# GiviMAD/rustpotter

Measured on AMD Instinct MI355X. Metric: 10ms-frame MFCC+DTW scorings/sec, higher is better.
Workload: dtype f32; 1 GPU; C3: 65536 synthetic 16 kHz f32 streams x 8 templates per GPU (4 s streams, L=100, K=5, band 5, ScoreMode::Max, avg gate off); streams_per_gpu=65536, templates=8, template_chunks=1, device=AMD Radeon Graphics, compute_units=256, build=gfx950, world_size=1, backend=none (one rank)

## Files before the change

### bindings/rustpotter_hip.rs

```rust
#![allow(non_camel_case_types)]
use std::collections::HashMap;
use std::ffi::{c_void, CStr, CString};
use std::os::raw::{c_char, c_int};

use crate::{
    AudioFmt, BandPassConfig, DetectorConfig, Endianness, FiltersConfig, GainNormalizationConfig, RustpotterConfig, SampleFormat,
    ScoreMode, VADMode, WakewordModel, WakewordRef, WakewordSave,
};

pub const RP_SAMPLE_I8: c_int = 0;
pub const RP_SAMPLE_I16: c_int = 1;
pub const RP_SAMPLE_I32: c_int = 2;
pub const RP_SAMPLE_F32: c_int = 3;
pub const RP_ENDIAN_BIG: c_int = 0;
pub const RP_ENDIAN_LITTLE: c_int = 1;
pub const RP_ENDIAN_NATIVE: c_int = 2;
pub const RP_SCORE_AVERAGE: c_int = 0;
pub const RP_SCORE_MAX: c_int = 1;
pub const RP_SCORE_MEDIAN: c_int = 2;
pub const RP_SCORE_P25: c_int = 3;
pub const RP_SCORE_P50: c_int = 4;
pub const RP_SCORE_P75: c_int = 5;
pub const RP_SCORE_P80: c_int = 6;
pub const RP_SCORE_P90: c_int = 7;
pub const RP_SCORE_P95: c_int = 8;
pub const RP_VAD_NONE: c_int = 0;
pub const RP_VAD_EASY: c_int = 1;
pub const RP_VAD_MEDIUM: c_int = 2;
pub const RP_VAD_HARD: c_int = 3;
pub const RP_MODEL_TINY: c_int = 0;
pub const RP_MODEL_SMALL: c_int = 1;
pub const RP_MODEL_MEDIUM: c_int = 2;
pub const RP_MODEL_LARGE: c_int = 3;
pub const RP_CTX_DEVICE_POINTERS: c_int = 0;
pub const RP_CTX_HOST_POINTERS: c_int = 1;
pub const RP_CTX_FULL_SCORES: c_int = 2;
pub const RP_CTX_ARITH_STRICT_F32: c_int = 4;
pub const RP_CTX_ARITH_FAST_SPLIT: c_int = 8;
pub const RP_CTX_RAGGED_MATRIX: c_int = 16;
pub const RP_ARITH_F32_MATRIX: c_int = 0;
pub const RP_ARITH_STRICT_F32: c_int = 1;
pub const RP_ARITH_FAST_SPLIT: c_int = 2;
pub const RP_DTW_KERNEL_MFMA: c_int = 1;
pub const RP_DTW_KERNEL_MFMA_WIDE: c_int = 2;
pub const RP_DTW_KERNEL_RAGGED: c_int = 4;
pub const RP_DTW_KERNEL_REGISTER: c_int = 8;
pub const RP_DTW_KERNEL_GENERIC: c_int = 16;
pub const RP_DTW_KERNEL_SINGLE: c_int = 32;
pub const RP_DTW_KERNEL_REF_ALL: c_int = 64;
pub const RP_DTW_KERNEL_MFMA_GROUP: c_int = 128;
pub const RP_DTW_PRODUCTS_BF16X3: c_int = 256;
pub const RP_DTW_PRODUCTS_F16X2: c_int = 512;
pub const RP_MLP_F32: c_int = 0;
pub const RP_MLP_BF16: c_int = 1;
pub const RP_MLP_F32_STRICT: c_int = 2;
pub const RP_MLP_F32_FAST: c_int = 3;

#[repr(C)] #[derive(Clone, Copy)] pub struct rp_audio_fmt { pub sample_rate: usize, pub sample_format: c_int, pub channels: u16, pub endianness: c_int }
#[repr(C)] #[derive(Clone, Copy)] pub struct rp_detector_config { pub avg_threshold: f32, pub threshold: f32, pub min_scores: usize, pub eager: bool, pub score_ref: f32, pub band_size: u16, pub score_mode: c_int, pub vad_mode: c_int }
#[repr(C)] #[derive(Clone, Copy)] pub struct rp_gain_normalization_config { pub enabled: bool, pub has_gain_ref: bool, pub gain_ref: f32, pub min_gain: f32, pub max_gain: f32 }
#[repr(C)] #[derive(Clone, Copy)] pub struct rp_band_pass_config { pub enabled: bool, pub low_cutoff: f32, pub high_cutoff: f32 }
#[repr(C)] #[derive(Clone, Copy)] pub struct rp_filters_config { pub gain_normalizer: rp_gain_normalization_config, pub band_pass: rp_band_pass_config }
#[repr(C)] #[derive(Clone, Copy)] pub struct rp_config { pub fmt: rp_audio_fmt, pub detector: rp_detector_config, pub filters: rp_filters_config }
#[repr(C)] pub struct rp_detection { pub name: *const c_char, pub avg_score: f32, pub score: f32, pub n_scores: usize, pub score_names: *const *const c_char, pub scores: *const f32, pub counter: usize, pub gain: f32 }
#[repr(C)] #[derive(Clone, Copy)] pub struct rp_train_options { pub m_type: c_int, pub learning_rate: f32, pub epochs: usize, pub test_epochs: usize, pub mfcc_size: u16, pub seed: u64 }
#[repr(C)] #[derive(Clone, Copy)] pub struct rp_wakeword_spec { pub templates: *const rp_templates, pub model: *const rp_model, pub none_index: c_int, pub precision: c_int, pub threshold: f32, pub avg_threshold: f32 }
#[repr(C)] #[derive(Clone, Copy, Default, Debug, PartialEq)] pub struct rp_batch_detection { pub stream: i32, pub frame: i32, pub window: i32, pub counter: i32, pub avg_score: f32, pub score: f32 }
pub enum rp_detector {}
pub enum rp_ctx {}
pub enum rp_templates {}
pub enum rp_stream_batch {}
pub enum rp_model {}

extern "C" {
    pub fn rp_config_default(out: *mut rp_config);
    pub fn rp_new(config: *const rp_config, out: *mut *mut rp_detector) -> c_int;
    pub fn rp_free(d: *mut rp_detector);
    pub fn rp_add_wakeword_from_buffer(d: *mut rp_detector, key: *const c_char, buffer: *const u8, len: usize) -> c_int;
    pub fn rp_add_wakeword_from_file(d: *mut rp_detector, key: *const c_char, path: *const c_char) -> c_int;
    pub fn rp_remove_wakeword(d: *mut rp_detector, key: *const c_char) -> bool;
    pub fn rp_remove_wakewords(d: *mut rp_detector) -> bool;
    pub fn rp_get_samples_per_frame(d: *const rp_detector) -> usize;
    pub fn rp_get_bytes_per_frame(d: *const rp_detector) -> usize;
    pub fn rp_get_partial_detection(d: *const rp_detector, out: *mut rp_detection) -> c_int;
    pub fn rp_get_rms_level(d: *const rp_detector) -> f32;
    pub fn rp_get_gain(d: *const rp_detector) -> f32;
    pub fn rp_get_rms_level_ref(d: *const rp_detector) -> f32;
    pub fn rp_process_bytes(d: *mut rp_detector, audio_bytes: *const u8, len: usize, out: *mut rp_detection) -> c_int;
    pub fn rp_process_samples_i8(d: *mut rp_detector, samples: *const i8, n: usize, out: *mut rp_detection) -> c_int;
    pub fn rp_process_samples_i16(d: *mut rp_detector, samples: *const i16, n: usize, out: *mut rp_detection) -> c_int;
    pub fn rp_process_samples_i32(d: *mut rp_detector, samples: *const i32, n: usize, out: *mut rp_detection) -> c_int;
    pub fn rp_process_samples_f32(d: *mut rp_detector, samples: *const f32, n: usize, out: *mut rp_detection) -> c_int;
    pub fn rp_update_config(d: *mut rp_detector, config: *const rp_config) -> c_int;
    pub fn rp_update_detector_config(d: *mut rp_detector, config: *const rp_detector_config) -> c_int;
    pub fn rp_update_filters_config(d: *mut rp_detector, config: *const rp_filters_config) -> c_int;
    pub fn rp_reset(d: *mut rp_detector);
    pub fn rp_last_error() -> *const c_char;

    pub fn rp_ctx_new(device: c_int, flags: c_int, out: *mut *mut rp_ctx) -> c_int;
    pub fn rp_ctx_free(ctx: *mut rp_ctx);
    pub fn rp_ctx_set_stream(ctx: *mut rp_ctx, hip_stream: *mut c_void) -> c_int;
    pub fn rp_ctx_synchronize(ctx: *mut rp_ctx) -> c_int;
    pub fn rp_ctx_dtw_ref_pairs(ctx: *mut rp_ctx, pairs: *mut u64) -> c_int;
    pub fn rp_ctx_dtw_kernels(ctx: *mut rp_ctx) -> c_int;
    pub fn rp_ctx_set_arithmetic(ctx: *mut rp_ctx, arith: c_int, ragged_matrix: c_int) -> c_int;
    pub fn rp_ctx_arithmetic(ctx: *mut rp_ctx, ragged_matrix: *mut c_int) -> c_int;
    pub fn rp_ctx_last_mlp_kernel(ctx: *mut rp_ctx) -> *const c_char;
    pub fn rp_build_info() -> *const c_char;
    pub fn rp_sharded_gather_info() -> *const c_char;
    pub fn rp_mfcc_num_frames(n_samples: usize) -> usize;
    pub fn rp_mfcc_batch(ctx: *mut rp_ctx, pcm: *const f32, S: usize, n_samples: usize, pcm_stride: usize, K: c_int, mfcc: *mut f32) -> c_int;
    pub fn rp_mfcc_batch_fmt(ctx: *mut rp_ctx, pcm: *const c_void, fmt: c_int, S: usize, n_samples: usize, pcm_stride: usize, K: c_int,
                             mfcc: *mut f32) -> c_int;
    pub fn rp_wakeword_ref_build(ctx: *mut rp_ctx, name: *const c_char, threshold: *const f32, avg_threshold: *const f32, n: usize,
                                 sample_names: *const *const c_char, wav_buffers: *const *const u8, wav_lens: *const usize,
                                 mfcc_size: u16, rms_from_files: c_int, out_rpw: *mut *mut u8, out_len: *mut usize) -> c_int;
    pub fn rp_buffer_free(buffer: *mut u8);
    pub fn rp_wakeword_model_train(ctx: *mut rp_ctx, options: *const rp_train_options, n_train: usize, train_names: *const *const c_char,
                                   train_wavs: *const *const u8, train_lens: *const usize, n_test: usize, test_names: *const *const c_char,
                                   test_wavs: *const *const u8, test_lens: *const usize, prev_model: *const u8, prev_model_len: usize,
                                   out_rpw: *mut *mut u8, out_len: *mut usize, final_loss: *mut f32, test_accuracy: *mut f32) -> c_int;
    pub fn rp_frontend_batch(ctx: *mut rp_ctx, pcm: *const c_void, fmt: c_int, S: usize, n_samples: usize, pcm_stride: usize,
                             filters: *const rp_filters_config, rms_level_ref: f32, window_size: usize, pcm_out: *mut f32,
                             out_stride: usize, rms: *mut f32, gains: *mut f32) -> c_int;
    pub fn rp_templates_new(ctx: *mut rp_ctx, T: c_int, K: c_int, lens: *const c_int, feats: *const f32, avg_len: c_int, avg: *const f32,
                            out: *mut *mut rp_templates) -> c_int;
    pub fn rp_templates_free(t: *mut rp_templates);
    pub fn rp_templates_max_len(t: *const rp_templates) -> c_int;
    pub fn rp_dtw_score_batch(ctx: *mut rp_ctx, mfcc: *const f32, S: usize, n_frames: usize, t: *const rp_templates, score_ref: f32,
                              band_size: c_int, score_mode: c_int, with_avg: c_int, scores: *mut f32, avg: *mut f32, agg: *mut f32) -> c_int;
    pub fn rp_detect_scan(ctx: *mut rp_ctx, agg: *const f32, avg: *const f32, S: usize, n_frames: usize, max_len: c_int,
                          config: *const rp_detector_config, avg_enabled: c_int, mfcc: *const f32, K: c_int,
                          det: *mut rp_batch_detection, n_det: *mut i32, max_det: c_int) -> c_int;
    pub fn rp_batch_detect(ctx: *mut rp_ctx, pcm: *const f32, S: usize, n_samples: usize, pcm_stride: usize, t: *const rp_templates,
                           config: *const rp_detector_config, det: *mut rp_batch_detection, n_det: *mut i32, max_det: c_int,
                           scores: *mut f32, agg: *mut f32) -> c_int;
    pub fn rp_batch_detect_fmt(ctx: *mut rp_ctx, pcm: *const c_void, fmt: c_int, S: usize, n_samples: usize, pcm_stride: usize,
                               t: *const rp_templates, config: *const rp_detector_config, det: *mut rp_batch_detection, n_det: *mut i32,
                               max_det: c_int, scores: *mut f32, agg: *mut f32) -> c_int;
    pub fn rp_batch_detect_ingest(ctx: *mut rp_ctx, pcm: *const c_void, fmt: c_int, S: usize, n_samples: usize, pcm_stride: usize,
                                  t: *const rp_templates, config: *const rp_detector_config, det: *mut rp_batch_detection, n_det: *mut i32,
                                  max_det: c_int, block_streams: usize, seconds: *mut f64) -> c_int;
    pub fn rp_batch_detect_sharded(ctxs: *const *mut rp_ctx, t: *const *const rp_templates, n_shards: c_int, pcm: *const *const c_void,
                                   fmt: c_int, S: *const usize, n_samples: usize, pcm_stride: usize, config: *const rp_detector_config,
                                   det: *mut rp_batch_detection, n_det: *mut i32, max_det: c_int) -> c_int;
    pub fn rp_batch_detect_multi(ctx: *mut rp_ctx, pcm: *const c_void, fmt: c_int, S: usize, n_samples: usize, pcm_stride: usize,
                                 n_wakewords: usize, t: *const *const rp_templates, config: *const rp_detector_config,
                                 thresholds: *const f32, avg_thresholds: *const f32, det: *mut rp_batch_detection,
                                 det_wakeword: *mut i32, n_det: *mut i32, max_det: c_int) -> c_int;
    pub fn rp_resampler_frame_lengths(sample_rate: usize, in_len: *mut usize, out_len: *mut usize) -> c_int;
    pub fn rp_resample_batch(ctx: *mut rp_ctx, pcm: *const c_void, fmt: c_int, channels: c_int, sample_rate: usize, S: usize,
                             n_samples: usize, pcm_stride: usize, out: *mut f32, out_stride: usize) -> c_int;
    pub fn rp_stream_batch_new(ctx: *mut rp_ctx, t: *const rp_templates, config: *const rp_detector_config, S: usize,
                               max_chunks_per_call: usize, out: *mut *mut rp_stream_batch) -> c_int;
    pub fn rp_stream_batch_free(b: *mut rp_stream_batch);
    pub fn rp_stream_batch_process(b: *mut rp_stream_batch, pcm: *const c_void, fmt: c_int, n_chunks: usize, pcm_stride: usize,
                                   det: *mut rp_batch_detection, n_det: *mut i32, max_det: c_int, agg: *mut f32) -> c_int;
    pub fn rp_stream_batch_set_input(b: *mut rp_stream_batch, sample_rate: usize, channels: c_int) -> c_int;
    pub fn rp_stream_batch_samples_per_chunk(b: *const rp_stream_batch) -> usize;
    pub fn rp_stream_batch_reset(b: *mut rp_stream_batch, stream: i64) -> c_int;
    pub fn rp_stream_batch_chunks_seen(b: *const rp_stream_batch) -> usize;
    pub fn rp_stream_batch_set_filters(b: *mut rp_stream_batch, filters: *const rp_filters_config, rms_level_ref: f32) -> c_int;
    pub fn rp_stream_batch_levels(b: *mut rp_stream_batch, rms: *mut f32, gains: *mut f32) -> c_int;
    pub fn rp_stream_batch_new_multi(ctx: *mut rp_ctx, n_wakewords: usize, wakewords: *const rp_wakeword_spec, mfcc_size: c_int,
                                     config: *const rp_detector_config, S: usize, max_chunks_per_call: usize, out: *mut *mut rp_stream_batch) -> c_int;
    pub fn rp_stream_batch_process_multi(b: *mut rp_stream_batch, pcm: *const c_void, fmt: c_int, n_chunks: usize, pcm_stride: usize,
                                         det: *mut rp_batch_detection, det_wakeword: *mut i32, det_label: *mut i32, n_det: *mut i32, max_det: c_int) -> c_int;
    pub fn rp_model_new(ctx: *mut rp_ctx, n_layers: c_int, dims: *const c_int, weights: *const *const f32, biases: *const *const f32,
                        out: *mut *mut rp_model) -> c_int;
    pub fn rp_model_free(m: *mut rp_model);
    pub fn rp_mlp_forward_batch(ctx: *mut rp_ctx, model: *const rp_model, x: *const f32, B: usize, precision: c_int, logits: *mut f32) -> c_int;
    pub fn rp_mlp_forward_windows(ctx: *mut rp_ctx, model: *const rp_model, mfcc: *const f32, S: usize, n_frames: usize, mfcc_size: c_int, precision: c_int, logits: *mut f32) -> c_int;
    pub fn rp_batch_detect_model(ctx: *mut rp_ctx, pcm: *const c_void, fmt: c_int, S: usize, n_samples: usize, pcm_stride: usize,
                                 model: *const rp_model, mfcc_size: c_int, none_index: c_int, config: *const rp_detector_config,
                                 precision: c_int, det: *mut rp_batch_detection, det_label: *mut i32, n_det: *mut i32, max_det: c_int) -> c_int;
    pub fn rp_synth_pcm_batch(ctx: *mut rp_ctx, seed: u64, first_stream: u64, S: usize, n_samples: usize, pcm_stride: usize, pcm: *mut f32) -> c_int;
    pub fn rp_ctx_timing_enable(ctx: *mut rp_ctx, enable: c_int) -> c_int;
    pub fn rp_ctx_timing_read(ctx: *mut rp_ctx, kernel: c_int, avg_ms: *mut f64, launches: *mut c_int) -> c_int;
    pub fn rp_ctx_timing_reset(ctx: *mut rp_ctx) -> c_int;
    pub fn rp_version() -> *const c_char;
}

impl From<&AudioFmt> for rp_audio_fmt {
    fn from(f: &AudioFmt) -> Self {
        rp_audio_fmt {
            sample_rate: f.sample_rate,
            sample_format: match f.sample_format { SampleFormat::I8 => RP_SAMPLE_I8, SampleFormat::I16 => RP_SAMPLE_I16, SampleFormat::I32 => RP_SAMPLE_I32, SampleFormat::F32 => RP_SAMPLE_F32 },
            channels: f.channels,
            endianness: match f.endianness { Endianness::Big => RP_ENDIAN_BIG, Endianness::Little => RP_ENDIAN_LITTLE, Endianness::Native => RP_ENDIAN_NATIVE },
        }
    }
}
pub fn score_mode_to_c(m: ScoreMode) -> c_int {
    match m {
        ScoreMode::Average => RP_SCORE_AVERAGE, ScoreMode::Max => RP_SCORE_MAX, ScoreMode::Median => RP_SCORE_MEDIAN,
        ScoreMode::P25 => RP_SCORE_P25, ScoreMode::P50 => RP_SCORE_P50, ScoreMode::P75 => RP_SCORE_P75,
        ScoreMode::P80 => RP_SCORE_P80, ScoreMode::P90 => RP_SCORE_P90, ScoreMode::P95 => RP_SCORE_P95,
    }
}
impl From<&DetectorConfig> for rp_detector_config {
    fn from(d: &DetectorConfig) -> Self {
        rp_detector_config {
            avg_threshold: d.avg_threshold, threshold: d.threshold, min_scores: d.min_scores, eager: d.eager, score_ref: d.score_ref,
            band_size: d.band_size, score_mode: score_mode_to_c(d.score_mode),
            vad_mode: match d.vad_mode { None => RP_VAD_NONE, Some(VADMode::Easy) => RP_VAD_EASY, Some(VADMode::Medium) => RP_VAD_MEDIUM, Some(VADMode::Hard) => RP_VAD_HARD },
        }
    }
}
impl From<&GainNormalizationConfig> for rp_gain_normalization_config {
    fn from(g: &GainNormalizationConfig) -> Self {
        rp_gain_normalization_config { enabled: g.enabled, has_gain_ref: g.gain_ref.is_some(), gain_ref: g.gain_ref.unwrap_or(0.0), min_gain: g.min_gain, max_gain: g.max_gain }
    }
}
impl From<&BandPassConfig> for rp_band_pass_config {
    fn from(b: &BandPassConfig) -> Self { rp_band_pass_config { enabled: b.enabled, low_cutoff: b.low_cutoff, high_cutoff: b.high_cutoff } }
}
impl From<&FiltersConfig> for rp_filters_config {
    fn from(f: &FiltersConfig) -> Self { rp_filters_config { gain_normalizer: (&f.gain_normalizer).into(), band_pass: (&f.band_pass).into() } }
}
impl From<&RustpotterConfig> for rp_config {
    fn from(c: &RustpotterConfig) -> Self { rp_config { fmt: (&c.fmt).into(), detector: (&c.detector).into(), filters: (&c.filters).into() } }
}

pub struct RustpotterDetection { pub name: String, pub avg_score: f32, pub score: f32, pub scores: HashMap<String, f32>, pub counter: usize, pub gain: f32 }

pub trait Sample: Copy { unsafe fn process(d: *mut rp_detector, s: &[Self], out: *mut rp_detection) -> c_int; }
impl Sample for i8 { unsafe fn process(d: *mut rp_detector, s: &[i8], o: *mut rp_detection) -> c_int { rp_process_samples_i8(d, s.as_ptr(), s.len(), o) } }
impl Sample for i16 { unsafe fn process(d: *mut rp_detector, s: &[i16], o: *mut rp_detection) -> c_int { rp_process_samples_i16(d, s.as_ptr(), s.len(), o) } }
impl Sample for i32 { unsafe fn process(d: *mut rp_detector, s: &[i32], o: *mut rp_detection) -> c_int { rp_process_samples_i32(d, s.as_ptr(), s.len(), o) } }
impl Sample for f32 { unsafe fn process(d: *mut rp_detector, s: &[f32], o: *mut rp_detection) -> c_int { rp_process_samples_f32(d, s.as_ptr(), s.len(), o) } }

fn last_error() -> String { unsafe { CStr::from_ptr(rp_last_error()).to_string_lossy().into_owned() } }
fn status(r: c_int) -> Result<(), String> { if r < 0 { Err(last_error()) } else { Ok(()) } }
unsafe fn owned(d: &rp_detection) -> RustpotterDetection {
    let mut scores = HashMap::new();
    for i in 0..d.n_scores { scores.insert(CStr::from_ptr(*d.score_names.add(i)).to_string_lossy().into_owned(), *d.scores.add(i)); }
    RustpotterDetection { name: CStr::from_ptr(d.name).to_string_lossy().into_owned(), avg_score: d.avg_score, score: d.score, scores, counter: d.counter, gain: d.gain }
}

pub struct Rustpotter { h: *mut rp_detector, partial: Option<RustpotterDetection> }
unsafe impl Send for Rustpotter {}
impl Drop for Rustpotter { fn drop(&mut self) { unsafe { rp_free(self.h) } } }
impl Rustpotter {
    pub fn new(config: &RustpotterConfig) -> Result<Rustpotter, String> {
        let c: rp_config = config.into();
        let mut h = std::ptr::null_mut();
        if unsafe { rp_new(&c, &mut h) } < 0 { Err(last_error()) } else { Ok(Rustpotter { h, partial: None }) }
    }
    fn refresh_partial(&mut self) {
        let mut d = std::mem::MaybeUninit::<rp_detection>::uninit();
        self.partial = unsafe { if rp_get_partial_detection(self.h, d.as_mut_ptr()) == 1 { Some(owned(&d.assume_init())) } else { None } };
    }
    pub fn add_wakeword_ref(&mut self, key: &str, wakeword: WakewordRef) -> Result<(), String> {
        self.add_wakeword_from_buffer(key, &wakeword.save_to_buffer()?)
    }
    pub fn add_wakeword_model(&mut self, key: &str, wakeword: WakewordModel) -> Result<(), String> {
        self.add_wakeword_from_buffer(key, &wakeword.save_to_buffer()?)
    }
    pub fn add_wakeword_from_buffer(&mut self, key: &str, buffer: &[u8]) -> Result<(), String> {
        let k = CString::new(key).map_err(|e| e.to_string())?;
        let r = status(unsafe { rp_add_wakeword_from_buffer(self.h, k.as_ptr(), buffer.as_ptr(), buffer.len()) });
        self.refresh_partial();
        r
    }
    pub fn add_wakeword_from_file(&mut self, key: &str, path: &str) -> Result<(), String> {
        let (k, p) = (CString::new(key).map_err(|e| e.to_string())?, CString::new(path).map_err(|e| e.to_string())?);
        let r = status(unsafe { rp_add_wakeword_from_file(self.h, k.as_ptr(), p.as_ptr()) });
        self.refresh_partial();
        r
    }
    pub fn remove_wakeword(&mut self, key: &str) -> bool { CString::new(key).map(|k| unsafe { rp_remove_wakeword(self.h, k.as_ptr()) }).unwrap_or(false) }
    pub fn remove_wakewords(&mut self) -> bool { unsafe { rp_remove_wakewords(self.h) } }
    pub fn get_samples_per_frame(&self) -> usize { unsafe { rp_get_samples_per_frame(self.h) } }
    pub fn get_bytes_per_frame(&self) -> usize { unsafe { rp_get_bytes_per_frame(self.h) } }
    pub fn get_partial_detection(&self) -> Option<&RustpotterDetection> { self.partial.as_ref() }
    pub fn get_rms_level(&self) -> f32 { unsafe { rp_get_rms_level(self.h) } }
    pub fn get_gain(&self) -> f32 { unsafe { rp_get_gain(self.h) } }
    pub fn get_rms_level_ref(&self) -> f32 { unsafe { rp_get_rms_level_ref(self.h) } }
    pub fn process_bytes(&mut self, audio_bytes: &[u8]) -> Option<RustpotterDetection> {
        let mut d = std::mem::MaybeUninit::<rp_detection>::uninit();
        let r = unsafe { if rp_process_bytes(self.h, audio_bytes.as_ptr(), audio_bytes.len(), d.as_mut_ptr()) == 1 { Some(owned(&d.assume_init())) } else { None } };
        self.refresh_partial();
        r
    }
    pub fn process_samples<T: Sample>(&mut self, audio_samples: Vec<T>) -> Option<RustpotterDetection> {
        let mut d = std::mem::MaybeUninit::<rp_detection>::uninit();
        let r = unsafe { if T::process(self.h, &audio_samples, d.as_mut_ptr()) == 1 { Some(owned(&d.assume_init())) } else { None } };
        self.refresh_partial();
        r
    }
    pub fn update_config(&mut self, config: &RustpotterConfig) { let c: rp_config = config.into(); unsafe { rp_update_config(self.h, &c); } self.refresh_partial(); }
    pub fn update_detector_config(&mut self, config: &DetectorConfig) { let c: rp_detector_config = config.into(); unsafe { rp_update_detector_config(self.h, &c); } self.refresh_partial(); }
    pub fn update_filters_config(&mut self, config: &FiltersConfig) { let c: rp_filters_config = config.into(); unsafe { rp_update_filters_config(self.h, &c); } self.refresh_partial(); }
    pub fn reset(&mut self) { unsafe { rp_reset(self.h) } self.partial = None; }
}

pub fn default_c_config() -> rp_config { let mut c = std::mem::MaybeUninit::<rp_config>::uninit(); unsafe { rp_config_default(c.as_mut_ptr()); c.assume_init() } }
pub fn version() -> String { unsafe { CStr::from_ptr(rp_version()).to_string_lossy().into_owned() } }
pub fn build_info() -> String { unsafe { CStr::from_ptr(rp_build_info()).to_string_lossy().into_owned() } }
pub fn sharded_gather_info() -> String { unsafe { CStr::from_ptr(rp_sharded_gather_info()).to_string_lossy().into_owned() } }
pub fn mfcc_num_frames(n_samples: usize) -> usize { unsafe { rp_mfcc_num_frames(n_samples) } }
pub fn resampler_frame_lengths(sample_rate: usize) -> Result<(usize, usize), String> {
    let (mut i, mut o) = (0usize, 0usize);
    status(unsafe { rp_resampler_frame_lengths(sample_rate, &mut i, &mut o) })?;
    Ok((i, o))
}

pub struct Templates { h: *mut rp_templates, pub n_templates: usize, pub mfcc_size: usize }
impl Drop for Templates { fn drop(&mut self) { unsafe { rp_templates_free(self.h) } } }
impl Templates {
    pub fn max_len(&self) -> usize { unsafe { rp_templates_max_len(self.h) as usize } }
}
pub struct Model { h: *mut rp_model, pub dims: Vec<c_int> }
impl Drop for Model { fn drop(&mut self) { unsafe { rp_model_free(self.h) } } }

pub struct WindowScores { pub n_win: usize, pub scores: Vec<f32>, pub avg: Vec<f32>, pub agg: Vec<f32> }
pub type Detections = Vec<Vec<rp_batch_detection>>;

fn split_detections(det: Vec<rp_batch_detection>, n_det: Vec<i32>, max_det: usize) -> Detections {
    (0..n_det.len()).map(|s| det[s * max_det..s * max_det + (n_det[s].max(0) as usize).min(max_det)].to_vec()).collect()
}

pub struct HipContext { h: *mut rp_ctx }
unsafe impl Send for HipContext {}
impl Drop for HipContext { fn drop(&mut self) { unsafe { rp_ctx_free(self.h) } } }
impl HipContext {
    pub fn new(device: c_int) -> Result<HipContext, String> { HipContext::with_flags(device, RP_CTX_HOST_POINTERS) }
    pub fn with_flags(device: c_int, flags: c_int) -> Result<HipContext, String> {
        let mut h = std::ptr::null_mut();
        status(unsafe { rp_ctx_new(device, flags, &mut h) })?;
        Ok(HipContext { h })
    }
    pub fn raw(&self) -> *mut rp_ctx { self.h }
    pub fn set_stream(&self, hip_stream: *mut c_void) -> Result<(), String> { status(unsafe { rp_ctx_set_stream(self.h, hip_stream) }) }
    pub fn synchronize(&self) -> Result<(), String> { status(unsafe { rp_ctx_synchronize(self.h) }) }
    pub fn last_mlp_kernel(&self) -> String {
        let p = unsafe { rp_ctx_last_mlp_kernel(self.h) };
        if p.is_null() { String::new() } else { unsafe { CStr::from_ptr(p) }.to_string_lossy().into_owned() }
    }
    pub fn dtw_kernels(&self) -> u32 { unsafe { rp_ctx_dtw_kernels(self.h) as u32 } }
    pub fn set_arithmetic(&self, arith: c_int, ragged_matrix: bool) -> Result<(), String> {
        status(unsafe { rp_ctx_set_arithmetic(self.h, arith, ragged_matrix as c_int) })
    }
    pub fn arithmetic(&self) -> (c_int, bool) {
        let mut r: c_int = 0;
        let a = unsafe { rp_ctx_arithmetic(self.h, &mut r) };
        (a, r != 0)
    }
    pub fn dtw_ref_pairs(&self) -> Result<u64, String> {
        let mut v: u64 = 0;
        status(unsafe { rp_ctx_dtw_ref_pairs(self.h, &mut v) })?;
        Ok(v)
    }

    pub fn mfcc_batch(&self, pcm: &[f32], n_streams: usize, n_samples: usize, mfcc_size: u16) -> Result<Vec<f32>, String> {
        assert!(pcm.len() >= n_streams * n_samples);
        let mut out = vec![0f32; n_streams * mfcc_num_frames(n_samples) * mfcc_size as usize];
        status(unsafe { rp_mfcc_batch(self.h, pcm.as_ptr(), n_streams, n_samples, n_samples, mfcc_size as c_int, out.as_mut_ptr()) })?;
        Ok(out)
    }
    pub fn mfcc_batch_fmt<T: Sample>(&self, pcm: &[T], fmt: SampleFormat, n_streams: usize, n_samples: usize, mfcc_size: u16) -> Result<Vec<f32>, String> {
        assert!(pcm.len() >= n_streams * n_samples);
        let f = rp_audio_fmt::from(&AudioFmt { sample_rate: 16000, sample_format: fmt, channels: 1, endianness: Endianness::Native }).sample_format;
        let mut out = vec![0f32; n_streams * mfcc_num_frames(n_samples) * mfcc_size as usize];
        status(unsafe { rp_mfcc_batch_fmt(self.h, pcm.as_ptr() as *const c_void, f, n_streams, n_samples, n_samples, mfcc_size as c_int, out.as_mut_ptr()) })?;
        Ok(out)
    }
    pub fn templates(&self, templates: &[Vec<Vec<f32>>], avg: Option<&Vec<Vec<f32>>>) -> Result<Templates, String> {
        let k = templates.first().and_then(|t| t.first()).map_or(0, |f| f.len());
        let lens: Vec<c_int> = templates.iter().map(|t| t.len() as c_int).collect();
        let feats: Vec<f32> = templates.iter().flat_map(|t| t.iter().flatten().copied()).collect();
        let avg_flat: Vec<f32> = avg.map_or(Vec::new(), |a| a.iter().flatten().copied().collect());
        let mut h = std::ptr::null_mut();
        status(unsafe {
            rp_templates_new(self.h, lens.len() as c_int, k as c_int, lens.as_ptr(), feats.as_ptr(), avg.map_or(0, |a| a.len() as c_int),
                             if avg.is_some() { avg_flat.as_ptr() } else { std::ptr::null() }, &mut h)
        })?;
        Ok(Templates { h, n_templates: lens.len(), mfcc_size: k })
    }
    pub fn templates_from_ref(&self, w: &WakewordRef) -> Result<Templates, String> {
        let t: Vec<Vec<Vec<f32>>> = w.samples_features.values().cloned().collect();
        self.templates(&t, w.avg_features.as_ref())
    }
    pub fn dtw_score_batch(&self, mfcc: &[f32], n_streams: usize, n_frames: usize, t: &Templates, score_ref: f32, band_size: u16,
                           score_mode: ScoreMode, with_avg: bool) -> Result<WindowScores, String> {
        assert!(mfcc.len() >= n_streams * n_frames * t.mfcc_size);
        let n_win = (n_frames + 1).saturating_sub(t.max_len());
        let mut r = WindowScores { n_win, scores: vec![0f32; n_streams * n_win * t.n_templates], avg: vec![0f32; if with_avg { n_streams * n_win } else { 0 }],
                                   agg: vec![0f32; n_streams * n_win] };
        status(unsafe {
            rp_dtw_score_batch(self.h, mfcc.as_ptr(), n_streams, n_frames, t.h, score_ref, band_size as c_int, score_mode_to_c(score_mode),
                               with_avg as c_int, r.scores.as_mut_ptr(), if with_avg { r.avg.as_mut_ptr() } else { std::ptr::null_mut() }, r.agg.as_mut_ptr())
        })?;
        Ok(r)
    }
    pub fn detect_scan(&self, w: &WindowScores, n_streams: usize, n_frames: usize, max_len: usize, config: &DetectorConfig,
                       mfcc: Option<(&[f32], u16)>, max_det: usize) -> Result<Detections, String> {
        let c: rp_detector_config = config.into();
        let mut det = vec![rp_batch_detection::default(); n_streams * max_det];
        let mut n_det = vec![0i32; n_streams];
        let (mp, k) = mfcc.map_or((std::ptr::null(), 0), |(m, k)| (m.as_ptr(), k as c_int));
        status(unsafe {
            rp_detect_scan(self.h, w.agg.as_ptr(), if w.avg.is_empty() { std::ptr::null() } else { w.avg.as_ptr() }, n_streams, n_frames,
                           max_len as c_int, &c, !w.avg.is_empty() as c_int, mp, k, det.as_mut_ptr(), n_det.as_mut_ptr(), max_det as c_int)
        })?;
        Ok(split_detections(det, n_det, max_det))
    }
    pub fn batch_detect(&self, pcm: &[f32], n_streams: usize, n_samples: usize, t: &Templates, config: &DetectorConfig, max_det: usize) -> Result<Detections, String> {
        assert!(pcm.len() >= n_streams * n_samples);
        let c: rp_detector_config = config.into();
        let mut det = vec![rp_batch_detection::default(); n_streams * max_det];
        let mut n_det = vec![0i32; n_streams];
        status(unsafe {
            rp_batch_detect(self.h, pcm.as_ptr(), n_streams, n_samples, n_samples, t.h, &c, det.as_mut_ptr(), n_det.as_mut_ptr(), max_det as c_int,
                            std::ptr::null_mut(), std::ptr::null_mut())
        })?;
        Ok(split_detections(det, n_det, max_det))
    }
    pub fn batch_detect_i16(&self, pcm: &[i16], n_streams: usize, n_samples: usize, t: &Templates, config: &DetectorConfig, max_det: usize) -> Result<Detections, String> {
        assert!(pcm.len() >= n_streams * n_samples);
        let c: rp_detector_config = config.into();
        let mut det = vec![rp_batch_detection::default(); n_streams * max_det];
        let mut n_det = vec![0i32; n_streams];
        status(unsafe {
            rp_batch_detect_fmt(self.h, pcm.as_ptr() as *const c_void, RP_SAMPLE_I16, n_streams, n_samples, n_samples, t.h, &c, det.as_mut_ptr(),
                                n_det.as_mut_ptr(), max_det as c_int, std::ptr::null_mut(), std::ptr::null_mut())
        })?;
        Ok(split_detections(det, n_det, max_det))
    }
    pub fn batch_detect_ingest_i16(&self, pcm: &[i16], n_streams: usize, n_samples: usize, t: &Templates, config: &DetectorConfig, max_det: usize,
                                   block_streams: usize) -> Result<(Detections, f64), String> {
        assert!(pcm.len() >= n_streams * n_samples);
        let c: rp_detector_config = config.into();
        let mut det = vec![rp_batch_detection::default(); n_streams * max_det];
        let mut n_det = vec![0i32; n_streams];
        let mut seconds = 0f64;
        status(unsafe {
            rp_batch_detect_ingest(self.h, pcm.as_ptr() as *const c_void, RP_SAMPLE_I16, n_streams, n_samples, n_samples, t.h, &c, det.as_mut_ptr(),
                                   n_det.as_mut_ptr(), max_det as c_int, block_streams, &mut seconds)
        })?;
        Ok((split_detections(det, n_det, max_det), seconds))
    }
    pub fn batch_detect_multi(&self, pcm: &[f32], n_streams: usize, n_samples: usize, wakewords: &[&Templates], overrides: &[(Option<f32>, Option<f32>)],
                              config: &DetectorConfig, max_det: usize) -> Result<(Detections, Vec<Vec<i32>>), String> {
        assert!(pcm.len() >= n_streams * n_samples && overrides.len() == wakewords.len());
        let c: rp_detector_config = config.into();
        let ts: Vec<*const rp_templates> = wakewords.iter().map(|t| t.h as *const rp_templates).collect();
        let thr: Vec<f32> = overrides.iter().map(|o| o.0.unwrap_or(f32::NAN)).collect();
        let athr: Vec<f32> = overrides.iter().map(|o| o.1.unwrap_or(f32::NAN)).collect();
        let mut det = vec![rp_batch_detection::default(); n_streams * max_det];
        let mut which = vec![0i32; n_streams * max_det];
        let mut n_det = vec![0i32; n_streams];
        status(unsafe {
            rp_batch_detect_multi(self.h, pcm.as_ptr() as *const c_void, RP_SAMPLE_F32, n_streams, n_samples, n_samples, ts.len(), ts.as_ptr(), &c,
                                  thr.as_ptr(), athr.as_ptr(), det.as_mut_ptr(), which.as_mut_ptr(), n_det.as_mut_ptr(), max_det as c_int)
        })?;
        let w = (0..n_streams).map(|s| which[s * max_det..s * max_det + (n_det[s].max(0) as usize).min(max_det)].to_vec()).collect();
        Ok((split_detections(det, n_det, max_det), w))
    }
    pub fn model(&self, dims: &[c_int], weights: &[Vec<f32>], biases: &[Vec<f32>]) -> Result<Model, String> {
        assert!(dims.len() == weights.len() + 1 && weights.len() == biases.len());
        let wp: Vec<*const f32> = weights.iter().map(|w| w.as_ptr()).collect();
        let bp: Vec<*const f32> = biases.iter().map(|b| b.as_ptr()).collect();
        let mut h = std::ptr::null_mut();
        status(unsafe { rp_model_new(self.h, weights.len() as c_int, dims.as_ptr(), wp.as_ptr(), bp.as_ptr(), &mut h) })?;
        Ok(Model { h, dims: dims.to_vec() })
    }
    pub fn mlp_forward_batch(&self, m: &Model, x: &[f32], rows: usize, bf16: bool) -> Result<Vec<f32>, String> {
        assert!(x.len() >= rows * m.dims[0] as usize);
        let mut out = vec![0f32; rows * *m.dims.last().unwrap() as usize];
        status(unsafe { rp_mlp_forward_batch(self.h, m.h, x.as_ptr(), rows, if bf16 { RP_MLP_BF16 } else { RP_MLP_F32 }, out.as_mut_ptr()) })?;
        Ok(out)
    }
    pub fn mlp_forward_windows(&self, m: &Model, mfcc: &[f32], n_streams: usize, n_frames: usize, mfcc_size: u16) -> Result<Vec<f32>, String> {
        assert!(mfcc.len() >= n_streams * n_frames * mfcc_size as usize);
        let train_size = m.dims[0] as usize / mfcc_size as usize;
        let n_win = if n_frames >= train_size { n_frames - train_size + 1 } else { 0 };
        let mut out = vec![0f32; n_streams * n_win * *m.dims.last().unwrap() as usize];
        status(unsafe { rp_mlp_forward_windows(self.h, m.h, mfcc.as_ptr(), n_streams, n_frames, mfcc_size as c_int, RP_MLP_F32, out.as_mut_ptr()) })?;
        Ok(out)
    }
    pub fn batch_detect_model(&self, pcm: &[f32], n_streams: usize, n_samples: usize, m: &Model, mfcc_size: u16, none_index: Option<usize>,
                              config: &DetectorConfig, bf16: bool, max_det: usize) -> Result<(Detections, Vec<Vec<i32>>), String> {
        assert!(pcm.len() >= n_streams * n_samples);
        let c: rp_detector_config = config.into();
        let mut det = vec![rp_batch_detection::default(); n_streams * max_det];
        let mut label = vec![0i32; n_streams * max_det];
        let mut n_det = vec![0i32; n_streams];
        status(unsafe {
            rp_batch_detect_model(self.h, pcm.as_ptr() as *const c_void, RP_SAMPLE_F32, n_streams, n_samples, n_samples, m.h, mfcc_size as c_int,
                                  none_index.map_or(-1, |i| i as c_int), &c, if bf16 { RP_MLP_BF16 } else { RP_MLP_F32 }, det.as_mut_ptr(),
                                  label.as_mut_ptr(), n_det.as_mut_ptr(), max_det as c_int)
        })?;
        let l = (0..n_streams).map(|s| label[s * max_det..s * max_det + (n_det[s].max(0) as usize).min(max_det)].to_vec()).collect();
        Ok((split_detections(det, n_det, max_det), l))
    }
    pub fn frontend_batch(&self, pcm: &[f32], n_streams: usize, n_samples: usize, filters: &FiltersConfig, rms_level_ref: f32,
                          window_size: usize) -> Result<(Vec<f32>, Vec<f32>, Vec<f32>), String> {
        assert!(pcm.len() >= n_streams * n_samples);
        let f: rp_filters_config = filters.into();
        let nch = n_samples / 480;
        let (mut out, mut rms, mut gains) = (vec![0f32; n_streams * n_samples], vec![0f32; n_streams * nch], vec![0f32; n_streams * nch]);
        status(unsafe {
            rp_frontend_batch(self.h, pcm.as_ptr() as *const c_void, RP_SAMPLE_F32, n_streams, n_samples, n_samples, &f, rms_level_ref, window_size,
                              out.as_mut_ptr(), n_samples, rms.as_mut_ptr(), gains.as_mut_ptr())
        })?;
        Ok((out, rms, gains))
    }
    pub fn resample_batch(&self, pcm: &[f32], channels: u16, sample_rate: usize, n_streams: usize, n_samples: usize) -> Result<Vec<f32>, String> {
        assert!(pcm.len() >= n_streams * n_samples * channels as usize);
        let (fi, fo) = resampler_frame_lengths(sample_rate)?;
        let per = (n_samples / fi) * fo;
        let mut out = vec![0f32; n_streams * per];
        status(unsafe {
            rp_resample_batch(self.h, pcm.as_ptr() as *const c_void, RP_SAMPLE_F32, channels as c_int, sample_rate, n_streams, n_samples,
                              n_samples * channels as usize, out.as_mut_ptr(), per)
        })?;
        Ok(out)
    }
    pub fn synth_pcm_batch(&self, seed: u64, first_stream: u64, n_streams: usize, n_samples: usize) -> Result<Vec<f32>, String> {
        let mut out = vec![0f32; n_streams * n_samples];
        status(unsafe { rp_synth_pcm_batch(self.h, seed, first_stream, n_streams, n_samples, n_samples, out.as_mut_ptr()) })?;
        Ok(out)
    }
    pub fn timing_enable(&self, on: bool) -> Result<(), String> { status(unsafe { rp_ctx_timing_enable(self.h, on as c_int) }) }
    pub fn timing_reset(&self) -> Result<(), String> { status(unsafe { rp_ctx_timing_reset(self.h) }) }
    pub fn timing_read(&self, kernel: c_int) -> Result<(f64, c_int), String> {
        let (mut ms, mut n) = (0f64, 0 as c_int);
        status(unsafe { rp_ctx_timing_read(self.h, kernel, &mut ms, &mut n) })?;
        Ok((ms, n))
    }
}

pub struct StreamBatch<'a> { h: *mut rp_stream_batch, n_streams: usize, last_chunks: usize, _ctx: &'a HipContext, _t: std::marker::PhantomData<&'a Templates> }
pub enum BatchWakeword<'a> {
    Ref { templates: &'a Templates, threshold: Option<f32>, avg_threshold: Option<f32> },
    Model { model: &'a Model, none_index: Option<usize>, bf16: bool },
}
impl<'a> Drop for StreamBatch<'a> { fn drop(&mut self) { unsafe { rp_stream_batch_free(self.h) } } }
impl<'a> StreamBatch<'a> {
    pub fn new(ctx: &'a HipContext, t: &'a Templates, config: &DetectorConfig, n_streams: usize, max_chunks_per_call: usize) -> Result<StreamBatch<'a>, String> {
        let c: rp_detector_config = config.into();
        let mut h = std::ptr::null_mut();
        status(unsafe { rp_stream_batch_new(ctx.h, t.h, &c, n_streams, max_chunks_per_call, &mut h) })?;
        Ok(StreamBatch { h, n_streams, last_chunks: 0, _ctx: ctx, _t: std::marker::PhantomData })
    }
    pub fn new_multi(ctx: &'a HipContext, wakewords: &[BatchWakeword<'a>], mfcc_size: u16, config: &DetectorConfig, n_streams: usize,
                     max_chunks_per_call: usize) -> Result<StreamBatch<'a>, String> {
        let c: rp_detector_config = config.into();
        let specs: Vec<rp_wakeword_spec> = wakewords.iter().map(|w| match w {
            BatchWakeword::Ref { templates, threshold, avg_threshold } => rp_wakeword_spec {
                templates: templates.h as *const rp_templates, model: std::ptr::null(), none_index: -1, precision: RP_MLP_F32,
                threshold: threshold.unwrap_or(f32::NAN), avg_threshold: avg_threshold.unwrap_or(f32::NAN) },
            BatchWakeword::Model { model, none_index, bf16 } => rp_wakeword_spec {
                templates: std::ptr::null(), model: model.h as *const rp_model, none_index: none_index.map_or(-1, |i| i as c_int),
                precision: if *bf16 { RP_MLP_BF16 } else { RP_MLP_F32 }, threshold: f32::NAN, avg_threshold: f32::NAN },
        }).collect();
        let mut h = std::ptr::null_mut();
        status(unsafe { rp_stream_batch_new_multi(ctx.h, specs.len(), specs.as_ptr(), mfcc_size as c_int, &c, n_streams, max_chunks_per_call, &mut h) })?;
        Ok(StreamBatch { h, n_streams, last_chunks: 0, _ctx: ctx, _t: std::marker::PhantomData })
    }
    pub fn process_multi(&mut self, pcm: &[f32], n_chunks: usize, max_det: usize) -> Result<(Detections, Vec<Vec<i32>>, Vec<Vec<i32>>), String> {
        let stride = n_chunks * self.samples_per_chunk();
        assert!(pcm.len() >= self.n_streams * stride);
        let mut det = vec![rp_batch_detection::default(); self.n_streams * max_det];
        let (mut which, mut label) = (vec![0i32; self.n_streams * max_det], vec![0i32; self.n_streams * max_det]);
        let mut n_det = vec![0i32; self.n_streams];
        status(unsafe {
            rp_stream_batch_process_multi(self.h, pcm.as_ptr() as *const c_void, RP_SAMPLE_F32, n_chunks, stride, det.as_mut_ptr(), which.as_mut_ptr(),
                                          label.as_mut_ptr(), n_det.as_mut_ptr(), max_det as c_int)
        })?;
        self.last_chunks = n_chunks;
        let cut = |v: &Vec<i32>| -> Vec<Vec<i32>> { (0..self.n_streams).map(|s| v[s * max_det..s * max_det + (n_det[s].max(0) as usize).min(max_det)].to_vec()).collect() };
        let (w, l) = (cut(&which), cut(&label));
        Ok((split_detections(det, n_det, max_det), w, l))
    }
    pub fn set_input(&mut self, sample_rate: usize, channels: u16) -> Result<(), String> { status(unsafe { rp_stream_batch_set_input(self.h, sample_rate, channels as c_int) }) }
    pub fn set_filters(&mut self, filters: &FiltersConfig, rms_level_ref: f32) -> Result<(), String> {
        let f: rp_filters_config = filters.into();
        status(unsafe { rp_stream_batch_set_filters(self.h, &f, rms_level_ref) })
    }
    pub fn levels(&mut self) -> Result<(Vec<f32>, Vec<f32>), String> {
        let n = self.n_streams * self.last_chunks.max(1);
        let (mut rms, mut gains) = (vec![0f32; n], vec![0f32; n]);
        status(unsafe { rp_stream_batch_levels(self.h, rms.as_mut_ptr(), gains.as_mut_ptr()) })?;
        Ok((rms, gains))
    }
    pub fn samples_per_chunk(&self) -> usize { unsafe { rp_stream_batch_samples_per_chunk(self.h) } }
    pub fn chunks_seen(&self) -> usize { unsafe { rp_stream_batch_chunks_seen(self.h) } }
    pub fn process(&mut self, pcm: &[f32], n_chunks: usize, max_det: usize) -> Result<Detections, String> {
        let stride = n_chunks * self.samples_per_chunk();
        assert!(pcm.len() >= self.n_streams * stride);
        let mut det = vec![rp_batch_detection::default(); self.n_streams * max_det];
        let mut n_det = vec![0i32; self.n_streams];
        status(unsafe {
            rp_stream_batch_process(self.h, pcm.as_ptr() as *const c_void, RP_SAMPLE_F32, n_chunks, stride, det.as_mut_ptr(), n_det.as_mut_ptr(),
                                    max_det as c_int, std::ptr::null_mut())
        })?;
        self.last_chunks = n_chunks;
        Ok(split_detections(det, n_det, max_det))
    }
    pub fn reset(&mut self, stream: Option<usize>) -> Result<(), String> { status(unsafe { rp_stream_batch_reset(self.h, stream.map_or(-1, |s| s as i64)) }) }
}

pub fn batch_detect_sharded(devices: &[c_int], templates: &[Vec<Vec<f32>>], avg: Option<&Vec<Vec<f32>>>, config: &DetectorConfig,
                            shards: &[Vec<Vec<f32>>], max_det: usize) -> Result<Detections, String> {
    assert_eq!(devices.len(), shards.len());
    let c: rp_detector_config = config.into();
    let n_samples = shards.iter().flat_map(|s| s.iter()).map(|x| x.len()).next().unwrap_or(0);
    assert!(shards.iter().flat_map(|s| s.iter()).all(|x| x.len() == n_samples), "every stream must hold the same number of samples");
    let ctxs: Vec<HipContext> = devices.iter().map(|&d| HipContext::new(d)).collect::<Result<_, _>>()?;
    let tms: Vec<Templates> = ctxs.iter().map(|c| c.templates(templates, avg)).collect::<Result<_, _>>()?;
    let cp: Vec<*mut rp_ctx> = ctxs.iter().map(|c| c.h).collect();
    let tp: Vec<*const rp_templates> = tms.iter().map(|t| t.h as *const rp_templates).collect();
    let flat: Vec<Vec<f32>> = shards.iter().map(|s| s.iter().flatten().copied().collect()).collect();
    let ptrs: Vec<*const c_void> = flat.iter().map(|f| f.as_ptr() as *const c_void).collect();
    let counts: Vec<usize> = shards.iter().map(|s| s.len()).collect();
    let total: usize = counts.iter().sum();
    let mut det = vec![rp_batch_detection::default(); total * max_det];
    let mut n_det = vec![0i32; total];
    status(unsafe {
        rp_batch_detect_sharded(cp.as_ptr(), tp.as_ptr(), devices.len() as c_int, ptrs.as_ptr(), RP_SAMPLE_F32, counts.as_ptr(), n_samples,
                                n_samples, &c, det.as_mut_ptr(), n_det.as_mut_ptr(), max_det as c_int)
    })?;
    Ok(split_detections(det, n_det, max_det))
}

fn take_buffer(r: c_int, out: *mut u8, out_len: usize) -> Result<Vec<u8>, String> {
    let res = if r < 0 { Err(last_error()) } else { Ok(unsafe { std::slice::from_raw_parts(out, out_len) }.to_vec()) };
    if !out.is_null() { unsafe { rp_buffer_free(out) }; }
    res
}
pub fn wakeword_ref_from_sample_buffers(name: &str, threshold: Option<f32>, avg_threshold: Option<f32>,
                                        samples: &HashMap<String, Vec<u8>>, mfcc_size: u16) -> Result<Vec<u8>, String> {
    let cname = CString::new(name).map_err(|e| e.to_string())?;
    let names: Vec<CString> = samples.keys().map(|k| CString::new(k.as_str()).unwrap()).collect();
    let name_ptrs: Vec<*const c_char> = names.iter().map(|n| n.as_ptr()).collect();
    let bufs: Vec<*const u8> = samples.values().map(|v| v.as_ptr()).collect();
    let lens: Vec<usize> = samples.values().map(|v| v.len()).collect();
    let ctx = HipContext::with_flags(0, RP_CTX_DEVICE_POINTERS)?;
    let (mut out, mut out_len) = (std::ptr::null_mut(), 0usize);
    let r = unsafe {
        rp_wakeword_ref_build(ctx.h, cname.as_ptr(), threshold.as_ref().map_or(std::ptr::null(), |t| t as *const f32),
                              avg_threshold.as_ref().map_or(std::ptr::null(), |t| t as *const f32), names.len(),
                              name_ptrs.as_ptr(), bufs.as_ptr(), lens.as_ptr(), mfcc_size, 0, &mut out, &mut out_len)
    };
    take_buffer(r, out, out_len)
}
pub fn wakeword_model_train_from_buffers(m_type: c_int, train: &HashMap<String, Vec<u8>>, test: &HashMap<String, Vec<u8>>,
                                         learning_rate: f64, epochs: usize, test_epochs: usize, mfcc_size: u16,
                                         wakeword_model: Option<&[u8]>) -> Result<(Vec<u8>, f32, f32), String> {
    fn pack(d: &HashMap<String, Vec<u8>>) -> (Vec<CString>, Vec<*const u8>, Vec<usize>) {
        (d.keys().map(|k| CString::new(k.as_str()).unwrap()).collect(), d.values().map(|v| v.as_ptr()).collect(), d.values().map(|v| v.len()).collect())
    }
    let (trn, trb, trl) = pack(train);
    let (ten, teb, tel) = pack(test);
    let trp: Vec<*const c_char> = trn.iter().map(|n| n.as_ptr()).collect();
    let tep: Vec<*const c_char> = ten.iter().map(|n| n.as_ptr()).collect();
    let opt = rp_train_options { m_type, learning_rate: learning_rate as f32, epochs, test_epochs, mfcc_size, seed: 1 };
    let ctx = HipContext::with_flags(0, RP_CTX_DEVICE_POINTERS)?;
    let (mut out, mut out_len, mut loss, mut acc) = (std::ptr::null_mut(), 0usize, 0f32, 0f32);
    let (pm, pl) = wakeword_model.map_or((std::ptr::null(), 0), |m| (m.as_ptr(), m.len()));
    let r = unsafe {
        rp_wakeword_model_train(ctx.h, &opt, trp.len(), trp.as_ptr(), trb.as_ptr(), trl.as_ptr(), tep.len(), tep.as_ptr(), teb.as_ptr(),
                                tel.as_ptr(), pm, pl, &mut out, &mut out_len, &mut loss, &mut acc)
    };
    take_buffer(r, out, out_len).map(|b| (b, loss, acc))
}
```

### include/rustpotter_hip.h

```cpp
#ifndef RUSTPOTTER_HIP_H
#define RUSTPOTTER_HIP_H

#include <stdbool.h>
#include <stddef.h>
#include <stdint.h>

#ifdef __cplusplus
extern "C" {
#endif

typedef enum { RP_SAMPLE_I8 = 0, RP_SAMPLE_I16 = 1, RP_SAMPLE_I32 = 2, RP_SAMPLE_F32 = 3 } rp_sample_format;
typedef enum { RP_ENDIAN_BIG = 0, RP_ENDIAN_LITTLE = 1, RP_ENDIAN_NATIVE = 2 } rp_endianness;
typedef enum {
    RP_SCORE_AVERAGE = 0, RP_SCORE_MAX = 1, RP_SCORE_MEDIAN = 2, RP_SCORE_P25 = 3, RP_SCORE_P50 = 4,
    RP_SCORE_P75 = 5, RP_SCORE_P80 = 6, RP_SCORE_P90 = 7, RP_SCORE_P95 = 8
} rp_score_mode;
typedef enum { RP_VAD_NONE = 0, RP_VAD_EASY = 1, RP_VAD_MEDIUM = 2, RP_VAD_HARD = 3 } rp_vad_mode;

typedef struct {
    size_t sample_rate;
    rp_sample_format sample_format;
    uint16_t channels;
    rp_endianness endianness;
} rp_audio_fmt;

typedef struct {
    float avg_threshold;
    float threshold;
    size_t min_scores;
    bool eager;
    float score_ref;
    uint16_t band_size;
    rp_score_mode score_mode;
    rp_vad_mode vad_mode;
} rp_detector_config;

typedef struct {
    bool enabled;
    bool has_gain_ref;
    float gain_ref;
    float min_gain;
    float max_gain;
} rp_gain_normalization_config;

typedef struct {
    bool enabled;
    float low_cutoff;
    float high_cutoff;
} rp_band_pass_config;

typedef struct {
    rp_gain_normalization_config gain_normalizer;
    rp_band_pass_config band_pass;
} rp_filters_config;

typedef struct {
    rp_audio_fmt fmt;
    rp_detector_config detector;
    rp_filters_config filters;
} rp_config;

void rp_config_default(rp_config *out);

typedef struct {
    const char *name;
    float avg_score;
    float score;
    size_t n_scores;
    const char *const *score_names;
    const float *scores;
    size_t counter;
    float gain;
} rp_detection;

typedef struct rp_detector rp_detector;

int rp_new(const rp_config *config, rp_detector **out);
void rp_free(rp_detector *d);

int rp_add_wakeword_from_buffer(rp_detector *d, const char *key, const uint8_t *buffer, size_t len);
int rp_add_wakeword_from_file(rp_detector *d, const char *key, const char *path);
bool rp_remove_wakeword(rp_detector *d, const char *key);
bool rp_remove_wakewords(rp_detector *d);

size_t rp_get_samples_per_frame(const rp_detector *d);
size_t rp_get_bytes_per_frame(const rp_detector *d);
int rp_get_partial_detection(const rp_detector *d, rp_detection *out);
float rp_get_rms_level(const rp_detector *d);
float rp_get_gain(const rp_detector *d);
float rp_get_rms_level_ref(const rp_detector *d);

int rp_process_bytes(rp_detector *d, const uint8_t *audio_bytes, size_t len, rp_detection *out);
int rp_process_samples_i8(rp_detector *d, const int8_t *samples, size_t n, rp_detection *out);
int rp_process_samples_i16(rp_detector *d, const int16_t *samples, size_t n, rp_detection *out);
int rp_process_samples_i32(rp_detector *d, const int32_t *samples, size_t n, rp_detection *out);
int rp_process_samples_f32(rp_detector *d, const float *samples, size_t n, rp_detection *out);

int rp_update_config(rp_detector *d, const rp_config *config);
int rp_update_detector_config(rp_detector *d, const rp_detector_config *config);
int rp_update_filters_config(rp_detector *d, const rp_filters_config *config);
void rp_reset(rp_detector *d);

const char *rp_last_error(void);

typedef struct rp_ctx rp_ctx;
typedef struct rp_templates rp_templates;

enum {
    RP_CTX_DEVICE_POINTERS = 0, RP_CTX_HOST_POINTERS = 1, RP_CTX_FULL_SCORES = 2,
    RP_CTX_ARITH_STRICT_F32 = 4, RP_CTX_ARITH_FAST_SPLIT = 8,
    RP_CTX_RAGGED_MATRIX = 16
};

int rp_ctx_new(int device, int flags, rp_ctx **out);
enum { RP_ARITH_F32_MATRIX = 0, RP_ARITH_STRICT_F32 = 1, RP_ARITH_FAST_SPLIT = 2 };
int rp_ctx_set_arithmetic(rp_ctx *ctx, int arith, int ragged_matrix);
int rp_ctx_arithmetic(rp_ctx *ctx, int *ragged_matrix);
void rp_ctx_free(rp_ctx *ctx);
int rp_ctx_set_stream(rp_ctx *ctx, void *hip_stream);
int rp_ctx_synchronize(rp_ctx *ctx);
int rp_ctx_dtw_ref_pairs(rp_ctx *ctx, uint64_t *pairs);
enum {
    RP_DTW_KERNEL_MFMA = 1,
    RP_DTW_KERNEL_MFMA_WIDE = 2,
    RP_DTW_KERNEL_RAGGED = 4,
    RP_DTW_KERNEL_REGISTER = 8,
    RP_DTW_KERNEL_GENERIC = 16,
    RP_DTW_KERNEL_SINGLE = 32,
    RP_DTW_KERNEL_REF_ALL = 64,
    RP_DTW_KERNEL_MFMA_GROUP = 128,
    RP_DTW_PRODUCTS_BF16X3 = 256,
    RP_DTW_PRODUCTS_F16X2 = 512
};
int rp_ctx_dtw_kernels(rp_ctx *ctx);
const char *rp_build_info(void);
const char *rp_ctx_last_mlp_kernel(rp_ctx *ctx);

size_t rp_mfcc_num_frames(size_t n_samples);

int rp_mfcc_batch(rp_ctx *ctx, const float *pcm, size_t S, size_t n_samples, size_t pcm_stride, int K, float *mfcc);

int rp_mfcc_batch_fmt(rp_ctx *ctx, const void *pcm, rp_sample_format fmt, size_t S, size_t n_samples, size_t pcm_stride,
                      int K, float *mfcc);

int rp_wakeword_ref_build(rp_ctx *ctx, const char *name, const float *threshold, const float *avg_threshold, size_t n,
                          const char *const *sample_names, const uint8_t *const *wav_buffers, const size_t *wav_lens,
                          uint16_t mfcc_size, int rms_from_files, uint8_t **out_rpw, size_t *out_len);
void rp_buffer_free(uint8_t *buffer);

typedef enum { RP_MODEL_TINY = 0, RP_MODEL_SMALL = 1, RP_MODEL_MEDIUM = 2, RP_MODEL_LARGE = 3 } rp_model_type;
typedef struct {
    int m_type;
    float learning_rate;
    size_t epochs, test_epochs;
    uint16_t mfcc_size;
    uint64_t seed;
} rp_train_options;
int rp_wakeword_model_train(rp_ctx *ctx, const rp_train_options *options, size_t n_train, const char *const *train_names,
                            const uint8_t *const *train_wavs, const size_t *train_lens, size_t n_test,
                            const char *const *test_names, const uint8_t *const *test_wavs, const size_t *test_lens,
                            const uint8_t *prev_model, size_t prev_model_len, uint8_t **out_rpw, size_t *out_len,
                            float *final_loss, float *test_accuracy);

int rp_frontend_batch(rp_ctx *ctx, const void *pcm, rp_sample_format fmt, size_t S, size_t n_samples, size_t pcm_stride,
                      const rp_filters_config *filters, float rms_level_ref, size_t window_size, float *pcm_out,
                      size_t out_stride, float *rms, float *gains);

int rp_templates_new(rp_ctx *ctx, int T, int K, const int *lens, const float *feats, int avg_len, const float *avg,
                     rp_templates **out);
void rp_templates_free(rp_templates *t);
int rp_templates_max_len(const rp_templates *t);

int rp_dtw_score_batch(rp_ctx *ctx, const float *mfcc, size_t S, size_t n_frames, const rp_templates *t,
                       float score_ref, int band_size, rp_score_mode score_mode, int with_avg,
                       float *scores, float *avg, float *agg);

typedef struct {
    int32_t stream;
    int32_t frame;
    int32_t window;
    int32_t counter;
    float avg_score;
    float score;
} rp_batch_detection;

int rp_detect_scan(rp_ctx *ctx, const float *agg, const float *avg, size_t S, size_t n_frames, int max_len,
                   const rp_detector_config *config, int avg_enabled, const float *mfcc, int K,
                   rp_batch_detection *det, int32_t *n_det, int max_det);

int rp_batch_detect(rp_ctx *ctx, const float *pcm, size_t S, size_t n_samples, size_t pcm_stride, const rp_templates *t,
                    const rp_detector_config *config, rp_batch_detection *det, int32_t *n_det, int max_det,
                    float *scores, float *agg);

int rp_batch_detect_fmt(rp_ctx *ctx, const void *pcm, rp_sample_format fmt, size_t S, size_t n_samples, size_t pcm_stride,
                        const rp_templates *t, const rp_detector_config *config, rp_batch_detection *det, int32_t *n_det,
                        int max_det, float *scores, float *agg);

int rp_batch_detect_ingest(rp_ctx *ctx, const void *pcm, rp_sample_format fmt, size_t S, size_t n_samples, size_t pcm_stride,
                           const rp_templates *t, const rp_detector_config *config, rp_batch_detection *det, int32_t *n_det,
                           int max_det, size_t block_streams, double *seconds);

int rp_batch_detect_sharded(rp_ctx *const *ctxs, const rp_templates *const *t, int n_shards, const void *const *pcm,
                            rp_sample_format fmt, const size_t *S, size_t n_samples, size_t pcm_stride,
                            const rp_detector_config *config, rp_batch_detection *det, int32_t *n_det, int max_det);
const char *rp_sharded_gather_info(void);

int rp_batch_detect_multi(rp_ctx *ctx, const void *pcm, rp_sample_format fmt, size_t S, size_t n_samples, size_t pcm_stride,
                          size_t n_wakewords, const rp_templates *const *t, const rp_detector_config *config,
                          const float *thresholds, const float *avg_thresholds, rp_batch_detection *det,
                          int32_t *det_wakeword, int32_t *n_det, int max_det);

int rp_resampler_frame_lengths(size_t sample_rate, size_t *in_len, size_t *out_len);
int rp_resample_batch(rp_ctx *ctx, const void *pcm, rp_sample_format fmt, int channels, size_t sample_rate, size_t S,
                      size_t n_samples, size_t pcm_stride, float *out, size_t out_stride);

typedef struct rp_stream_batch rp_stream_batch;
int rp_stream_batch_new(rp_ctx *ctx, const rp_templates *t, const rp_detector_config *config, size_t S,
                        size_t max_chunks_per_call, rp_stream_batch **out);
void rp_stream_batch_free(rp_stream_batch *b);
int rp_stream_batch_process(rp_stream_batch *b, const void *pcm, rp_sample_format fmt, size_t n_chunks, size_t pcm_stride,
                            rp_batch_detection *det, int32_t *n_det, int max_det, float *agg);
int rp_stream_batch_set_input(rp_stream_batch *b, size_t sample_rate, int channels);
size_t rp_stream_batch_samples_per_chunk(const rp_stream_batch *b);
int rp_stream_batch_reset(rp_stream_batch *b, long long stream);
size_t rp_stream_batch_chunks_seen(const rp_stream_batch *b);
int rp_stream_batch_set_filters(rp_stream_batch *b, const rp_filters_config *filters, float rms_level_ref);
int rp_stream_batch_levels(rp_stream_batch *b, float *rms, float *gains);

typedef struct rp_model rp_model;
typedef struct {
    const rp_templates *templates;
    const rp_model *model;
    int none_index;
    int precision;
    float threshold;
    float avg_threshold;
} rp_wakeword_spec;
int rp_stream_batch_new_multi(rp_ctx *ctx, size_t n_wakewords, const rp_wakeword_spec *wakewords, int mfcc_size,
                              const rp_detector_config *config, size_t S, size_t max_chunks_per_call, rp_stream_batch **out);
int rp_stream_batch_process_multi(rp_stream_batch *b, const void *pcm, rp_sample_format fmt, size_t n_chunks, size_t pcm_stride,
                                  rp_batch_detection *det, int32_t *det_wakeword, int32_t *det_label, int32_t *n_det, int max_det);

int rp_model_new(rp_ctx *ctx, int n_layers, const int *dims, const float *const *weights, const float *const *biases,
                 rp_model **out);
void rp_model_free(rp_model *m);

enum { RP_MLP_F32 = 0, RP_MLP_BF16 = 1, RP_MLP_F32_STRICT = 2, RP_MLP_F32_FAST = 3 };

int rp_mlp_forward_batch(rp_ctx *ctx, const rp_model *model, const float *x, size_t B, int precision, float *logits);

int rp_mlp_forward_windows(rp_ctx *ctx, const rp_model *model, const float *mfcc, size_t S, size_t n_frames, int mfcc_size,
                           int precision, float *logits);

int rp_batch_detect_model(rp_ctx *ctx, const void *pcm, rp_sample_format fmt, size_t S, size_t n_samples, size_t pcm_stride,
                          const rp_model *model, int mfcc_size, int none_index, const rp_detector_config *config, int precision,
                          rp_batch_detection *det, int32_t *det_label, int32_t *n_det, int max_det);

int rp_synth_pcm_batch(rp_ctx *ctx, uint64_t seed, uint64_t first_stream, size_t S, size_t n_samples, size_t pcm_stride,
                       float *pcm);

int rp_ctx_timing_enable(rp_ctx *ctx, int enable);
int rp_ctx_timing_read(rp_ctx *ctx, int kernel, double *avg_ms, int *launches);
int rp_ctx_timing_reset(rp_ctx *ctx);

const char *rp_version(void);

#ifdef __cplusplus
}
#endif
#endif
```

### rustpotter_amd/api.py

```python
import ctypes as C
import weakref
import enum
import os

_HERE = os.path.dirname(os.path.abspath(__file__))
_LIB = None


class RustpotterError(RuntimeError):
    """Result::Err(String) of the reference."""


def lib_path():
    return os.environ.get("RP_LIB_PATH") or os.path.join(_HERE, "librustpotter_hip.so")


class SampleFormat(enum.IntEnum):
    I8 = 0
    I16 = 1
    I32 = 2
    F32 = 3


class Endianness(enum.IntEnum):
    Big = 0
    Little = 1
    Native = 2


class ScoreMode(enum.IntEnum):
    Average = 0
    Max = 1
    Median = 2
    P25 = 3
    P50 = 4
    P75 = 5
    P80 = 6
    P90 = 7
    P95 = 8


class VADMode(enum.IntEnum):
    Off = 0
    Easy = 1
    Medium = 2
    Hard = 3


class _AudioFmt(C.Structure):
    _fields_ = [("sample_rate", C.c_size_t), ("sample_format", C.c_int), ("channels", C.c_uint16), ("endianness", C.c_int)]


class _DetectorConfig(C.Structure):
    _fields_ = [("avg_threshold", C.c_float), ("threshold", C.c_float), ("min_scores", C.c_size_t), ("eager", C.c_bool),
                ("score_ref", C.c_float), ("band_size", C.c_uint16), ("score_mode", C.c_int), ("vad_mode", C.c_int)]


class _GainCfg(C.Structure):
    _fields_ = [("enabled", C.c_bool), ("has_gain_ref", C.c_bool), ("gain_ref", C.c_float), ("min_gain", C.c_float),
                ("max_gain", C.c_float)]


class _BandPassCfg(C.Structure):
    _fields_ = [("enabled", C.c_bool), ("low_cutoff", C.c_float), ("high_cutoff", C.c_float)]


class _FiltersCfg(C.Structure):
    _fields_ = [("gain_normalizer", _GainCfg), ("band_pass", _BandPassCfg)]


class _Config(C.Structure):
    _fields_ = [("fmt", _AudioFmt), ("detector", _DetectorConfig), ("filters", _FiltersCfg)]


class _Detection(C.Structure):
    _fields_ = [("name", C.c_char_p), ("avg_score", C.c_float), ("score", C.c_float), ("n_scores", C.c_size_t),
                ("score_names", C.POINTER(C.c_char_p)), ("scores", C.POINTER(C.c_float)), ("counter", C.c_size_t),
                ("gain", C.c_float)]


class _TrainOptions(C.Structure):
    _fields_ = [("m_type", C.c_int), ("learning_rate", C.c_float), ("epochs", C.c_size_t), ("test_epochs", C.c_size_t),
                ("mfcc_size", C.c_uint16), ("seed", C.c_uint64)]


class _BatchDetection(C.Structure):
    _fields_ = [("stream", C.c_int32), ("frame", C.c_int32), ("window", C.c_int32), ("counter", C.c_int32),
                ("avg_score", C.c_float), ("score", C.c_float)]


SYMBOLS = [
    "rp_config_default", "rp_new", "rp_free", "rp_add_wakeword_from_buffer", "rp_add_wakeword_from_file",
    "rp_remove_wakeword", "rp_remove_wakewords", "rp_get_samples_per_frame", "rp_get_bytes_per_frame",
    "rp_get_partial_detection", "rp_get_rms_level", "rp_get_gain", "rp_get_rms_level_ref", "rp_process_bytes",
    "rp_process_samples_i8", "rp_process_samples_i16", "rp_process_samples_i32", "rp_process_samples_f32",
    "rp_update_config", "rp_update_detector_config", "rp_update_filters_config", "rp_reset", "rp_last_error",
    "rp_ctx_new", "rp_ctx_free", "rp_ctx_set_stream", "rp_ctx_synchronize", "rp_ctx_dtw_ref_pairs", "rp_ctx_dtw_kernels", "rp_ctx_set_arithmetic", "rp_ctx_arithmetic", "rp_ctx_last_mlp_kernel", "rp_build_info", "rp_sharded_gather_info", "rp_mfcc_num_frames", "rp_mfcc_batch", "rp_mfcc_batch_fmt", "rp_batch_detect_fmt", "rp_batch_detect_ingest", "rp_frontend_batch", "rp_wakeword_ref_build", "rp_buffer_free",
    "rp_templates_new", "rp_templates_free", "rp_templates_max_len", "rp_dtw_score_batch", "rp_detect_scan", "rp_batch_detect",
    "rp_model_new", "rp_model_free", "rp_mlp_forward_batch", "rp_mlp_forward_windows", "rp_synth_pcm_batch", "rp_ctx_timing_enable", "rp_ctx_timing_read", "rp_ctx_timing_reset",
    "rp_version", "rp_stream_batch_new", "rp_stream_batch_free", "rp_stream_batch_process", "rp_stream_batch_reset",
    "rp_stream_batch_chunks_seen", "rp_resampler_frame_lengths", "rp_resample_batch",
    "rp_wakeword_model_train", "rp_stream_batch_set_input", "rp_stream_batch_samples_per_chunk",
    "rp_batch_detect_multi", "rp_batch_detect_model", "rp_batch_detect_sharded",
    "rp_stream_batch_new_multi", "rp_stream_batch_process_multi",
    "rp_stream_batch_set_filters", "rp_stream_batch_levels",
]


class _WakewordSpec(C.Structure):
    _fields_ = [("templates", C.c_void_p), ("model", C.c_void_p), ("none_index", C.c_int), ("precision", C.c_int),
                ("threshold", C.c_float), ("avg_threshold", C.c_float)]


def load_library():
    global _LIB
    if _LIB is not None:
        return _LIB
    path = lib_path()
    if not os.path.exists(path):
        raise RustpotterError(
            "librustpotter_hip.so is not built (%s): run `python -c 'import __graft_entry__ as g; g.build()'` "
            "or `make -C rustpotter_amd/csrc`; there is no CPU fallback" % path)
    try:
        import torch
    except Exception:
        pass
    L = C.CDLL(path)
    vp, fp, ip = C.c_void_p, C.POINTER(C.c_float), C.POINTER(C.c_int)
    L.rp_last_error.restype = C.c_char_p
    L.rp_version.restype = C.c_char_p
    L.rp_config_default.argtypes = [C.POINTER(_Config)]
    L.rp_new.argtypes = [C.POINTER(_Config), C.POINTER(vp)]
    L.rp_free.argtypes = [vp]
    L.rp_add_wakeword_from_buffer.argtypes = [vp, C.c_char_p, C.c_char_p, C.c_size_t]
    L.rp_add_wakeword_from_file.argtypes = [vp, C.c_char_p, C.c_char_p]
    L.rp_remove_wakeword.argtypes = [vp, C.c_char_p]
    L.rp_remove_wakeword.restype = C.c_bool
    L.rp_remove_wakewords.argtypes = [vp]
    L.rp_remove_wakewords.restype = C.c_bool
    L.rp_get_samples_per_frame.argtypes = [vp]
    L.rp_get_samples_per_frame.restype = C.c_size_t
    L.rp_get_bytes_per_frame.argtypes = [vp]
    L.rp_get_bytes_per_frame.restype = C.c_size_t
    L.rp_get_partial_detection.argtypes = [vp, C.POINTER(_Detection)]
    for n in ("rp_get_rms_level", "rp_get_gain", "rp_get_rms_level_ref"):
        getattr(L, n).argtypes = [vp]
        getattr(L, n).restype = C.c_float
    L.rp_process_bytes.argtypes = [vp, C.c_char_p, C.c_size_t, C.POINTER(_Detection)]
    for n in ("rp_process_samples_i8", "rp_process_samples_i16", "rp_process_samples_i32", "rp_process_samples_f32"):
        getattr(L, n).argtypes = [vp, vp, C.c_size_t, C.POINTER(_Detection)]
    L.rp_update_config.argtypes = [vp, C.POINTER(_Config)]
    L.rp_update_detector_config.argtypes = [vp, C.POINTER(_DetectorConfig)]
    L.rp_update_filters_config.argtypes = [vp, C.POINTER(_FiltersCfg)]
    L.rp_reset.argtypes = [vp]
    L.rp_ctx_new.argtypes = [C.c_int, C.c_int, C.POINTER(vp)]
    L.rp_ctx_free.argtypes = [vp]
    L.rp_ctx_set_stream.argtypes = [vp, vp]
    L.rp_ctx_synchronize.argtypes = [vp]
    L.rp_ctx_dtw_ref_pairs.argtypes = [vp, C.POINTER(C.c_uint64)]
    L.rp_ctx_dtw_kernels.argtypes = [vp]
    L.rp_ctx_dtw_kernels.restype = C.c_int
    L.rp_ctx_set_arithmetic.argtypes = [vp, C.c_int, C.c_int]
    L.rp_ctx_set_arithmetic.restype = C.c_int
    L.rp_ctx_arithmetic.argtypes = [vp, C.POINTER(C.c_int)]
    L.rp_ctx_arithmetic.restype = C.c_int
    L.rp_sharded_gather_info.argtypes = []
    L.rp_sharded_gather_info.restype = C.c_char_p
    L.rp_build_info.argtypes = []
    L.rp_build_info.restype = C.c_char_p
    L.rp_ctx_last_mlp_kernel.argtypes = [vp]
    L.rp_ctx_last_mlp_kernel.restype = C.c_char_p
    L.rp_mfcc_num_frames.argtypes = [C.c_size_t]
    L.rp_mfcc_num_frames.restype = C.c_size_t
    L.rp_mfcc_batch.argtypes = [vp, vp, C.c_size_t, C.c_size_t, C.c_size_t, C.c_int, vp]
    L.rp_mfcc_batch_fmt.argtypes = [vp, vp, C.c_int, C.c_size_t, C.c_size_t, C.c_size_t, C.c_int, vp]
    L.rp_batch_detect_fmt.argtypes = [vp, vp, C.c_int, C.c_size_t, C.c_size_t, C.c_size_t, vp, C.POINTER(_DetectorConfig), vp, vp, C.c_int, vp, vp]
    L.rp_batch_detect_ingest.argtypes = [vp, vp, C.c_int, C.c_size_t, C.c_size_t, C.c_size_t, vp, C.POINTER(_DetectorConfig), vp, vp, C.c_int, C.c_size_t,
                                         C.POINTER(C.c_double)]
    L.rp_frontend_batch.argtypes = [vp, vp, C.c_int, C.c_size_t, C.c_size_t, C.c_size_t, C.POINTER(_FiltersCfg), C.c_float, C.c_size_t, vp, C.c_size_t, vp, vp]
    L.rp_wakeword_ref_build.argtypes = [vp, C.c_char_p, fp, fp, C.c_size_t, C.POINTER(C.c_char_p), C.POINTER(C.c_char_p),
                                        C.POINTER(C.c_size_t), C.c_uint16, C.c_int, C.POINTER(vp), C.POINTER(C.c_size_t)]
    L.rp_buffer_free.argtypes = [vp]
    L.rp_templates_new.argtypes = [vp, C.c_int, C.c_int, ip, fp, C.c_int, fp, C.POINTER(vp)]
    L.rp_templates_free.argtypes = [vp]
    L.rp_templates_max_len.argtypes = [vp]
    L.rp_dtw_score_batch.argtypes = [vp, vp, C.c_size_t, C.c_size_t, vp, C.c_float, C.c_int, C.c_int, C.c_int, vp, vp, vp]
    L.rp_detect_scan.argtypes = [vp, vp, vp, C.c_size_t, C.c_size_t, C.c_int, C.POINTER(_DetectorConfig), C.c_int, vp, C.c_int, vp, vp, C.c_int]
    L.rp_batch_detect.argtypes = [vp, vp, C.c_size_t, C.c_size_t, C.c_size_t, vp, C.POINTER(_DetectorConfig), vp, vp, C.c_int, vp, vp]
    L.rp_wakeword_model_train.argtypes = [vp, C.POINTER(_TrainOptions), C.c_size_t, C.POINTER(C.c_char_p), C.POINTER(C.c_char_p),
                                          C.POINTER(C.c_size_t), C.c_size_t, C.POINTER(C.c_char_p), C.POINTER(C.c_char_p),
                                          C.POINTER(C.c_size_t), C.c_char_p, C.c_size_t, C.POINTER(vp), C.POINTER(C.c_size_t), fp, fp]
    L.rp_batch_detect_multi.argtypes = [vp, vp, C.c_int, C.c_size_t, C.c_size_t, C.c_size_t, C.c_size_t, C.POINTER(vp),
                                        C.POINTER(_DetectorConfig), fp, fp, vp, vp, vp, C.c_int]
    L.rp_batch_detect_sharded.argtypes = [C.POINTER(vp), C.POINTER(vp), C.c_int, C.POINTER(vp), C.c_int, C.POINTER(C.c_size_t), C.c_size_t,
                                          C.c_size_t, C.POINTER(_DetectorConfig), vp, vp, C.c_int]
    L.rp_batch_detect_model.argtypes = [vp, vp, C.c_int, C.c_size_t, C.c_size_t, C.c_size_t, vp, C.c_int, C.c_int,
                                        C.POINTER(_DetectorConfig), C.c_int, vp, vp, vp, C.c_int]
    L.rp_resampler_frame_lengths.argtypes = [C.c_size_t, C.POINTER(C.c_size_t), C.POINTER(C.c_size_t)]
    L.rp_resample_batch.argtypes = [vp, vp, C.c_int, C.c_int, C.c_size_t, C.c_size_t, C.c_size_t, C.c_size_t, vp, C.c_size_t]
    L.rp_stream_batch_new.argtypes = [vp, vp, C.POINTER(_DetectorConfig), C.c_size_t, C.c_size_t, C.POINTER(vp)]
    L.rp_stream_batch_new_multi.argtypes = [vp, C.c_size_t, C.POINTER(_WakewordSpec), C.c_int, C.POINTER(_DetectorConfig), C.c_size_t,
                                            C.c_size_t, C.POINTER(vp)]
    L.rp_stream_batch_process_multi.argtypes = [vp, vp, C.c_int, C.c_size_t, C.c_size_t, vp, vp, vp, vp, C.c_int]
    L.rp_stream_batch_free.argtypes = [vp]
    L.rp_stream_batch_free.restype = None
    L.rp_stream_batch_process.argtypes = [vp, vp, C.c_int, C.c_size_t, C.c_size_t, vp, vp, C.c_int, vp]
    L.rp_stream_batch_reset.argtypes = [vp, C.c_longlong]
    L.rp_stream_batch_set_input.argtypes = [vp, C.c_size_t, C.c_int]
    L.rp_stream_batch_set_filters.argtypes = [vp, C.POINTER(_FiltersCfg), C.c_float]
    L.rp_stream_batch_levels.argtypes = [vp, vp, vp]
    L.rp_stream_batch_samples_per_chunk.argtypes = [vp]
    L.rp_stream_batch_samples_per_chunk.restype = C.c_size_t
    L.rp_stream_batch_chunks_seen.argtypes = [vp]
    L.rp_stream_batch_chunks_seen.restype = C.c_size_t
    L.rp_model_new.argtypes = [vp, C.c_int, ip, C.POINTER(fp), C.POINTER(fp), C.POINTER(vp)]
    L.rp_model_free.argtypes = [vp]
    L.rp_mlp_forward_batch.argtypes = [vp, vp, vp, C.c_size_t, C.c_int, vp]
    L.rp_mlp_forward_windows.argtypes = [vp, vp, vp, C.c_size_t, C.c_size_t, C.c_int, C.c_int, vp]
    L.rp_synth_pcm_batch.argtypes = [vp, C.c_uint64, C.c_uint64, C.c_size_t, C.c_size_t, C.c_size_t, vp]
    L.rp_ctx_timing_enable.argtypes = [vp, C.c_int]
    L.rp_ctx_timing_read.argtypes = [vp, C.c_int, C.POINTER(C.c_double), ip]
    L.rp_ctx_timing_reset.argtypes = [vp]
    _LIB = L
    return L


def _err():
    return RustpotterError(load_library().rp_last_error().decode("utf-8", "replace"))


def sharded_gather_info():
    return load_library().rp_sharded_gather_info().decode()


def build_info():
    return load_library().rp_build_info().decode()


def resampler_frame_lengths(sample_rate):
    a, b = C.c_size_t(), C.c_size_t()
    if load_library().rp_resampler_frame_lengths(sample_rate, C.byref(a), C.byref(b)) < 0:
        raise _err()
    return a.value, b.value


def mfcc_num_frames(n_samples):
    return int(load_library().rp_mfcc_num_frames(n_samples))


class AudioFmt:
    def __init__(self):
        self.sample_rate = 16000
        self.sample_format = SampleFormat.F32
        self.channels = 1
        self.endianness = Endianness.Little


class GainNormalizationConfig:
    def __init__(self):
        self.enabled = False
        self.gain_ref = None
        self.min_gain = 0.1
        self.max_gain = 1.0


class BandPassConfig:
    def __init__(self):
        self.enabled = False
        self.low_cutoff = 80.0
        self.high_cutoff = 400.0


class FiltersConfig:
    def __init__(self):
        self.gain_normalizer = GainNormalizationConfig()
        self.band_pass = BandPassConfig()


class DetectorConfig:
    def __init__(self):
        self.avg_threshold = 0.2
        self.threshold = 0.5
        self.min_scores = 5
        self.eager = False
        self.score_ref = 0.22
        self.band_size = 5
        self.score_mode = ScoreMode.Max
        self.vad_mode = None

    def _c(self):
        c = _DetectorConfig()
        c.avg_threshold, c.threshold, c.min_scores, c.eager = self.avg_threshold, self.threshold, self.min_scores, self.eager
        c.score_ref, c.band_size, c.score_mode = self.score_ref, self.band_size, int(self.score_mode)
        c.vad_mode = int(self.vad_mode) if self.vad_mode is not None else 0
        return c


class RustpotterConfig:
    def __init__(self):
        self.fmt = AudioFmt()
        self.detector = DetectorConfig()
        self.filters = FiltersConfig()

    @staticmethod
    def default():
        return RustpotterConfig()

    def _filters_c(self):
        f = _FiltersCfg()
        g, b = self.filters.gain_normalizer, self.filters.band_pass
        f.gain_normalizer.enabled = g.enabled
        f.gain_normalizer.has_gain_ref = g.gain_ref is not None
        f.gain_normalizer.gain_ref = g.gain_ref if g.gain_ref is not None else 0.0
        f.gain_normalizer.min_gain, f.gain_normalizer.max_gain = g.min_gain, g.max_gain
        f.band_pass.enabled, f.band_pass.low_cutoff, f.band_pass.high_cutoff = b.enabled, b.low_cutoff, b.high_cutoff
        return f

    def _c(self):
        c = _Config()
        c.fmt.sample_rate, c.fmt.sample_format = self.fmt.sample_rate, int(self.fmt.sample_format)
        c.fmt.channels, c.fmt.endianness = self.fmt.channels, int(self.fmt.endianness)
        c.detector = self.detector._c()
        c.filters = self._filters_c()
        return c


class RustpotterDetection:
    def __init__(self, d):
        import numpy as np
        self.name = d.name.decode()
        self.avg_score = np.float32(d.avg_score)
        self.score = np.float32(d.score)
        self.scores = {d.score_names[i].decode(): np.float32(d.scores[i]) for i in range(d.n_scores)}
        self.counter = int(d.counter)
        self.gain = np.float32(d.gain)

    def __repr__(self):
        return "RustpotterDetection(name=%r, avg_score=%r, score=%r, counter=%d)" % (self.name, float(self.avg_score),
                                                                                      float(self.score), self.counter)


class Rustpotter:

    def __init__(self, config):
        self._L = load_library()
        self._h = C.c_void_p()
        c = config._c()
        if self._L.rp_new(C.byref(c), C.byref(self._h)) < 0:
            self._h = None
            raise _err()

    @staticmethod
    def new(config):
        return Rustpotter(config)

    def __del__(self):
        if getattr(self, "_h", None):
            self._L.rp_free(self._h)
            self._h = None

    def add_wakeword_from_file(self, key, path):
        if self._L.rp_add_wakeword_from_file(self._h, key.encode(), path.encode()) < 0:
            raise _err()

    def add_wakeword_from_buffer(self, key, buffer):
        if self._L.rp_add_wakeword_from_buffer(self._h, key.encode(), bytes(buffer), len(buffer)) < 0:
            raise _err()

    def remove_wakeword(self, key):
        return bool(self._L.rp_remove_wakeword(self._h, key.encode()))

    def remove_wakewords(self):
        return bool(self._L.rp_remove_wakewords(self._h))

    def get_samples_per_frame(self):
        return int(self._L.rp_get_samples_per_frame(self._h))

    def get_bytes_per_frame(self):
        return int(self._L.rp_get_bytes_per_frame(self._h))

    def get_partial_detection(self):
        d = _Detection()
        return RustpotterDetection(d) if self._L.rp_get_partial_detection(self._h, C.byref(d)) == 1 else None

    def get_rms_level(self):
        return float(self._L.rp_get_rms_level(self._h))

    def get_gain(self):
        return float(self._L.rp_get_gain(self._h))

    def get_rms_level_ref(self):
        return float(self._L.rp_get_rms_level_ref(self._h))

    def _ret(self, r, d):
        if r < 0:
            raise _err()
        return RustpotterDetection(d) if r == 1 else None

    def process_bytes(self, audio_bytes):
        d = _Detection()
        b = bytes(audio_bytes)
        return self._ret(self._L.rp_process_bytes(self._h, b, len(b), C.byref(d)), d)

    def process_samples(self, samples):
        import numpy as np
        a = np.ascontiguousarray(samples)
        fn = {np.dtype(np.int8): self._L.rp_process_samples_i8, np.dtype(np.int16): self._L.rp_process_samples_i16,
              np.dtype(np.int32): self._L.rp_process_samples_i32, np.dtype(np.float32): self._L.rp_process_samples_f32}[a.dtype]
        d = _Detection()
        return self._ret(fn(self._h, a.ctypes.data, a.size, C.byref(d)), d)

    def update_config(self, config):
        c = config._c()
        self._L.rp_update_config(self._h, C.byref(c))

    def update_detector_config(self, config):
        c = config._c()
        self._L.rp_update_detector_config(self._h, C.byref(c))

    def update_filters_config(self, config):
        rc = RustpotterConfig()
        rc.filters = config
        f = rc._filters_c()
        self._L.rp_update_filters_config(self._h, C.byref(f))

    def reset(self):
        self._L.rp_reset(self._h)


class Templates:

    def __init__(self, ctx, templates, avg=None):
        import numpy as np
        self._L = load_library()
        self.ctx = ctx
        self.T = len(templates)
        self.K = int(np.asarray(templates[0]).shape[1])
        lens = np.array([len(t) for t in templates], np.int32)
        feats = np.concatenate([np.ascontiguousarray(t, np.float32).reshape(-1) for t in templates]).astype(np.float32)
        avg_a = None if avg is None else np.ascontiguousarray(avg, np.float32)
        self._h = C.c_void_p()
        r = self._L.rp_templates_new(ctx._h, self.T, self.K, lens.ctypes.data_as(C.POINTER(C.c_int)),
                                     feats.ctypes.data_as(C.POINTER(C.c_float)), 0 if avg_a is None else avg_a.shape[0],
                                     None if avg_a is None else avg_a.ctypes.data_as(C.POINTER(C.c_float)), C.byref(self._h))
        if r < 0:
            self._h = None
            raise _err()
        self.max_len = int(self._L.rp_templates_max_len(self._h))
        self.has_avg = avg_a is not None

    def __del__(self):
        if getattr(self, "_h", None):
            self._L.rp_templates_free(self._h)
            self._h = None


class Model:

    def __init__(self, ctx, weights, biases):
        import numpy as np
        self._L = load_library()
        self.ctx = ctx
        ws = [np.ascontiguousarray(w, np.float32) for w in weights]
        bs = [np.ascontiguousarray(b, np.float32) for b in biases]
        dims = np.array([ws[0].shape[1]] + [w.shape[0] for w in ws], np.int32)
        fp = C.POINTER(C.c_float)
        wp = (fp * len(ws))(*[w.ctypes.data_as(fp) for w in ws])
        bp = (fp * len(bs))(*[b.ctypes.data_as(fp) for b in bs])
        self._h = C.c_void_p()
        if self._L.rp_model_new(ctx._h, len(ws), dims.ctypes.data_as(C.POINTER(C.c_int)), wp, bp, C.byref(self._h)) < 0:
            self._h = None
            raise _err()
        self.n_in, self.n_out = int(dims[0]), int(dims[-1])

    def __del__(self):
        if getattr(self, "_h", None):
            self._L.rp_model_free(self._h)
            self._h = None


DET_DTYPE = [("stream", "<i4"), ("frame", "<i4"), ("window", "<i4"), ("counter", "<i4"), ("avg_score", "<f4"), ("score", "<f4")]


class StreamBatch:

    def __init__(self, ctx, templates, detector_config, S, max_chunks_per_call=1, sample_rate=16000, channels=1, wakewords=None,
                 mfcc_size=None, filters=None, rms_level_ref=float("nan")):
        self._L = load_library()
        self.ctx, self.templates, self.S, self.max_chunks = ctx, templates, S, max_chunks_per_call
        h = C.c_void_p()
        c = detector_config._c()
        if wakewords is None:
            if self._L.rp_stream_batch_new(ctx._h, templates._h, C.byref(c), S, max_chunks_per_call, C.byref(h)) < 0:
                raise _err()
        else:
            specs = (_WakewordSpec * len(wakewords))()
            self._keep = list(wakewords)
            for sp, w in zip(specs, wakewords):
                sp.templates = w["templates"]._h if w.get("templates") is not None else None
                sp.model = w["model"]._h if w.get("model") is not None else None
                sp.none_index = w.get("none_index", -1)
                sp.precision = {"f32": 0, "bf16": 1}[w.get("precision", "f32")]
                sp.threshold = float("nan") if w.get("threshold") is None else w["threshold"]
                sp.avg_threshold = float("nan") if w.get("avg_threshold") is None else w["avg_threshold"]
            if self._L.rp_stream_batch_new_multi(ctx._h, len(wakewords), specs, mfcc_size, C.byref(c), S, max_chunks_per_call, C.byref(h)) < 0:
                raise _err()
        self._h = h
        if (sample_rate, channels) != (16000, 1) and self._L.rp_stream_batch_set_input(h, sample_rate, channels) < 0:
            raise _err()
        if filters is not None:
            self.set_filters(filters, rms_level_ref)
        self.samples_per_chunk = self._L.rp_stream_batch_samples_per_chunk(h)
        self._last_chunks = 0
        self.frames_per_chunk = resampler_frame_lengths(sample_rate)[1] // 160

    def __del__(self):
        if getattr(self, "_h", None):
            self._L.rp_stream_batch_free(self._h)
            self._h = None

    @property
    def chunks_seen(self):
        return self._L.rp_stream_batch_chunks_seen(self._h)

    def set_input(self, sample_rate, channels=1):
        if self._L.rp_stream_batch_set_input(self._h, sample_rate, channels) < 0:
            raise _err()
        self.samples_per_chunk = self._L.rp_stream_batch_samples_per_chunk(self._h)
        self.frames_per_chunk = resampler_frame_lengths(sample_rate)[1] // 160

    def set_filters(self, filters, rms_level_ref=float("nan")):
        rc = RustpotterConfig()
        rc.filters = filters
        f = rc._filters_c()
        if self._L.rp_stream_batch_set_filters(self._h, C.byref(f), rms_level_ref) < 0:
            raise _err()

    def levels(self):
        import numpy as np
        assert self.ctx.host
        n = max(self._last_chunks, 1)
        rms = np.empty((self.S, n), np.float32)
        gains = np.empty((self.S, n), np.float32)
        if self._L.rp_stream_batch_levels(self._h, rms.ctypes.data, gains.ctypes.data) < 0:
            raise _err()
        return rms, gains

    def process(self, pcm, max_det=4, want_agg=False, n_chunks=None):
        import numpy as np
        assert self.ctx.host
        pcm = np.ascontiguousarray(pcm)
        fmt = {np.dtype(np.int8): 0, np.dtype(np.int16): 1, np.dtype(np.int32): 2}.get(pcm.dtype)
        if fmt is None:
            pcm, fmt = np.ascontiguousarray(pcm, np.float32), 3
        S, N = pcm.shape
        spc = self.samples_per_chunk
        if S != self.S or (n_chunks is None and N % spc) or (n_chunks is not None and n_chunks * spc > N):
            raise ValueError("pcm must be [S][n_chunks*samples_per_chunk]")
        nc = N // spc if n_chunks is None else n_chunks
        det = np.zeros((S, max_det), dtype=DET_DTYPE)
        n_det = np.zeros(S, np.int32)
        agg = np.empty((S, self.frames_per_chunk * nc), np.float32) if want_agg else None
        if self._L.rp_stream_batch_process(self._h, pcm.ctypes.data, fmt, nc, N, det.ctypes.data, n_det.ctypes.data, max_det,
                                           None if agg is None else agg.ctypes.data) < 0:
            raise _err()
        self._last_chunks = nc
        return (det, n_det, agg) if want_agg else (det, n_det)

    def process_multi(self, pcm, max_det=4, n_chunks=None):
        import numpy as np
        assert self.ctx.host
        pcm = np.ascontiguousarray(pcm)
        fmt = {np.dtype(np.int8): 0, np.dtype(np.int16): 1, np.dtype(np.int32): 2}.get(pcm.dtype)
        if fmt is None:
            pcm, fmt = np.ascontiguousarray(pcm, np.float32), 3
        S, N = pcm.shape
        spc = self.samples_per_chunk
        if S != self.S or (n_chunks is None and N % spc) or (n_chunks is not None and n_chunks * spc > N):
            raise ValueError("pcm must be [S][n_chunks*samples_per_chunk]")
        nc = N // spc if n_chunks is None else n_chunks
        det = np.zeros((S, max_det), dtype=DET_DTYPE)
        dww = np.zeros((S, max_det), np.int32)
        dlab = np.zeros((S, max_det), np.int32)
        n_det = np.zeros(S, np.int32)
        if self._L.rp_stream_batch_process_multi(self._h, pcm.ctypes.data, fmt, nc, N, det.ctypes.data, dww.ctypes.data, dlab.ctypes.data,
                                                 n_det.ctypes.data, max_det) < 0:
            raise _err()
        self._last_chunks = nc
        return det, dww, dlab, n_det

    def process_dev(self, pcm_ptr, fmt, n_chunks, stride, det_ptr, n_det_ptr, max_det, agg_ptr=None):
        if self._L.rp_stream_batch_process(self._h, pcm_ptr, fmt, n_chunks, stride, det_ptr, n_det_ptr, max_det, agg_ptr) < 0:
            raise _err()
        self._last_chunks = n_chunks

    def reset(self, stream=-1):
        if self._L.rp_stream_batch_reset(self._h, stream) < 0:
            raise _err()


def batch_detect_sharded(ctxs, templates, pcms, detector_config, max_det=8):
    import numpy as np
    L = load_library()
    n = len(ctxs)
    assert n == len(templates) == len(pcms) and all(c.host for c in ctxs)
    arrs = [np.ascontiguousarray(p) for p in pcms]
    if any(a.ndim != 2 for a in arrs):
        raise ValueError("batch_detect_sharded: every shard must be a 2-D array [streams][samples]")
    N = arrs[0].shape[1]
    if any(a.shape[1] != N or a.dtype != arrs[0].dtype for a in arrs):
        raise ValueError("batch_detect_sharded: all shards must hold streams of the same length and sample type")
    fmt = {np.dtype(np.int8): 0, np.dtype(np.int16): 1, np.dtype(np.int32): 2}.get(arrs[0].dtype)
    if fmt is None:
        arrs, fmt = [np.ascontiguousarray(a, np.float32) for a in arrs], 3
    S = (C.c_size_t * n)(*[a.shape[0] for a in arrs])
    total = sum(a.shape[0] for a in arrs)
    det = np.zeros((total, max_det), dtype=DET_DTYPE)
    n_det = np.zeros(total, np.int32)
    c = detector_config._c()
    hc = (C.c_void_p * n)(*[x._h for x in ctxs])
    ht = (C.c_void_p * n)(*[x._h for x in templates])
    hp = (C.c_void_p * n)(*[a.ctypes.data for a in arrs])
    if L.rp_batch_detect_sharded(hc, ht, n, hp, fmt, S, N, N, C.byref(c), det.ctypes.data, n_det.ctypes.data, max_det) < 0:
        raise _err()
    return det, n_det


def batch_detect_sharded_dev(ctxs, templates, pcm_ptrs, S_list, N, stride, detector_config, det_ptr, n_det_ptr, max_det):
    L = load_library()
    n = len(ctxs)
    if not (n == len(templates) == len(pcm_ptrs) == len(S_list)):
        raise ValueError("batch_detect_sharded_dev: one context, template set, PCM pointer and stream count per shard")
    if any(x.host for x in ctxs):
        raise ValueError("batch_detect_sharded_dev: the contexts must take device pointers (host_pointers=False)")
    c = detector_config._c()
    hc = (C.c_void_p * n)(*[x._h for x in ctxs])
    ht = (C.c_void_p * n)(*[x._h for x in templates])
    hp = (C.c_void_p * n)(*pcm_ptrs)
    S = (C.c_size_t * n)(*S_list)
    if L.rp_batch_detect_sharded(hc, ht, n, hp, 3, S, N, stride, C.byref(c), det_ptr, n_det_ptr, max_det) < 0:
        raise _err()


MLP_PRECISION = {"f32": 0, "bf16": 1, "f32_strict": 2, "f32_fast": 3}


_LIVE_CONTEXTS = weakref.WeakSet()


class arithmetic_all:

    def __init__(self, arithmetic, ragged_matrix=False):
        self.arithmetic, self.ragged = arithmetic, ragged_matrix

    def __enter__(self):
        self.saved = [(c, c.get_arithmetic()) for c in list(_LIVE_CONTEXTS) if getattr(c, "_h", None)]
        for c, _ in self.saved:
            c.set_arithmetic(self.arithmetic, self.ragged)
        return self

    def __exit__(self, *a):
        for c, old in self.saved:
            if getattr(c, "_h", None):
                c.set_arithmetic(*old)


class BatchContext:

    ARITH = {"f32_matrix": 0, "strict_f32": 1, "fast_split": 2}

    def __init__(self, device=0, host_pointers=True, full_scores=False, arithmetic="f32_matrix", ragged_matrix=False):
        self._L = load_library()
        self._h = C.c_void_p()
        self.host = host_pointers
        flags = (1 if host_pointers else 0) | (2 if full_scores else 0) | {0: 0, 1: 4, 2: 8}[self.ARITH[arithmetic]] | (16 if ragged_matrix else 0)
        if self._L.rp_ctx_new(device, flags, C.byref(self._h)) < 0:
            self._h = None
            raise _err()
        _LIVE_CONTEXTS.add(self)

    def set_arithmetic(self, arithmetic, ragged_matrix=False):
        if self._L.rp_ctx_set_arithmetic(self._h, self.ARITH[arithmetic], 1 if ragged_matrix else 0) < 0:
            raise _err()

    def get_arithmetic(self):
        r = C.c_int(0)
        m = int(self._L.rp_ctx_arithmetic(self._h, C.byref(r)))
        return {v: k for k, v in self.ARITH.items()}[m], bool(r.value)

    def arithmetic(self, arithmetic, ragged_matrix=False):
        ctx = self

        class _Scope:
            def __enter__(self):
                self.old = ctx.get_arithmetic()
                ctx.set_arithmetic(arithmetic, ragged_matrix)
                return ctx

            def __exit__(self, *a):
                ctx.set_arithmetic(*self.old)
        return _Scope()

    def __del__(self):
        if getattr(self, "_h", None):
            self._L.rp_ctx_free(self._h)
            self._h = None

    def set_stream(self, hip_stream):
        self._L.rp_ctx_set_stream(self._h, C.c_void_p(hip_stream))

    def synchronize(self):
        if self._L.rp_ctx_synchronize(self._h) < 0:
            raise _err()

    def last_mlp_kernel(self):
        self._L.rp_ctx_last_mlp_kernel.restype = C.c_char_p
        v = self._L.rp_ctx_last_mlp_kernel(self._h)
        return v.decode() if v else ""

    def dtw_ref_pairs(self):
        v = C.c_uint64(0)
        if self._L.rp_ctx_dtw_ref_pairs(self._h, C.byref(v)) < 0:
            raise _err()
        return int(v.value)

    DTW_KERNELS = {1: "dtw_mfma_kernel", 2: "dtw_mfma_wide_kernel", 4: "dtw_ragged_kernel", 8: "register kernels", 16: "dtw_generic_kernel",
                   32: "dtw_single_kernel", 64: "dtw_ref_kernel (every window)", 128: "dtw_mfma_group_kernel"}
    DTW_PRODUCTS = {256: "bf16x3", 512: "f16x2"}

    def dtw_kernels(self):
        m = int(self._L.rp_ctx_dtw_kernels(self._h))
        self.last_dtw_products = [n for b, n in self.DTW_PRODUCTS.items() if m & b]
        return [n for b, n in self.DTW_KERNELS.items() if m & b]

    def mfcc(self, pcm, K):
        import numpy as np
        assert self.host
        pcm = np.ascontiguousarray(pcm)
        fmt = {np.dtype(np.int8): 0, np.dtype(np.int16): 1, np.dtype(np.int32): 2}.get(pcm.dtype)
        if fmt is None:
            pcm, fmt = np.ascontiguousarray(pcm, np.float32), 3
        if pcm.ndim == 1:
            pcm = pcm[None, :]
        S, N = pcm.shape
        nf = mfcc_num_frames(N)
        out = np.empty((S, nf, K), np.float32)
        if self._L.rp_mfcc_batch_fmt(self._h, pcm.ctypes.data, fmt, S, N, N, K, out.ctypes.data) < 0:
            raise _err()
        return out

    def build_wakeword_ref(self, name, samples, mfcc_size, threshold=None, avg_threshold=None, from_files=True):
        names = [k.encode() for k in samples]
        bufs = [bytes(v) for v in samples.values()]
        n = len(names)
        c_names = (C.c_char_p * n)(*names)
        c_bufs = (C.c_char_p * n)(*bufs)
        c_lens = (C.c_size_t * n)(*[len(b) for b in bufs])
        thr = None if threshold is None else C.byref(C.c_float(threshold))
        athr = None if avg_threshold is None else C.byref(C.c_float(avg_threshold))
        out, out_len = C.c_void_p(), C.c_size_t()
        if self._L.rp_wakeword_ref_build(self._h, name.encode(), C.cast(thr, C.POINTER(C.c_float)) if thr else None,
                                         C.cast(athr, C.POINTER(C.c_float)) if athr else None, n, c_names, c_bufs, c_lens,
                                         mfcc_size, 1 if from_files else 0, C.byref(out), C.byref(out_len)) < 0:
            raise _err()
        data = C.string_at(out, out_len.value)
        self._L.rp_buffer_free(out)
        return data

    def train_wakeword_model(self, train, test, m_type="medium", learning_rate=0.027, epochs=10, test_epochs=10, mfcc_size=16,
                             seed=1, prev_model=None):
        def pack(d):
            names = [k.encode() for k in d]
            bufs = [bytes(v) for v in d.values()]
            n = len(names)
            return n, (C.c_char_p * n)(*names), (C.c_char_p * n)(*bufs), (C.c_size_t * n)(*[len(b) for b in bufs])
        ntr, trn, trb, trl = pack(train)
        nte, ten, teb, tel = pack(test)
        opt = _TrainOptions({"tiny": 0, "small": 1, "medium": 2, "large": 3}[m_type], learning_rate, epochs, test_epochs, mfcc_size, seed)
        out, out_len, loss, acc = C.c_void_p(), C.c_size_t(), C.c_float(), C.c_float()
        if self._L.rp_wakeword_model_train(self._h, C.byref(opt), ntr, trn, trb, trl, nte, ten, teb, tel, prev_model,
                                           0 if prev_model is None else len(prev_model), C.byref(out), C.byref(out_len),
                                           C.byref(loss), C.byref(acc)) < 0:
            raise _err()
        data = C.string_at(out, out_len.value)
        self._L.rp_buffer_free(out)
        return data, loss.value, acc.value

    def frontend(self, pcm, filters_config, rms_level_ref, window_size):
        import numpy as np
        assert self.host
        pcm = np.ascontiguousarray(pcm)
        fmt = {np.dtype(np.int8): 0, np.dtype(np.int16): 1, np.dtype(np.int32): 2}.get(pcm.dtype)
        if fmt is None:
            pcm, fmt = np.ascontiguousarray(pcm, np.float32), 3
        if pcm.ndim == 1:
            pcm = pcm[None, :]
        S, N = pcm.shape
        rc = RustpotterConfig()
        rc.filters = filters_config
        f = rc._filters_c()
        out = np.empty((S, N), np.float32)
        rms = np.empty((S, N // 480), np.float32)
        gains = np.empty((S, N // 480), np.float32)
        if self._L.rp_frontend_batch(self._h, pcm.ctypes.data, fmt, S, N, N, C.byref(f), rms_level_ref, window_size,
                                     out.ctypes.data, N, rms.ctypes.data, gains.ctypes.data) < 0:
            raise _err()
        return out, rms, gains

    def dtw_scores(self, mfcc, templates, score_ref=0.22, band_size=5, score_mode=ScoreMode.Max, with_avg=False):
        import numpy as np
        assert self.host
        mfcc = np.ascontiguousarray(mfcc, np.float32)
        if mfcc.ndim == 2:
            mfcc = mfcc[None]
        S, nf, K = mfcc.shape
        assert K == templates.K
        n_win = max(0, nf - templates.max_len + 1)
        scores = np.empty((S, n_win, templates.T), np.float32)
        agg = np.empty((S, n_win), np.float32)
        avg = np.empty((S, n_win), np.float32) if (with_avg and templates.has_avg) else None
        r = self._L.rp_dtw_score_batch(self._h, mfcc.ctypes.data, S, nf, templates._h, score_ref, band_size, int(score_mode),
                                       1 if avg is not None else 0, scores.ctypes.data,
                                       None if avg is None else avg.ctypes.data, agg.ctypes.data)
        if r < 0:
            raise _err()
        return scores, avg, agg

    def detect_scan(self, agg, avg, n_frames, max_len, detector_config, max_det=8, mfcc=None):
        import numpy as np
        assert self.host
        agg = np.ascontiguousarray(agg, np.float32)
        S = agg.shape[0]
        det = np.zeros((S, max_det), dtype=[("stream", "<i4"), ("frame", "<i4"), ("window", "<i4"), ("counter", "<i4"),
                                             ("avg_score", "<f4"), ("score", "<f4")])
        n_det = np.zeros(S, np.int32)
        c = detector_config._c()
        avg_a = None if avg is None else np.ascontiguousarray(avg, np.float32)
        mf = None if mfcc is None else np.ascontiguousarray(mfcc, np.float32)
        r = self._L.rp_detect_scan(self._h, agg.ctypes.data, None if avg_a is None else avg_a.ctypes.data, S, n_frames,
                                   max_len, C.byref(c), 1 if avg_a is not None else 0,
                                   None if mf is None else mf.ctypes.data, 0 if mf is None else mf.shape[-1],
                                   det.ctypes.data, n_det.ctypes.data, max_det)
        if r < 0:
            raise _err()
        return det, n_det

    def batch_detect(self, pcm, templates, detector_config, max_det=8, want_scores=False):
        import numpy as np
        assert self.host
        pcm = np.ascontiguousarray(pcm)
        fmt = {np.dtype(np.int8): 0, np.dtype(np.int16): 1, np.dtype(np.int32): 2}.get(pcm.dtype)
        if fmt is None:
            pcm, fmt = np.ascontiguousarray(pcm, np.float32), 3
        if pcm.ndim == 1:
            pcm = pcm[None, :]
        S, N = pcm.shape
        nf = mfcc_num_frames(N)
        n_win = max(0, nf - templates.max_len + 1)
        det = np.zeros((S, max_det), dtype=[("stream", "<i4"), ("frame", "<i4"), ("window", "<i4"), ("counter", "<i4"),
                                             ("avg_score", "<f4"), ("score", "<f4")])
        n_det = np.zeros(S, np.int32)
        scores = np.empty((S, n_win, templates.T), np.float32) if want_scores else None
        agg = np.empty((S, n_win), np.float32) if want_scores else None
        c = detector_config._c()
        r = self._L.rp_batch_detect_fmt(self._h, pcm.ctypes.data, fmt, S, N, N, templates._h, C.byref(c), det.ctypes.data,
                                        n_det.ctypes.data, max_det, None if scores is None else scores.ctypes.data,
                                        None if agg is None else agg.ctypes.data)
        if r < 0:
            raise _err()
        return (det, n_det, scores, agg) if want_scores else (det, n_det)

    def resample(self, pcm, sample_rate, channels=1):
        import numpy as np
        assert self.host
        pcm = np.ascontiguousarray(pcm)
        fmt = {np.dtype(np.int8): 0, np.dtype(np.int16): 1, np.dtype(np.int32): 2}.get(pcm.dtype)
        if fmt is None:
            pcm, fmt = np.ascontiguousarray(pcm, np.float32), 3
        if pcm.ndim == 1:
            pcm = pcm[None, :]
        S, N = pcm.shape
        n = N // channels
        fi, fo = resampler_frame_lengths(sample_rate)
        n_out = (n // fi) * fo
        out = np.empty((S, n_out), np.float32)
        if self._L.rp_resample_batch(self._h, pcm.ctypes.data, fmt, channels, sample_rate, S, n, N, out.ctypes.data, n_out) < 0:
            raise _err()
        return out

    def resample_dev(self, pcm_ptr, fmt, channels, sample_rate, S, n, stride, out_ptr, out_stride):
        if self._L.rp_resample_batch(self._h, pcm_ptr, fmt, channels, sample_rate, S, n, stride, out_ptr, out_stride) < 0:
            raise _err()

    def batch_detect_multi(self, pcm, templates, detector_config, thresholds=None, avg_thresholds=None, max_det=8):
        import numpy as np
        assert self.host
        pcm = np.ascontiguousarray(pcm)
        fmt = {np.dtype(np.int8): 0, np.dtype(np.int16): 1, np.dtype(np.int32): 2}.get(pcm.dtype)
        if fmt is None:
            pcm, fmt = np.ascontiguousarray(pcm, np.float32), 3
        if pcm.ndim == 1:
            pcm = pcm[None, :]
        S, N = pcm.shape
        n = len(templates)
        hs = (C.c_void_p * n)(*[t._h for t in templates])
        def arr(v):
            if v is None:
                return None
            a = np.array([np.nan if x is None else x for x in v], np.float32)
            return a
        th, ath = arr(thresholds), arr(avg_thresholds)
        det = np.zeros((S, max_det), dtype=DET_DTYPE)
        dww = np.zeros((S, max_det), np.int32)
        n_det = np.zeros(S, np.int32)
        c = detector_config._c()
        fpt = C.POINTER(C.c_float)
        if self._L.rp_batch_detect_multi(self._h, pcm.ctypes.data, fmt, S, N, N, n, hs, C.byref(c),
                                         None if th is None else th.ctypes.data_as(fpt), None if ath is None else ath.ctypes.data_as(fpt),
                                         det.ctypes.data, dww.ctypes.data, n_det.ctypes.data, max_det) < 0:
            raise _err()
        return det, dww, n_det

    def batch_detect_model(self, pcm, model, mfcc_size, none_index, detector_config, precision="f32", max_det=8):
        import numpy as np
        assert self.host
        pcm = np.ascontiguousarray(pcm)
        fmt = {np.dtype(np.int8): 0, np.dtype(np.int16): 1, np.dtype(np.int32): 2}.get(pcm.dtype)
        if fmt is None:
            pcm, fmt = np.ascontiguousarray(pcm, np.float32), 3
        if pcm.ndim == 1:
            pcm = pcm[None, :]
        S, N = pcm.shape
        det = np.zeros((S, max_det), dtype=DET_DTYPE)
        dlab = np.zeros((S, max_det), np.int32)
        n_det = np.zeros(S, np.int32)
        c = detector_config._c()
        if self._L.rp_batch_detect_model(self._h, pcm.ctypes.data, fmt, S, N, N, model._h, mfcc_size, none_index, C.byref(c),
                                         MLP_PRECISION[precision], det.ctypes.data, dlab.ctypes.data, n_det.ctypes.data, max_det) < 0:
            raise _err()
        return det, dlab, n_det

    def batch_detect_dev(self, pcm_ptr, S, N, stride, templates, detector_config, det_ptr, n_det_ptr, max_det,
                         scores_ptr=None, agg_ptr=None):
        c = detector_config._c()
        if self._L.rp_batch_detect(self._h, pcm_ptr, S, N, stride, templates._h, C.byref(c), det_ptr, n_det_ptr, max_det,
                                   scores_ptr, agg_ptr) < 0:
            raise _err()

    def batch_detect_fmt_dev(self, pcm_ptr, fmt, S, N, stride, templates, detector_config, det_ptr, n_det_ptr, max_det,
                             scores_ptr=None, agg_ptr=None):
        c = detector_config._c()
        if self._L.rp_batch_detect_fmt(self._h, pcm_ptr, int(fmt), S, N, stride, templates._h, C.byref(c), det_ptr, n_det_ptr, max_det,
                                       scores_ptr, agg_ptr) < 0:
            raise _err()

    def batch_detect_ingest(self, pcm, templates, detector_config, max_det=8, block_streams=0):
        import numpy as np
        pcm = np.ascontiguousarray(pcm)
        S, N = pcm.shape
        fmt = {np.dtype(np.int8): 0, np.dtype(np.int16): 1, np.dtype(np.int32): 2, np.dtype(np.float32): 3}[pcm.dtype]
        det = np.zeros((S, max_det), dtype=[("stream", "<i4"), ("frame", "<i4"), ("window", "<i4"), ("counter", "<i4"), ("avg_score", "<f4"), ("score", "<f4")])
        n_det = np.zeros((S,), np.int32)
        sec = C.c_double(0.0)
        c = detector_config._c()
        if self._L.rp_batch_detect_ingest(self._h, pcm.ctypes.data, fmt, S, N, N, templates._h, C.byref(c), det.ctypes.data, n_det.ctypes.data, max_det,
                                          block_streams, C.byref(sec)) < 0:
            raise _err()
        return det, n_det, sec.value

    def batch_detect_ingest_ptr(self, pcm_host_ptr, fmt, S, N, stride, templates, detector_config, det_host_ptr, n_det_host_ptr, max_det, block_streams=0):
        sec = C.c_double(0.0)
        c = detector_config._c()
        if self._L.rp_batch_detect_ingest(self._h, pcm_host_ptr, int(fmt), S, N, stride, templates._h, C.byref(c), det_host_ptr, n_det_host_ptr, max_det,
                                          block_streams, C.byref(sec)) < 0:
            raise _err()
        return sec.value

    def mlp_forward(self, x, model, precision="f32"):
        import numpy as np
        assert self.host
        x = np.ascontiguousarray(x, np.float32)
        out = np.empty((x.shape[0], model.n_out), np.float32)
        if self._L.rp_mlp_forward_batch(self._h, model._h, x.ctypes.data, x.shape[0], MLP_PRECISION[precision],
                                        out.ctypes.data) < 0:
            raise _err()
        return out

    def mlp_forward_windows(self, mfcc, model, precision="f32"):
        import numpy as np
        assert self.host
        mfcc = np.ascontiguousarray(mfcc, np.float32)
        S, nf, K = mfcc.shape
        L = model.n_in // K
        n_win = max(nf - L + 1, 0)
        out = np.empty((S, n_win, model.n_out), np.float32)
        if self._L.rp_mlp_forward_windows(self._h, model._h, mfcc.ctypes.data, S, nf, K, MLP_PRECISION[precision], out.ctypes.data) < 0:
            raise _err()
        return out

    def mlp_dev(self, model, x_ptr, B, precision, out_ptr):
        if self._L.rp_mlp_forward_batch(self._h, model._h, x_ptr, B, MLP_PRECISION[precision], out_ptr) < 0:
            raise _err()

    def synth_pcm(self, seed, first_stream, S, N):
        import numpy as np
        assert self.host
        out = np.empty((S, N), np.float32)
        if self._L.rp_synth_pcm_batch(self._h, seed, first_stream, S, N, N, out.ctypes.data) < 0:
            raise _err()
        return out

    def mfcc_dev(self, pcm_ptr, S, N, stride, K, out_ptr):
        if self._L.rp_mfcc_batch(self._h, pcm_ptr, S, N, stride, K, out_ptr) < 0:
            raise _err()

    def dtw_dev(self, mfcc_ptr, S, n_frames, templates, score_ref, band_size, score_mode, with_avg, scores_ptr, avg_ptr, agg_ptr):
        if self._L.rp_dtw_score_batch(self._h, mfcc_ptr, S, n_frames, templates._h, score_ref, band_size, int(score_mode),
                                      int(with_avg), scores_ptr, avg_ptr, agg_ptr) < 0:
            raise _err()

    def scan_dev(self, agg_ptr, avg_ptr, S, n_frames, max_len, detector_config, det_ptr, n_det_ptr, max_det):
        c = detector_config._c()
        if self._L.rp_detect_scan(self._h, agg_ptr, avg_ptr, S, n_frames, max_len, C.byref(c), 1 if avg_ptr else 0, None, 0,
                                  det_ptr, n_det_ptr, max_det) < 0:
            raise _err()

    def synth_dev(self, seed, first_stream, S, N, stride, out_ptr):
        if self._L.rp_synth_pcm_batch(self._h, seed, first_stream, S, N, stride, out_ptr) < 0:
            raise _err()

    def timing_enable(self, on=True):
        self._L.rp_ctx_timing_enable(self._h, 1 if on else 0)

    def timing_reset(self):
        self._L.rp_ctx_timing_reset(self._h)

    def timing_read(self, kernel):
        ms, n = C.c_double(), C.c_int()
        self._L.rp_ctx_timing_read(self._h, kernel, C.byref(ms), C.byref(n))
        return ms.value, n.value
```

### rustpotter_amd/csrc/rp_dtw_mfma.hip

```cpp
#include "rp_device.h"

#include <cstdlib>

namespace rp {

namespace {

typedef unsigned u32x6 __attribute__((ext_vector_type(6)));

constexpr int kMK = 5;
constexpr int kMWin = 32;
constexpr int mfma_slots(int nt) { return nt == 8 ? 12 : 16; }
constexpr int mfma_tiles(int nt) { return nt == 8 ? 3 : 2; }
constexpr int kMSlotsMax = 16;
constexpr int mfma_acc_reg(int nt, int slot, int p, int e) {
    return nt == 8 ? 4 * (slot % 4) + 2 * p + e : 4 * ((slot % 8) >> 1) + 2 * (slot & 1) + e;
}

#ifdef RP_MFMA_CVT_BACK
typedef __fp16 fp16x2 __attribute__((ext_vector_type(2)));
__device__ __forceinline__ float lo_f32(unsigned p) { return (float)__builtin_bit_cast(fp16x2, p)[0]; }
__device__ __forceinline__ float hi_f32(unsigned p) { return (float)__builtin_bit_cast(fp16x2, p)[1]; }
#endif

template <int W, int NT>
__host__ __device__ constexpr int mfma_last_use(int u, int g) {
    int last = -1;
    for (int q = 0; q < 2 * W; ++q)
        if (((u + q + mfma_slots(NT) - W + 2) % mfma_slots(NT)) / (32 / NT) == g) last = q;
    return last;
}

constexpr bool mfma_whole_frame(int nw, bool gx, int nt, bool p3) { return p3 && !(gx && nw == 12 && nt == 8); }

}

#ifdef RP_MFMA_TRACE
#define RP_TRACE(slot)                                                                                                        \
    do {                                                                                                                      \
        if ((threadIdx.x & 63) == 0 && ((threadIdx.x >> 6) == 0 || (threadIdx.x >> 6) == NW - 1) && blockIdx.x < 96)             \
            reinterpret_cast<unsigned long long *>(sched + 1024)[(blockIdx.x * 2 + ((threadIdx.x >> 6) ? 1 : 0)) * 8 + (slot)] = \
                __builtin_amdgcn_s_memrealtime();                                                                             \
    } while (0)
#else
#define RP_TRACE(slot)
#endif

#ifndef RP_MFMA_WAVES_PER_EU
#define RP_MFMA_WAVES_PER_EU 0
#endif
#if RP_MFMA_WAVES_PER_EU
#define RP_MFMA_OCC __attribute__((amdgpu_waves_per_eu(RP_MFMA_WAVES_PER_EU, RP_MFMA_WAVES_PER_EU)))
#else
#define RP_MFMA_OCC
#endif
template <int W, int NW, bool GX, int NT, bool P3>
RP_MFMA_OCC __global__ __launch_bounds__(64 * NW, 1) void dtw_mfma_kernel(
    const float *__restrict__ mfcc, size_t frame_pitch, size_t n_frames_total, size_t total_tiles, unsigned n_chunks, int chunk_base,
    size_t first_win, size_t n_win, size_t out_win_pitch, const DtwChunk *__restrict__ chunks, const uint4 *__restrict__ aimg, int T,
    float score_ref, float *__restrict__ scores, float *__restrict__ avg, size_t n_streams, int max_len, const uint32_t *__restrict__ list,
    const uint32_t *__restrict__ count, uint32_t dense_min, float abandon_nc, uint32_t *__restrict__ sched, unsigned static_rounds,
    float *__restrict__ agg_out, uint32_t *__restrict__ agg_hot, float agg_threshold, uint32_t *__restrict__ fix) {
    constexpr int K = kMK, B = 2 * W, NS = mfma_slots(NT), NTILE = mfma_tiles(NT), SPT = 32 / NT, NP = NT / 4;
    constexpr int kRowBytes = P3 ? kDtwMfma3RowBytes : kDtwMfmaRowBytes;
#ifndef RP_MFMA_GX_PD
    constexpr int PD = GX ? (NS % 3 == 0 ? 3 : 4) : 1;
#else
    constexpr int PD = GX ? RP_MFMA_GX_PD : 1;
#endif
    static_assert(NS % PD == 0, "the frame ring's slot must be a compile-time index");
    constexpr bool WF = mfma_whole_frame(NW, GX, NT, P3);
    constexpr int PP = GX ? 2 : 1;
    static_assert(NS % (2 * PP) == 0, "the pair ring's slot must be a compile-time index");
    static_assert(NT == 8 || NT == 4, "template slots per chunk");
    static_assert(B + 2 <= NS, "the band and its two neighbours must fit the circular row slots");
    size_t total_entries = n_streams * n_win;
    if (list) {
        const uint32_t n_listed = *count;
        if (dense_min && n_listed >= dense_min) return;
        total_entries = n_listed;
        total_tiles = ((size_t)n_listed + kMWin - 1) / kMWin;
    } else if (count && *count < dense_min) return;
    extern __shared__ __attribute__((aligned(16))) unsigned char smem[];
    RP_TRACE(0);
    const unsigned ci = blockIdx.x % n_chunks;
    const unsigned n_groups = gridDim.x / n_chunks;
    const DtwChunk *ch = chunks + chunk_base + ci;
    const int L = ch->len;
    const int a_bytes = (max_len + kMSlotsMax) * kRowBytes;
    const int xs_floats = dtw_mfma_stage_floats(max_len);
    const int tid = threadIdx.x, lane = tid & 63, wave = tid >> 6;
    dtw_load_aimg<64 * NW>(smem, aimg, P3 ? ch->aimg3_off : ch->aimg_off, (L + kMSlotsMax) * kRowBytes / 16, tid);
    __syncthreads();
    RP_TRACE(1);
    float *xs = reinterpret_cast<float *>(smem + a_bytes) + wave * xs_floats;
    (void)xs;
    const int n = lane & 31, h = lane >> 5;
    const int mrow = lane & 31;
    const int jj = NT == 8 ? mrow >> 3 : 2 * (mrow >> 3) + ((mrow >> 1) & 1);
    const int tA = NT == 8 ? ((mrow >> 2) & 1) * 4 + (mrow & 3) : ((mrow >> 2) & 1) * 2 + (mrow & 1);
    const unsigned a_lane = (unsigned)(h * 128 + tA * 16);
    unsigned dl[SPT];
#pragma unroll
    for (int e = 0; e < SPT; ++e) dl[e] = (unsigned)(((e - jj + NS) % NS) * kRowBytes);
    const unsigned sel_one = h ? 0x07060100u : 0x03020100u;
    const unsigned sel_c2 = h ? 0x03020706u : 0x07060302u;
    const unsigned mask_c2 = h ? 0xffff0000u : 0u;
    (void)sel_c2; (void)mask_c2;
    const float abandon_cost = abandon_nc * (float)(L + L);
    bool slot_real[2 * NP], slot_avg[2 * NP];
#pragma unroll
    for (int e = 0; e < 2 * NP; ++e) {
        slot_real[e] = 2 * NP * h + e < ch->count;
        slot_avg[e] = slot_real[e] && ch->tid[2 * NP * h + e] >= T;
    }

    uint32_t *next_tile = sched + 2 * (chunk_base + ci);
    unsigned round = 0;
    const size_t chunk_waves = (size_t)n_groups * NW;
    for (;;) {
        const size_t tile = dtw_next_tile<NW>(next_tile, round, static_rounds, chunk_waves, n_chunks, wave, lane);
        if (tile >= total_tiles) break;
        const size_t f0 = tile * kMWin;
        bool valid;
        size_t s;
        int w;
        const float *xw;
        if (GX) {
            size_t f = f0 + n;
            valid = f < total_entries;
            if (list) f = list[valid ? f : total_entries - 1];
            s = valid ? f / n_win : 0;
            w = valid ? (int)(f - s * n_win) : 0;
            xw = mfcc + (s * frame_pitch + first_win + (size_t)w) * K;
        } else {
            const size_t sA = f0 / n_win;
            const int wA = (int)(f0 - sA * n_win);
            const int nA = (int)n_win - wA < kMWin ? (int)n_win - wA : kMWin;
            const int nB = (nA < kMWin && sA + 1 < n_streams) ? kMWin - nA : 0;
            const int segA = nA + L + 3;
            auto stage =[&](const float *src, size_t g0, int n_floats, float *dst) {
                for (int i0 = lane; i0 < n_floats; i0 += 256) {
                    float v[4];
#pragma unroll
                    for (int j = 0; j < 4; ++j) {
                        const int i = i0 + 64 * j;
                        v[j] = (i < n_floats && g0 + (size_t)(i / K) < n_frames_total) ? src[g0 * K + i] : 0.f;
                    }
#pragma unroll
                    for (int j = 0; j < 4; ++j)
                        if (i0 + 64 * j < n_floats) dst[i0 + 64 * j] = v[j];
                }
            };
            stage(mfcc + sA * frame_pitch * K, first_win + wA, segA * K, xs);
            if (nB > 0) stage(mfcc + (sA + 1) * frame_pitch * K, first_win, (nB + L + 3) * K, xs + segA * K);
            wave_lds_sync();
            const bool inA = n < nA;
            valid = inA || (n - nA < nB);
            s = inA ? sA : sA + 1;
            w = inA ? wA + n : n - nA;
            xw = xs + (inA ? n : (valid ? segA + n - nA : 0)) * K;
        }
        const float *xa = xw + (h ? 3 : 0);
        const float *x2 = xw + 2;
        float mua = 0.f, mub = 0.f, mu2 = 0.f;
#ifndef RP_MFMA_GX_MEAN_UNROLL
#define RP_MFMA_GX_MEAN_UNROLL 20
#endif
#ifndef RP_MFMA_MEAN_UNROLL
#define RP_MFMA_MEAN_UNROLL 8
#endif
        constexpr int kMeanUnroll = GX ? RP_MFMA_GX_MEAN_UNROLL : RP_MFMA_MEAN_UNROLL;
#pragma unroll kMeanUnroll
        for (int i = 0; i < L; ++i) { mua += xa[i * K]; mub += xa[i * K + 1]; mu2 += x2[i * K]; }
        mua = mua / (float)L; mub = mub / (float)L; mu2 = mu2 / (float)L;
        float mu_[K] = {0.f, 0.f, 0.f, 0.f, 0.f};
        (void)mu_;
        if (WF) {
            const auto sa_ = __builtin_amdgcn_permlane32_swap(__float_as_uint(mua), __float_as_uint(mua), false, false);
            const auto sb_ = __builtin_amdgcn_permlane32_swap(__float_as_uint(mub), __float_as_uint(mub), false, false);
            mu_[0] = __uint_as_float(sa_[0]); mu_[3] = __uint_as_float(sa_[1]);
            mu_[1] = __uint_as_float(sb_[0]); mu_[4] = __uint_as_float(sb_[1]);
            mu_[2] = mu2;
        }
        const float *xh = xw + h * K;
        (void)xh;
        if (round == 1) RP_TRACE(2);

        v2f Q[NP][B + 1];
#pragma unroll
        for (int p = 0; p < NP; ++p) {
#pragma unroll
            for (int q = 0; q <= B; ++q) Q[p][q] = (v2f){RP_INF, RP_INF};
            Q[p][W - 1] = (v2f){0.f, 0.f};
        }
        u32x4 Areg[NTILE], Areg2[P3 ? NTILE : 1];
#pragma unroll
        for (int g = 0; g < NTILE; ++g) {
            const int slot = SPT * g + jj;
            int r = W - ((W - slot + NS) % NS);
            r = r < 1 ? 1 : r;
            Areg[g] = *reinterpret_cast<const u32x4 *>(smem + a_lane + (unsigned)(r - 1) * kRowBytes);
            if (P3) Areg2[g] = *reinterpret_cast<const u32x4 *>(smem + a_lane + 256u + (unsigned)(r - 1) * kRowBytes);
        }
        v16f acc[NTILE];
        u32x4 bop[2];
        u32x6 bv[P3 ? 2 : 1];
        (void)bv;

#define RP_P0(cc, rs) fa_[rs] = xa[((cc) - 1) * K]; fb_[rs] = xa[((cc) - 1) * K + 1]; f2_[rs] = x2[((cc) - 1) * K];
#define RP_P1(cc, rs) da_ = fa_[rs] - mua; db_ = fb_[rs] - mub; d2_ = f2_[rs] - mu2;
#define RP_P2(cc) own_ = fmaf(da_, da_, db_ * db_);
#define RP_P3(cc) { const auto sw_ = __builtin_amdgcn_permlane32_swap(__float_as_uint(own_), __float_as_uint(own_), false, false); \
                    bb_ = fmaf(d2_, d2_, __uint_as_float(sw_[0]) + __uint_as_float(sw_[1])); }
#define RP_P4(cc) inv_ = bb_ > 0.f ? __builtin_amdgcn_rsqf(bb_) : 0.f;
#define RP_P5(cc) ua_ = da_ * inv_; ub_ = db_ * inv_; u2_ = d2_ * inv_;
#define RP_HI2(hi, lo) __builtin_amdgcn_perm(__float_as_uint(hi), __float_as_uint(lo), 0x07060302u)
#define RP_AND(x, m) __uint_as_float(__float_as_uint(x) & (m))
#define RP_BSET(par, i, v) bv[par][i] = (v)
#define RP_P6(cc, par) if (P3) { x0a_ = RP_AND(ua_, 0xffff0000u); x0b_ = RP_AND(ub_, 0xffff0000u); x0c_ = RP_AND(u2_, 0xffff0000u); RP_BSET(par, 2, RP_HI2(ub_, ua_)); } \
                       else { bop[par].x = pkrtz(ua_, ub_); bop[par].z = bop[par].x; }
#ifndef RP_MFMA_CVT_BACK
#define RP_X0F(x, packed, hi) x0f(x)
#else
#define RP_X0F(x, packed, hi) ((hi) ? hi_f32(packed) : lo_f32(packed))
#endif
#define RP_P7(cc, par) if (P3) { r1a_ = ua_ - x0a_; r1b_ = ub_ - x0b_; r1c_ = u2_ - x0c_; RP_BSET(par, 3, RP_HI2(r1b_, r1a_)); } \
                       else { bop[par].y = pk_f16_second(ua_ - RP_X0F(ua_, bop[par].x, 0), ub_ - RP_X0F(ub_, bop[par].x, 1)); }
#ifndef RP_AB_NO_RANGE_TEST
#define RP_P8(cc) chk_ = fmaxf(fmaxf(chk_, inv_), bb_);   \
                  if (P3) { x1a_ = RP_AND(r1a_, 0xffff0000u); x1b_ = RP_AND(r1b_, 0xffff0000u); tc_ = RP_AND(r1c_, mask_c2); }
#else
#define RP_P8(cc) if (P3) { x1a_ = RP_AND(r1a_, 0xffff0000u); x1b_ = RP_AND(r1b_, 0xffff0000u); tc_ = RP_AND(r1c_, mask_c2); }
#endif
#define RP_P9(cc, par) if (P3) { RP_BSET(par, 0, RP_HI2(r1b_ - x1b_, r1a_ - x1a_)); RP_BSET(par, 1, __builtin_amdgcn_perm(__float_as_uint(r1c_ - tc_), __float_as_uint(u2_), sel_c2)); } \
                       else { const float x0_ = RP_X0F(u2_, pkrtz(u2_, 0.f), 0);  \
                         bop[par].w = __builtin_amdgcn_perm(0x3c000000u, pk_f16_second(x0_, u2_ - x0_), sel_one); }
#define RP_P10(cc, par) if (P3) { bv[par][4] = bv[par][2]; bv[par][5] = h ? 0x00003f80u : bv[par][1]; }
#define RP_PREP_ALL(cc, par) RP_P0(cc, (cc) % PD) RP_P1(cc, (cc) % PD) RP_P2(cc) RP_P3(cc) RP_P4(cc) RP_P5(cc) RP_P6(cc, par) RP_P7(cc, par) RP_P8(cc) RP_P9(cc, par) RP_P10(cc, par)
#define RP_W_LOAD(cc, rs) g_[rs][0] = xh[((cc) - 1) * K]; g_[rs][1] = xh[((cc) - 1) * K + 1]; g_[rs][2] = xh[((cc) - 1) * K + 2];                 \
                          g_[rs][3] = xh[((cc) - 1) * K + 3]; g_[rs][4] = xh[((cc) - 1) * K + 4];
#define RP_W_NEAR(cc, rs) if (!GX) { RP_W_LOAD(cc, rs) }
#define RP_W_CENTRE(cc, rs) d_[0] = g_[rs][0] - mu_[0]; d_[1] = g_[rs][1] - mu_[1]; d_[2] = g_[rs][2] - mu_[2]; d_[3] = g_[rs][3] - mu_[3];         \
                            d_[4] = g_[rs][4] - mu_[4]; if (GX) { RP_W_LOAD((cc) + 2 * PP, rs) }
#define RP_W_NORM() bb_ = fmaf(d_[2], d_[2], fmaf(d_[0], d_[0], d_[1] * d_[1]) + fmaf(d_[3], d_[3], d_[4] * d_[4]));
#define RP_W_SCALE() w_[0] = d_[0] * inv_; w_[1] = d_[1] * inv_; w_[2] = d_[2] * inv_; w_[3] = d_[3] * inv_; w_[4] = d_[4] * inv_;
#ifndef RP_AB_NO_RANGE_TEST
#define RP_W_CHK(in_window) if (in_window) chk_ = fmaxf(fmaxf(chk_, inv_), bb_);
#else
#define RP_W_CHK(in_window)
#endif
#define RP_W_X0() x0_[0] = RP_AND(w_[0], 0xffff0000u); x0_[1] = RP_AND(w_[1], 0xffff0000u); x0_[2] = RP_AND(w_[2], 0xffff0000u);         \
                  x0_[3] = RP_AND(w_[3], 0xffff0000u); x0_[4] = RP_AND(w_[4], 0xffff0000u);                                              \
                  lo_[2] = RP_HI2(w_[1], w_[0]); up_[2] = RP_HI2(w_[4], w_[3]);
#define RP_W_R1() r_[0] = w_[0] - x0_[0]; r_[1] = w_[1] - x0_[1]; r_[2] = w_[2] - x0_[2]; r_[3] = w_[3] - x0_[3]; r_[4] = w_[4] - x0_[4]; \
                  lo_[3] = RP_HI2(r_[1], r_[0]); up_[3] = RP_HI2(r_[4], r_[3]); lo_[1] = RP_HI2(r_[2], w_[2]);
#define RP_W_X1() y_[0] = RP_AND(r_[0], 0xffff0000u); y_[1] = RP_AND(r_[1], 0xffff0000u); y_[2] = RP_AND(r_[2], 0xffff0000u);            \
                  y_[3] = RP_AND(r_[3], 0xffff0000u); y_[4] = RP_AND(r_[4], 0xffff0000u);
#define RP_W_X2() lo_[0] = RP_HI2(r_[1] - y_[1], r_[0] - y_[0]); up_[0] = RP_HI2(r_[4] - y_[4], r_[3] - y_[3]);                          \
                  up_[1] = __builtin_amdgcn_perm(__float_as_uint(r_[2] - y_[2]), __float_as_uint(w_[2]), 0x03020706u);
#define RP_W_SWAP()                                                                                                           \
    {                                                                                                                         \
        _Pragma("unroll") for (int i = 0; i < 4; ++i) {                                                                       \
            const auto sw_ = __builtin_amdgcn_permlane32_swap(lo_[i], up_[i], false, false);                                  \
            bv[1][i] = sw_[0]; bv[0][i] = sw_[1];                                                                             \
        }                                                                                                                     \
        bv[1][4] = bv[1][2]; bv[1][5] = h ? 0x00003f80u : bv[1][1];                                                           \
        bv[0][4] = bv[0][2]; bv[0][5] = h ? 0x00003f80u : bv[0][1];                                                           \
    }
#define RP_W_FIRST(cc, rs) RP_W_NEAR(cc, rs) RP_W_CENTRE(cc, rs) RP_W_NORM() RP_P4(cc) RP_W_SCALE()
#define RP_W_SECOND(in_window) RP_W_CHK(in_window) RP_W_X0() RP_W_R1() RP_W_X1() RP_W_X2()
#define RP_AREF(cc, uu, GUARD)                                                                                                \
    {                                                                                                                         \
        const int sn = ((uu) + 1 + W) % NS, g = sn / SPT, e = sn % SPT;                                                       \
        int off = ((cc) + W - 1) * kRowBytes - (int)dl[e];                                                                    \
        if (GUARD) off = off < 0 ? 0 : off;                                                                                   \
        Areg[g] = *reinterpret_cast<const u32x4 *>(smem + a_lane + (unsigned)off);                                            \
        if (P3) Areg2[g] = *reinterpret_cast<const u32x4 *>(smem + a_lane + 256u + (unsigned)off);                            \
    }
#define RP_B1(par) __builtin_shufflevector(bv[P3 ? (par) : 0], bv[P3 ? (par) : 0], 0, 1, 2, 3)
#define RP_B2(par) __builtin_shufflevector(bv[P3 ? (par) : 0], bv[P3 ? (par) : 0], 2, 3, 4, 5)
#define RP_MFMA(g, par)                                                                                                       \
    do {                                                                                                                      \
        const v16f zero16 = {0.f, 0.f, 0.f, 0.f, 0.f, 0.f, 0.f, 0.f, 0.f, 0.f, 0.f, 0.f, 0.f, 0.f, 0.f, 0.f};                  \
        if (P3) acc[g] = __builtin_amdgcn_mfma_f32_32x32x16_bf16(__builtin_bit_cast(bf16x8, Areg[g]), __builtin_bit_cast(bf16x8, RP_B1(par)), zero16, 0, 0, 0); \
        else acc[g] = __builtin_amdgcn_mfma_f32_32x32x16_f16(__builtin_bit_cast(f16x8, Areg[g]), __builtin_bit_cast(f16x8, bop[par]), zero16, 0, 0, 0); \
    } while (0)
#define RP_MFMA2(g, par)                                                                                                      \
    do {                                                                                                                      \
        if (P3) acc[g] = __builtin_amdgcn_mfma_f32_32x32x16_bf16(__builtin_bit_cast(bf16x8, Areg2[g]), __builtin_bit_cast(bf16x8, RP_B2(par)), acc[g], 0, 0, 0); \
    } while (0)

#ifndef RP_P3_GAP
#define RP_P3_GAP 1
#endif
#define RP_STEP(GUARD, TAIL)                                                                                                      \
    do {                                                                                                                      \
        RP_AREF(c + 1, (u + 1) % NS, GUARD)                                                                                   \
        v2f up[2] = {(v2f){RP_INF, RP_INF}, (v2f){RP_INF, RP_INF}};                                                           \
        _Pragma("unroll") for (int q = 0; q < B; ++q) {                                                                       \
            const int sl = (u + q + NS - W + 2) % NS;                                                                         \
            _Pragma("unroll") for (int p = 0; p < NP; ++p) {                 \
                const v2f cost = (v2f){acc[sl / SPT][mfma_acc_reg(NT, sl, p, 0)], acc[sl / SPT][mfma_acc_reg(NT, sl, p, 1)]}; \
                v2f m, v;                                                                                                     \
                m.x = fminf(fminf(up[p].x, Q[p][q + 1].x), Q[p][q].x);                                                        \
                m.y = fminf(fminf(up[p].y, Q[p][q + 1].y), Q[p][q].y);                                                        \
                v.x = cost.x + m.x; v.y = cost.y + m.y;  \
                if (GUARD) v = (c - W + 1 + q >= 1) ? v : (v2f){RP_INF, RP_INF};                                              \
                Q[p][q] = v;                                                                                                  \
                up[p] = v;                                                                                                    \
            }                                                                                                                 \
                                                                                              \
            if (WF) {   \
            const int gi = (u & 1) ? q : B + q;                                                                              \
            if (gi == 0) { RP_W_SWAP() RP_W_NEAR(c + 3, ((u + 3) / 2) % PP) }                                                 \
            if (gi == (1 * 2 * B) / 9) { RP_W_CENTRE(c + 3, ((u + 3) / 2) % PP) }                                             \
            if (gi == (2 * 2 * B) / 9) { RP_W_NORM() } if (gi == (3 * 2 * B) / 9) { RP_P4(c + 3) } if (gi == (4 * 2 * B) / 9) { RP_W_SCALE() } \
             \
            if (gi == (5 * 2 * B) / 9) { RP_W_CHK(!(TAIL) || c + h <= L) RP_W_X0() } if (gi == (6 * 2 * B) / 9) { RP_W_R1() }  \
            if (gi == (7 * 2 * B) / 9) { RP_W_X1() } if (gi == (8 * 2 * B) / 9) { RP_W_X2() }                                 \
            } else if (!P3) {                                                                                                 \
            if (q == (0 * B) / 10) { RP_P1(c + 2, (u + 3) % PD) RP_P0(c + 2 + PD, (u + 3) % PD) } if (q == (2 * B) / 10) { RP_P2(c + 2) }                       \
            if (q == (3 * B) / 10) { RP_P3(c + 2) } if (q == (4 * B) / 10) { RP_P4(c + 2) } if (q == (5 * B) / 10) { RP_P5(c + 2) } \
            if (q == (6 * B) / 10) { RP_P6(c + 2, (u + 1) & 1) } if (q == (7 * B) / 10) { RP_P7(c + 2, (u + 1) & 1) }         \
            if (q == (8 * B) / 10) { RP_P8(c + 2) } if (q == (9 * B) / 10) { RP_P9(c + 2, (u + 1) & 1) }                      \
            } else {                             \
            if (q == (0 * B) / 11) { RP_P1(c + 2, (u + 3) % PD) RP_P0(c + 2 + PD, (u + 3) % PD) } if (q == (1 * B) / 11) { RP_P2(c + 2) }                       \
            if (q == (2 * B) / 11) { RP_P3(c + 2) } if (q == (3 * B) / 11) { RP_P4(c + 2) } if (q == (4 * B) / 11) { RP_P5(c + 2) } \
            if (q == (5 * B) / 11) { RP_P6(c + 2, (u + 1) & 1) } if (q == (6 * B) / 11) { RP_P7(c + 2, (u + 1) & 1) }         \
            if (q == (7 * B) / 11) { RP_P8(c + 2) } if (q == (8 * B) / 11) { RP_P9(c + 2, (u + 1) & 1) }                      \
            if (q == (9 * B) / 11) { RP_P10(c + 2, (u + 1) & 1) }                                                             \
            }                                                                                                                 \
            _Pragma("unroll") for (int g = 0; g < NTILE; ++g) {                                                               \
                if (mfma_last_use<W, NT>(u, g) == q) RP_MFMA(g, u & 1);                                                       \
                if (q >= RP_P3_GAP && mfma_last_use<W, NT>(u, g) == q - RP_P3_GAP) RP_MFMA2(g, u & 1);                        \
            }                                                                                                                 \
            __builtin_amdgcn_sched_barrier(0);                                                                                \
        }                                                                                                                     \
        _Pragma("unroll") for (int g = 0; g < NTILE; ++g) {                                                                   \
            if (mfma_last_use<W, NT>(u, g) < 0) { RP_MFMA(g, u & 1); RP_MFMA2(g, u & 1); }                                    \
            else if (RP_P3_GAP > 0 && mfma_last_use<W, NT>(u, g) > B - 1 - RP_P3_GAP) RP_MFMA2(g, u & 1);                     \
        }                                                                                                                     \
    } while (0)

        float fa_[PD], fb_[PD], f2_[PD], da_, db_, d2_, own_, bb_, inv_, ua_, ub_, u2_, chk_ = 0.f;
        float x0a_ = 0.f, x0b_ = 0.f, x0c_ = 0.f, r1a_ = 0.f, r1b_ = 0.f, r1c_ = 0.f, x1a_ = 0.f, x1b_ = 0.f, tc_ = 0.f;
        (void)x0a_; (void)x0b_; (void)x0c_; (void)r1a_; (void)r1b_; (void)r1c_; (void)x1a_; (void)x1b_; (void)tc_;
        float g_[PP][K], d_[K], w_[K], x0_[K], r_[K], y_[K];
        unsigned lo_[4], up_[4];
        (void)g_; (void)d_; (void)w_; (void)x0_; (void)r_; (void)y_; (void)lo_; (void)up_; (void)da_; (void)db_; (void)d2_; (void)own_; (void)ua_; (void)ub_; (void)u2_;
        RP_AREF(1, 0, true)
        if (WF) {
            if (GX) { RP_W_LOAD(1, 0) RP_W_LOAD(3, 1 % PP) }
            RP_W_FIRST(1, 0) RP_W_SECOND(true) RP_W_SWAP()
        }
        else { RP_PREP_ALL(1, 1) }
        RP_MFMA(0, 1); RP_MFMA(1, 1);
        if (NTILE > 2) RP_MFMA(NTILE - 1, 1);
        RP_MFMA2(0, 1); RP_MFMA2(1, 1);
        if (NTILE > 2) RP_MFMA2(NTILE - 1, 1);
        if (WF) { RP_W_FIRST(3, 1 % PP) }
        else {
            RP_PREP_ALL(2, 0)
#pragma unroll
            for (int a = 0; a < PD; ++a) { RP_P0(3 + a, (3 + a) % PD) }
        }
        __builtin_amdgcn_sched_barrier(0);
        int c0 = 1;
        bool dead = false;
        {
#pragma unroll
            for (int u = 0; u < NS; ++u) { const int c = c0 + u; RP_STEP(true, false); }
        }
#ifdef RP_MFMA_PRICE_NO_ABANDON
#define RP_ABANDON_ON false
#else
#define RP_ABANDON_ON (abandon_nc < RP_INF)
#endif
#define RP_ABANDON_CHECK()                                                                                                    \
    if (RP_ABANDON_ON) {                                                                                                \
        bool alive = false;                                                                                                   \
        _Pragma("unroll") for (int p = 0; p < NP; ++p) {                                                                      \
            v2f m = Q[p][0];                                                                                                  \
            _Pragma("unroll") for (int q = 1; q < B; ++q) m = (v2f){fminf(m.x, Q[p][q].x), fminf(m.y, Q[p][q].y)};             \
            alive = alive || (slot_real[2 * p] && (m.x <= abandon_cost || slot_avg[2 * p])) ||                                \
                    (slot_real[2 * p + 1] && (m.y <= abandon_cost || slot_avg[2 * p + 1]));                                   \
        }                                                                                                                     \
        if (!__any(alive && valid)) dead = true;                                                                              \
    }
        for (c0 = 1 + NS; c0 + NS - 1 <= L; c0 += NS) {
            RP_ABANDON_CHECK()
            if (dead) break;
#pragma unroll
            for (int u = 0; u < NS; ++u) { const int c = c0 + u; RP_STEP(false, false); }
        }
        if (!dead && c0 <= L) {
            RP_ABANDON_CHECK()
            if (!dead) {
#pragma unroll
                for (int u = 0; u < NS - 1; ++u) {
                    const int c = c0 + u;
                    if (c <= L) RP_STEP(false, true);
                }
            }
        }
#undef RP_ABANDON_CHECK
#undef RP_ABANDON_ON
#undef RP_STEP
#undef RP_MFMA
#undef RP_MFMA2
#undef RP_P10
#undef RP_W_LOAD
#undef RP_W_NEAR
#undef RP_W_CENTRE
#undef RP_W_NORM
#undef RP_W_SCALE
#undef RP_W_CHK
#undef RP_W_X0
#undef RP_W_R1
#undef RP_W_X1
#undef RP_W_X2
#undef RP_W_SWAP
#undef RP_W_FIRST
#undef RP_W_SECOND
#undef RP_HI2
#undef RP_AND
#undef RP_BSET
#undef RP_B1
#undef RP_B2
#undef RP_AREF
#undef RP_PREP_ALL
#undef RP_P0
#undef RP_P1
#undef RP_P2
#undef RP_P3
#undef RP_P4
#undef RP_P5
#undef RP_P6
#undef RP_P7
#undef RP_P8
#undef RP_P9
#undef RP_X0F

        if (round == 1) RP_TRACE(3);
        if (WF) {
            const auto sw_ = __builtin_amdgcn_permlane32_swap(__float_as_uint(chk_), __float_as_uint(chk_), false, false);
            chk_ = fmaxf(__uint_as_float(sw_[0]), __uint_as_float(sw_[1]));
        }
        float best = 0.f;
        if (valid) {
            const size_t row = s * out_win_pitch + (size_t)w;
            const float denom = (float)(L + L);
#pragma unroll
            for (int p = 0; p < NP; ++p) {
#pragma unroll
                for (int e = 0; e < 2; ++e) {
                    const int slot = 2 * NP * h + 2 * p + e;
                    if (slot < ch->count) {
                        const float cost = e ? Q[p][W - 2].y : Q[p][W - 2].x;
                        const float nc = cost / denom;
                        const float sc = dead ? 0.f : dtw_logistic(nc, score_ref);
                        const int t = ch->tid[slot];
                        if (t < T) { scores[row * T + t] = sc; best = fmaxf(best, sc); }
                        else if (!dead) avg[row] = sc;
                    }
                }
            }
            if (h == 0 && chk_ > kDtwFixLimit) dtw_fix_append(fix, row, (uint32_t)(chunk_base + (int)ci));
        }
        if (agg_out) {
            const auto sw_ = __builtin_amdgcn_permlane32_swap(__float_as_uint(best), __float_as_uint(best), false, false);
            const float m = fmaxf(__uint_as_float(sw_[0]), __uint_as_float(sw_[1]));
            if (valid && h == 0) {
                agg_out[s * out_win_pitch + (size_t)w] = m;
                if (agg_hot && m > agg_threshold) agg_hot[s] = 1u;
            }
        }
        if (!GX) wave_lds_sync();
        if (round == 1) RP_TRACE(4);
    }
    RP_TRACE(5);
    __syncthreads();
    RP_TRACE(6);
    dtw_release_tiles(next_tile, n_groups, tid);
}

bool dtw_mfma_supported(const TemplatesDev &t, int band, size_t n_win, bool from_global, int slots, float score_ref) {
    const int mode = t.arith_mode();
    if (mode == kArithStrictF32 || t.K != kMK || !(mode == kArithFastSplit ? t.aimg : t.aimg3) || t.max_diff != 0) return false;
    const bool p3 = mode != kArithFastSplit;
    if (!p3 && !(score_ref >= kDtwMfmaMinScoreRef)) return false;
    if (slots == 8 ? (band < 3 || band > 5) : band != 5) return false;
    if (!from_global && n_win < (size_t)kMWin) return false;
    if (slots == 8 ? t.mfma_min_len < mfma_slots(8) : t.mfma_min_len4 < mfma_slots(4)) return false;
    return dtw_mfma_lds_bytes(t.max_len, 8, p3 ? kDtwMfma3RowBytes : kDtwMfmaRowBytes) <= 160 * 1024;
}

hipError_t launch_dtw_mfma(const DtwCall &c, int slots, int chunk_base, int n_chunks, bool from_global, const GateList &gate) {
    const TemplatesDev &t = *c.t;
    const DtwWork &wk = c.wk;
    const DtwFusedAgg *fuse = gate.fuse;
    if (n_chunks <= 0 || c.S == 0 || c.n_win == 0) return hipSuccess;
    const bool p3 = t.arith_mode() != kArithFastSplit;
    dtw_mark(wk, kDtwRanMfma | (p3 ? kDtwRanBf16x3 : kDtwRanF16x2));
    if (fuse && (n_chunks != 1 || gate.list || gate.count)) return hipErrorInvalidValue;
    float *agg_out = fuse ? fuse->agg : nullptr;
    uint32_t *agg_hot = fuse ? fuse->hot : nullptr;
    const float agg_threshold = fuse ? fuse->threshold : 0.f;
    if (gate.list && !from_global) return hipErrorNotSupported;
    const size_t total_tiles = (c.S * c.n_win + kMWin - 1) / kMWin;
    const int row_bytes = p3 ? kDtwMfma3RowBytes : kDtwMfmaRowBytes;
    int nw = dtw_mfma_lds_bytes(t.max_len, 12, row_bytes) <= 160 * 1024 ? 12 : 8;
    if (p3 && slots == 8) {
        static const int env_nw = [] { const char *e = std::getenv("RP_MFMA3_WAVES"); return e ? std::atoi(e) : 0; }();
        if (env_nw != 12) nw = 8;
    }
    const size_t lds = dtw_mfma_lds_bytes(t.max_len, nw, row_bytes);
    const void *image = p3 ? t.aimg3 : t.aimg;
    if (!wk.sched || !wk.fix) return hipErrorInvalidValue;
    unsigned blocks, static_rounds;
    if (hipError_t e = mfma_grid(total_tiles, n_chunks, nw, gate.list != nullptr, blocks, static_rounds); e != hipSuccess) return e;
#define RP_LAUNCH_MFMA_P(WW, NW, GXV, NT, PP)                                                                                       \
    do {                                                                                                                            \
        if (hipError_t e = allow_dynamic_lds(reinterpret_cast<const void *>(dtw_mfma_kernel<WW, NW, GXV, NT, PP>), 160 * 1024); e != hipSuccess) return e; \
        hipLaunchKernelGGL((dtw_mfma_kernel<WW, NW, GXV, NT, PP>), dim3(blocks), dim3(64 * NW), lds, c.st, c.mfcc, c.frame_pitch, c.frame_pitch, \
                           total_tiles, (unsigned)n_chunks, chunk_base, c.first_win, c.n_win, c.out_win_pitch, t.chunks,             \
                           reinterpret_cast<const uint4 *>(image), t.T, c.score_ref, c.scores, c.avg, c.S, t.max_len, gate.list, gate.count, \
                           gate.dense_min, gate.abandon_nc, wk.sched, static_rounds, agg_out, agg_hot, agg_threshold, wk.fix);      \
    } while (0)
#define RP_LAUNCH_MFMA(WW, NW, GXV, NT)                                                                                             \
    do {                                                                                                                            \
        if (p3) RP_LAUNCH_MFMA_P(WW, NW, GXV, NT, true); else RP_LAUNCH_MFMA_P(WW, NW, GXV, NT, false);                             \
    } while (0)
#define RP_LAUNCH_MFMA_W(WW, NT)                                                                                                    \
    do {                                                                                                                            \
        if (from_global) { if (nw == 12) RP_LAUNCH_MFMA(WW, 12, true, NT); else RP_LAUNCH_MFMA(WW, 8, true, NT); }                  \
        else { if (nw == 12) RP_LAUNCH_MFMA(WW, 12, false, NT); else RP_LAUNCH_MFMA(WW, 8, false, NT); }                            \
    } while (0)
    if (slots == 4) {
        if (c.band != 5) return hipErrorNotSupported;
        RP_LAUNCH_MFMA_W(5, 4);
    } else {
        switch (c.band) {
        case 3: RP_LAUNCH_MFMA_W(3, 8); break;
        case 4: RP_LAUNCH_MFMA_W(4, 8); break;
        case 5: RP_LAUNCH_MFMA_W(5, 8); break;
        default: return hipErrorNotSupported;
        }
    }
#undef RP_LAUNCH_MFMA_W
#undef RP_LAUNCH_MFMA
#undef RP_LAUNCH_MFMA_P
    return hipGetLastError();
}

}
```

### rustpotter_amd/csrc/rp_kernels.h

```cpp
#pragma once
#include <cstdlib>
#include <hip/hip_runtime.h>
#include <stddef.h>
#include <stdint.h>

namespace rp {

constexpr int kFrame = 480;
constexpr int kShift = 160;
constexpr int kBins = 240;

template <int K1T> struct MelCentres;
template <> struct MelCentres<6> { static constexpr int c[8] = {0, 9, 22, 41, 68, 106, 161, 240}; };
template <> struct MelCentres<14> { static constexpr int c[16] = {0, 4, 8, 14, 20, 28, 37, 47, 60, 74, 92, 112, 137, 166, 200, 240}; };
template <> struct MelCentres<17> {
    static constexpr int c[19] = {0, 3, 7, 11, 16, 21, 28, 35, 43, 53, 64, 77, 92, 109, 128, 150, 176, 206, 240};
};
template <int K1T> __host__ __device__ constexpr bool mel_touches(int f, int k2, bool mirror) {
    if (f < 0 || f >= K1T) return false;
    const int lo = MelCentres<K1T>::c[f] + 1, hi = MelCentres<K1T>::c[f + 2] - 1;
    const int g_lo = mirror ? 240 - (16 * k2 + 15) : 16 * k2;
    const int g_hi = mirror ? 240 - 16 * k2 : 16 * k2 + 15;
    return g_hi >= lo && g_lo <= hi;
}

template <int K1T> __host__ __device__ constexpr int mel_index(int f, int k2, bool mirror) {
    int n = 0;
    for (int ff = 0; ff < K1T; ++ff)
        for (int kk = 0; kk < 8; ++kk) {
            if (ff == f && kk == k2 && !mirror) return n;
            if (mel_touches<K1T>(ff, kk, false)) ++n;
            if (ff == f && kk == k2 && mirror) return n;
            if (mel_touches<K1T>(ff, kk, true)) ++n;
        }
    return n;
}
template <int K1T> constexpr int kMelEntries = mel_index<K1T>(K1T, 0, false);
template <int K1T> constexpr int kMelRowPitch = ((kMelEntries<K1T> + 3) / 4) * 4 + (((kMelEntries<K1T> + 3) / 4) % 2 == 0 ? 4 : 0);
static_assert(kMelEntries<6> == 31 && kMelRowPitch<6> == 36 && kMelEntries<17> == 41 && kMelRowPitch<17> == 44, "mel table shape");

struct MfccTablesDev {
    int K1 = 0;
    bool mel_sparse = false;
    float *hamming = nullptr;
    float2 *tw240 = nullptr;
    float2 *tw480 = nullptr;
    float *fb = nullptr;
    float *melw = nullptr;
    float *dct = nullptr;
};

constexpr int kChunkMax = 8;
struct DtwChunk {
    int len;
    int count;
    int tc;
    int rows_off;
    int tid[kChunkMax];
    int aimg_off;
    int aimg3_off;
};

constexpr int kDtwMfmaRowBytes = 256;
constexpr int kDtwMfma3RowBytes = 512;
__host__ __device__ inline int dtw_mfma_stage_floats(int max_len) { return ((32 + 2 * (max_len + 3)) * 5 + 3) & ~3; }
__host__ __device__ constexpr int dtw_mfma_wide_chm(int K) { return (K + 1) / 2; }
__host__ __device__ constexpr int dtw_mfma_wide_ksteps(int K) {
    return (3 * (dtw_mfma_wide_chm(K) / 2) + (dtw_mfma_wide_chm(K) % 2 ? 2 : 0) + 3) / 4;
}
__host__ __device__ constexpr int dtw_mfma_wide_row_bytes(int K) { return dtw_mfma_wide_ksteps(K) * 256 + 128; }
constexpr int kDtwWide3KSteps = 6;
constexpr int kDtwWide3RowBytes = kDtwWide3KSteps * 128 + 64;
struct W3Slot { int c0, p0, c1, p1; };
__host__ __device__ constexpr W3Slot dtw_mfma_wide3_slot(int K, int ks, int i) {
    constexpr int pair16[6][4] = {{0, 1, 0, 1}, {0, 1, 0, 1}, {0, 1, 2, 3}, {0, 1, 2, 3}, {2, 3, 2, 3}, {2, 3, 2, 3}};
    constexpr int part16[6][4] = {{0, 0, 0, 0}, {1, 1, 0, 0}, {1, 1, 0, 0}, {2, 2, 1, 1}, {2, 2, 0, 0}, {1, 1, 0, 0}};
    constexpr W3Slot s13[6][4] = {
        {{0, 0, 1, 0}, {2, 0, 3, 0}, {0, 0, 1, 0}, {2, 0, 3, 0}},
        {{0, 1, 1, 1}, {2, 1, 3, 1}, {0, 0, 1, 0}, {2, 0, 3, 0}},
        {{0, 1, 1, 1}, {2, 1, 3, 1}, {4, 0, 5, 0}, {6, 0, 6, 0}},
        {{0, 2, 1, 2}, {2, 2, 3, 2}, {4, 1, 5, 1}, {6, 1, 6, 1}},
        {{4, 2, 5, 2}, {6, 2, -1, 0}, {4, 0, 5, 0}, {6, 0, -2, 0}},
        {{4, 1, 5, 1}, {-1, 0, -1, 0}, {4, 0, 5, 0}, {-1, 0, -1, 0}}};
    return K == 16 ? W3Slot{2 * pair16[ks][i], part16[ks][i], 2 * pair16[ks][i] + 1, part16[ks][i]} : s13[ks][i];
}
inline unsigned mfma_static_rounds(size_t total_tiles, size_t chunk_waves, bool list) {
    const size_t r = chunk_waves ? total_tiles / chunk_waves : 0;
    if (const char *e = std::getenv("RP_MFMA_STATIC_ROUNDS")) return (unsigned)std::atoi(e);
    return (list || r > 3 || r < 1) ? 1u : (unsigned)r;
}
int device_cu_count();
inline hipError_t mfma_grid(size_t total_tiles, int n_chunks, int waves, bool list, unsigned &blocks, unsigned &static_rounds) {
    size_t groups = (size_t)device_cu_count() / (size_t)n_chunks;
    if (groups < 1) groups = 1;
    const size_t need = (total_tiles + waves - 1) / waves;
    if (groups > need) groups = need;
    if (groups * (size_t)n_chunks > 0x7fffffffULL) return hipErrorInvalidValue;
    blocks = (unsigned)(groups * (size_t)n_chunks);
    static_rounds = mfma_static_rounds(total_tiles, groups * (size_t)waves, list);
    return hipSuccess;
}
inline size_t dtw_mfma_lds_bytes(int max_len, int waves, int row_bytes = kDtwMfmaRowBytes) {
    return (size_t)(max_len + 16) * (size_t)row_bytes + (size_t)waves * (size_t)dtw_mfma_stage_floats(max_len) * sizeof(float);
}

enum { kArithF32Matrix = 0, kArithStrictF32 = 1, kArithFastSplit = 2 };
struct DtwArith {
    int mode = kArithF32Matrix;
    int ragged = 0;
};

struct TemplatesDev {
    const DtwArith *arith = nullptr;
    int arith_mode() const { return arith ? arith->mode : (int)kArithF32Matrix; }
    bool arith_ragged() const { return arith && arith->mode == kArithFastSplit && arith->ragged; }
    int T = 0;
    int K = 0;
    int Lpad = 0;
    int has_avg = 0;
    int max_len = 0;
    int max_diff = 0;
    int *lens = nullptr;
    float *unit = nullptr;
    DtwChunk *chunks = nullptr;
    float *dup = nullptr;
    int class_first[4] = {0, 0, 0, 0};
    int class_count[4] = {0, 0, 0, 0};
    int split_first = 0, split_count = 0;
    void *aimg = nullptr;
    void *aimg3 = nullptr;
    int mfma_min_len = 0;
    int mfma_min_len4 = 0;
    int wide8_first = 0, wide8_count = 0;
    int wide4_first = 0, wide4_count = 0, wide4_min_len = 0;
    int n_chunks_total = 0;
    float *raw = nullptr;
    int ref_only = 0;
    int *grp_first = nullptr;
    int grp_count = 0, grp4_max_len = 0;
    int rest_runs = 0, rest_first[8] = {0, 0, 0, 0, 0, 0, 0, 0}, rest_count[8] = {0, 0, 0, 0, 0, 0, 0, 0};
    int rag_first = 0, rag_count = 0;
    int rag_min_len = 0;
    int rag_a_cap = 0;
    int rag_rows_cap = 0;
    void *rimg = nullptr;
    int *rag_off = nullptr;
};
constexpr float kDtwNormLo = 8.673617379884035e-19f, kDtwNormHiRow = 1.152921504606847e18f, kDtwFixLimit = 1073741824.f;

constexpr int kDtwSchedChunks = 2048;
constexpr uint32_t kDtwFixCap = 1u << 18;
constexpr uint32_t kFixSpecTemplate = 1u << 22, kFixSpecAll = 1u << 23, kFixSpecMask = (1u << 24) - 1;
struct DtwWork {
    uint32_t *sched = nullptr;
    uint32_t *fix = nullptr;
    uint32_t *ran = nullptr;
    float *rag_prep = nullptr;
    uint32_t *rag_list = nullptr;
    size_t rag_streams = 0, rag_rows = 0;
};
enum : uint32_t { kDtwRanMfma = 1u, kDtwRanMfmaWide = 2u, kDtwRanRagged = 4u, kDtwRanRegister = 8u, kDtwRanGeneric = 16u, kDtwRanSingle = 32u, kDtwRanRefAll = 64u, kDtwRanMfmaGroup = 128u,
                  kDtwRanBf16x3 = 256u, kDtwRanF16x2 = 512u };
inline void dtw_mark(const DtwWork &wk, uint32_t bit) { if (wk.ran) *wk.ran |= bit; }
__host__ __device__ inline unsigned long long *dtw_fix_stats(uint32_t *fix) { return reinterpret_cast<unsigned long long *>(fix + 2 + 2 * (size_t)kDtwFixCap); }

struct DtwFusedAgg {
    float *agg = nullptr;
    uint32_t *hot = nullptr;
    float threshold = 0.f;
    bool done = false;
};

struct GateList {
    const uint32_t *list = nullptr, *count = nullptr;
    uint32_t dense_min = 0;
    uint32_t list_mult = 1;
    float abandon_nc = __builtin_inff();
    const DtwFusedAgg *fuse = nullptr;
    uint32_t *fix = nullptr;
};

struct DtwCall {
    hipStream_t st = nullptr;
    DtwWork wk;
    const TemplatesDev *t = nullptr;
    const float *mfcc = nullptr;
    size_t S = 0, frame_pitch = 0, first_win = 0, n_win = 0, out_win_pitch = 0;
    int band = 0;
    float score_ref = 0.f;
    float *scores = nullptr, *avg = nullptr;
    bool padded_rows = false;
};

constexpr float kDtwMfmaMinScoreRef = 0.05f;
bool dtw_mfma_supported(const TemplatesDev &t, int band, size_t n_win, bool from_global, int slots, float score_ref);
hipError_t launch_dtw_mfma(const DtwCall &c, int slots, int chunk_base, int n_chunks, bool from_global, const GateList &gate);
bool dtw_mfma_wide_supported(const TemplatesDev &t, int band, float score_ref);
hipError_t launch_dtw_mfma_wide(const DtwCall &c, const GateList &gate);
bool dtw_mfma_wide3_supported(const TemplatesDev &t, int band);
hipError_t launch_dtw_mfma_wide3(const DtwCall &c, const GateList &gate);
size_t dtw_mfma_group_lds_bytes(int L, int sh);
bool dtw_mfma_group_supported(const TemplatesDev &t, int band, size_t n_win, size_t S, float score_ref);
hipError_t launch_dtw_mfma_group(const DtwCall &c);

constexpr int kDtwRaggedWaves = 8;
constexpr int kDtwRaggedSegs = 16;
constexpr float kDtwRaggedMinScoreRef = 0.1f;
bool dtw_ragged_supported(const TemplatesDev &t, int band, size_t n_win, float score_ref);
size_t dtw_ragged_lds_bytes(const TemplatesDev &t, size_t n_win, int *frames_cap);
hipError_t launch_dtw_ragged(const DtwCall &c, float abandon_nc, bool list_rows);

hipError_t allow_dynamic_lds(const void *kernel, int bytes);

enum KernelId { kKernelMfcc = 0, kKernelDtw = 1, kKernelAggregate = 2, kKernelScan = 3, kKernelMlp = 4, kKernelResample = 5, kKernelCount = 6 };

struct ResamplerDev {
    int fs_in = 0, fi = 0, fo = 0, kpad = 0;
    const float *g2t = nullptr;
    const float *fft48 = nullptr;
};

constexpr int kR48OffTw240 = 0, kR48OffTw480 = 240, kR48OffTwc = 480, kR48OffW960c = 480 + 6 * 480, kR48OffHf = kR48OffW960c + 256,
              kR48TableLen = kR48OffHf + 480;

struct ScanConfig {
    float threshold, avg_threshold;
    int min_scores, eager, max_len, avg_enabled;
    int fpf = 3;
    int stream_base = 0;
};

constexpr int kScanMaxWakewords = 8;
struct ScanWakewords {
    int n;
    const float *agg[kScanMaxWakewords], *avg[kScanMaxWakewords];
    float threshold[kScanMaxWakewords], avg_threshold[kScanMaxWakewords];
    const int32_t *label[kScanMaxWakewords];
    uint32_t *hot = nullptr;
};

struct BatchDetection {
    int32_t stream, frame, window, counter;
    float avg_score, score;
};

hipError_t launch_mfcc(hipStream_t st, const MfccTablesDev &tb, const float *pcm, size_t S, size_t n_samples,
                       size_t pcm_stride, size_t first_frame, size_t n_frames, size_t out_frame_pitch, float *mfcc,
                       float *mfcc2 = nullptr);

hipError_t launch_mfcc_stream(hipStream_t st, const MfccTablesDev &tb, const void *pcm, int fmt, size_t S, size_t n_chunks,
                              size_t pcm_stride, const float *hist, size_t hist_pitch, float *hist_out, size_t out_frame_pitch,
                              float *mfcc);
hipError_t launch_mfcc_fmt(hipStream_t st, const MfccTablesDev &tb, const void *pcm, int fmt, size_t S, size_t n_samples,
                           size_t pcm_stride, size_t first_frame, size_t n_frames, size_t out_frame_pitch, float *mfcc);

struct Ctx;
struct DtwScore {
    const TemplatesDev *t = nullptr;
    const float *mfcc = nullptr;
    size_t S = 0, frame_pitch = 0, first_win = 0, n_win = 0;
    int band = 0;
    float score_ref = 0.f;
    bool with_avg = false;
    bool detect_only = false;
    float avg_threshold = 0.f, threshold = 0.f;
    int score_mode = 0;
    float *scores = nullptr, *avg = nullptr, *agg = nullptr;
    uint32_t *hot = nullptr, *gate_list = nullptr;
    bool gate_generic = false;
    bool gate_one_stream = true;
    bool fuse_max = false;
    bool ragged = false;
    bool padded_rows = true;
    bool timed = true;
};
bool dtw_score(Ctx &c, const DtwScore &q);

hipError_t launch_dtw_single_part(hipStream_t st, const DtwWork &wk, const TemplatesDev &t, const float *mfcc, size_t frame_pitch, size_t first_win, size_t n_win,
                                  size_t out_win_pitch, int band, float score_ref, int t_first, int t_count, float *scores, float *avg);

int dtw_register_tile(int K, int band);

struct AggExtra {
    const float *gate_avg = nullptr;
    float gate_threshold = 0.f;
    uint32_t *hot = nullptr;
    float threshold = 0.f;
    size_t n_win = 1;
};
hipError_t launch_aggregate(hipStream_t st, const float *scores, size_t n_rows, int T, int mode, float *agg, AggExtra x = AggExtra{});

hipError_t launch_vad_value(hipStream_t st, const float *mfcc, size_t n_frames_total, int K, float *out);
hipError_t launch_vad_value_rows(hipStream_t st, const float *mfcc, size_t S, size_t n, size_t pitch, int K, float *out);
hipError_t launch_scan_multi(hipStream_t st, const ScanWakewords &ww, const float *vad_value, float vad_mode_value, size_t S,
                             size_t n_frames, const ScanConfig &cfg, BatchDetection *det, int32_t *det_ww, int32_t *n_det, int max_det);
hipError_t launch_scan(hipStream_t st, const float *agg, const float *avg, const float *vad_value, float vad_mode_value,
                       size_t S, size_t n_frames, const ScanConfig &cfg, BatchDetection *det, int32_t *n_det, int max_det,
                       uint32_t *hot = nullptr);

hipError_t launch_frontend(hipStream_t st, const void *pcm, int fmt, size_t S, size_t n_samples, size_t pcm_stride, int gain_on,
                           float rms_level_ref, float min_gain, float max_gain, int window_size, int band_pass, float a0,
                           float a1, float a2, float b1, float b2, float *ring, float *rms, float *gains, float *out,
                           size_t out_stride);
hipError_t launch_chunk_rms(hipStream_t st, const void *pcm, int fmt, size_t S, size_t n_chunks, size_t pcm_stride, float *rms);
hipError_t launch_stream_filters(hipStream_t st, const void *pcm, int fmt, int channels, size_t S, size_t n_chunks, size_t pcm_stride,
                                 const float *old_hist, size_t old_off, float *hist, size_t hist_pitch, int gain_on,
                                 float rms_level_ref, float min_gain, float max_gain, int window_size, int band_pass, float a0,
                                 float a1, float a2, float b1, float b2, float *filter_state, float *rms, float *gains);
size_t stream_filter_state_bytes(size_t S, int window_size);
constexpr size_t kStreamFiltersMaxPitch = (size_t)1 << 25;

hipError_t launch_resample_stage(hipStream_t st, const void *pcm, int fmt, int channels, size_t S, size_t n_chunks, int fi,
                                 size_t pcm_stride, const float *prev, float *xs);
hipError_t launch_resample48(hipStream_t st, const float *tables, const void *pcm, int fmt, int channels, size_t pcm_stride,
                             int has_hist, const float *prev, float *prev_out, size_t S, size_t n_chunks, float *out,
                             size_t out_stride);
bool resample_reads_in_place(const ResamplerDev &rs, const void *pcm, int fmt, size_t pcm_stride, const float *out, size_t out_stride);
hipError_t launch_resample_in_place(hipStream_t st, const ResamplerDev &rs, const void *pcm, int fmt, int channels, size_t pcm_stride,
                                    const float *prev, float *prev_out, size_t S, size_t n_chunks, float *out, size_t out_stride);
hipError_t launch_resample(hipStream_t st, const ResamplerDev &rs, const float *xs, size_t S, size_t n_chunks, float *out,
                           size_t out_stride);

hipError_t launch_stream_stage(hipStream_t st, const void *pcm, int fmt, int channels, size_t S, size_t n_new, size_t pcm_stride,
                               const float *old_hist, size_t old_off, float *hist, size_t hist_pitch);
hipError_t launch_carry_rows(hipStream_t st, const float *src, size_t S, size_t src_pitch, size_t src_off, size_t count, float *dst,
                             size_t dst_pitch);
hipError_t launch_stream_state_init(hipStream_t st, void *state, size_t S);
size_t stream_state_bytes();
hipError_t launch_stream_state_reset(hipStream_t st, void *state, size_t S, long long stream, long long resume);
hipError_t launch_scan_stream_multi(hipStream_t st, const ScanWakewords &ww, const float *vad_value, float vad_mode_value, size_t S,
                                    long long f0, int n_new, const ScanConfig &cfg, void *state, BatchDetection *det, int32_t *det_ww,
                                    int32_t *det_label, int32_t *n_det, int max_det);

hipError_t launch_synth(hipStream_t st, uint64_t seed, uint64_t first_stream, size_t S, size_t n_samples,
                        size_t pcm_stride, float *pcm);

hipError_t launch_normalize_windows(hipStream_t st, const float *mfcc, size_t first_win, size_t n_win, int L, int K,
                                    float *x);

struct MlpDev {
    int n_layers = 0;
    int dims[5] = {0, 0, 0, 0, 0};
    int nt = 0;
    int kpad = 0;
    float *w1f = nullptr;
    void *w1h = nullptr;
    void *w1s = nullptr;
    void *w1t = nullptr;
    void *wwin = nullptr;
    void *wwin3 = nullptr;
    float *b1 = nullptr;
    float *tail = nullptr;
    int tail_floats = 0;
};
enum { kMlpF32 = 0, kMlpBf16 = 1, kMlpF16x2 = 2, kMlpBf16x3 = 5 };
bool mlp_mfma_fits(const MlpDev &m);
struct MlpStreamPlan {
    const void *wimg = nullptr;
    int q[2] = {0, 0};
    int units = 0;
    int par = 0;
    int nbt = 0;
};
bool mlp_stream_supported(const MlpDev &m, const float *x, int precision);
hipError_t launch_mlp_stream(hipStream_t st, const MlpDev &m, const MlpStreamPlan &p, const float *x, size_t B, int precision, float *out,
                             int n_cu, uint32_t *redo);
hipError_t launch_window_means(hipStream_t st, const float *mfcc, size_t S, size_t n_frames, size_t n_win, int L, int K, float *mean);

struct Model;
struct MlpForward {
    Model *m = nullptr;
    int precision = 0;
    const float *x = nullptr;
    size_t B = 0, S = 0, n_win = 0, frame_pitch = 0;
    bool windows = false;
    int K = 0;
    const float *mean = nullptr, *wsum = nullptr;
    float *out = nullptr;
    float *scratch[2] = {nullptr, nullptr};
    bool allow_stream = true;
    bool report = true;
    bool timed = true;
};
bool mlp_forward(Ctx &c, const MlpForward &q);

hipError_t launch_train_forward(hipStream_t st, const float *x, size_t B, int n_layers, const int *dims, float *const *W,
                                float *const *Bv, float *const *act);
hipError_t launch_train_step(hipStream_t st, const float *x, const int32_t *labels, size_t B, int n_layers, const int *dims,
                             float *const *W, float *const *Bv, float *const *act, float *const *dz, float lr, float *loss_rows);
hipError_t launch_normalize_windows_batch(hipStream_t st, const float *mfcc, size_t frame_pitch, size_t n_win, size_t first_row,
                                          size_t n_rows, int L, int K, float *x);
hipError_t launch_nn_score(hipStream_t st, const float *logits, size_t n_rows, int n_labels, int none_index, float score_ref10,
                           int calc_avg, float threshold, float avg_threshold, float *agg, float *avg, int32_t *label,
                           uint32_t *hot = nullptr, size_t rows_per_stream = 0);

}
```

Before: 902.3 million scorings/s.

## Default to 12-wave bf16x3 MFMA DTW with register-pressure controls and late A2 loads

Lane-derived constants are now rematerialised per tile and per loop instead of being kept live, using asm barriers, readfirstlane and a fresh lane-id helper. Second-pass A operands are loaded late in the 12-wave local-staging bf16x3 path. A separate abandon-enabled kernel instantiation lets the common path drop the early-abandon code. Together these let the bf16x3 8-slot path use 12 waves by default when not reading from global memory and not abandoning. They aim to cut register pressure enough for higher occupancy, at the cost of extra recomputed instructions, a risk of spills, and one more kernel instantiation.

```diff
diff --git a/bindings/rustpotter_hip.rs b/bindings/rustpotter_hip.rs
--- a/bindings/rustpotter_hip.rs
+++ b/bindings/rustpotter_hip.rs
@@ -51,6 +51,8 @@
 pub const RP_DTW_KERNEL_MFMA_GROUP: c_int = 128;
 pub const RP_DTW_PRODUCTS_BF16X3: c_int = 256;
 pub const RP_DTW_PRODUCTS_F16X2: c_int = 512;
+pub const RP_DTW_MFMA_WAVES_8: c_int = 1024;
+pub const RP_DTW_MFMA_WAVES_12: c_int = 2048;
 pub const RP_MLP_F32: c_int = 0;
 pub const RP_MLP_BF16: c_int = 1;
 pub const RP_MLP_F32_STRICT: c_int = 2;
diff --git a/include/rustpotter_hip.h b/include/rustpotter_hip.h
--- a/include/rustpotter_hip.h
+++ b/include/rustpotter_hip.h
@@ -130,7 +130,9 @@
     RP_DTW_KERNEL_REF_ALL = 64,
     RP_DTW_KERNEL_MFMA_GROUP = 128,
     RP_DTW_PRODUCTS_BF16X3 = 256,
-    RP_DTW_PRODUCTS_F16X2 = 512
+    RP_DTW_PRODUCTS_F16X2 = 512,
+    RP_DTW_MFMA_WAVES_8 = 1024,
+    RP_DTW_MFMA_WAVES_12 = 2048
 };
 int rp_ctx_dtw_kernels(rp_ctx *ctx);
 const char *rp_build_info(void);
diff --git a/rustpotter_amd/api.py b/rustpotter_amd/api.py
--- a/rustpotter_amd/api.py
+++ b/rustpotter_amd/api.py
@@ -727,10 +727,12 @@
     DTW_KERNELS = {1: "dtw_mfma_kernel", 2: "dtw_mfma_wide_kernel", 4: "dtw_ragged_kernel", 8: "register kernels", 16: "dtw_generic_kernel",
                    32: "dtw_single_kernel", 64: "dtw_ref_kernel (every window)", 128: "dtw_mfma_group_kernel"}
     DTW_PRODUCTS = {256: "bf16x3", 512: "f16x2"}
+    DTW_MFMA_WAVES = {1024: 8, 2048: 12}
 
     def dtw_kernels(self):
         m = int(self._L.rp_ctx_dtw_kernels(self._h))
         self.last_dtw_products = [n for b, n in self.DTW_PRODUCTS.items() if m & b]
+        self.last_dtw_mfma_waves = [n for b, n in self.DTW_MFMA_WAVES.items() if m & b]
         return [n for b, n in self.DTW_KERNELS.items() if m & b]
 
     def mfcc(self, pcm, K):
diff --git a/rustpotter_amd/csrc/rp_dtw_mfma.hip b/rustpotter_amd/csrc/rp_dtw_mfma.hip
--- a/rustpotter_amd/csrc/rp_dtw_mfma.hip
+++ b/rustpotter_amd/csrc/rp_dtw_mfma.hip
@@ -7,6 +7,19 @@
 namespace {
 
 typedef unsigned u32x6 __attribute__((ext_vector_type(6)));
+
+__device__ __forceinline__ int fresh_lane_id() {
+    unsigned ones = ~0u;
+    asm volatile("" : "+s"(ones));
+    return (int)__builtin_amdgcn_mbcnt_hi(ones, __builtin_amdgcn_mbcnt_lo(ones, 0u));
+}
+template <class T> __device__ __forceinline__ T not_hoisted(T v) {
+    asm volatile("" : "+s"(v));
+    return v;
+}
+__device__ __forceinline__ size_t wave_uniform(size_t v) {
+    return ((size_t)__builtin_amdgcn_readfirstlane((unsigned)(v >> 32)) << 32) | (size_t)__builtin_amdgcn_readfirstlane((unsigned)v);
+}
 
 constexpr int kMK = 5;
 constexpr int kMWin = 32;
@@ -32,6 +45,15 @@
 }
 
 constexpr bool mfma_whole_frame(int nw, bool gx, int nt, bool p3) { return p3 && !(gx && nw == 12 && nt == 8); }
+constexpr bool mfma_late_a2(int nw, bool gx, int nt, bool p3) { return p3 && nw == 12 && nt == 8 && !gx; }
+template <int W, int NT>
+__host__ __device__ constexpr int mfma_a2_request(int u, int g) {
+    const int lu = mfma_last_use<W, NT>(u, g);
+    return lu < 0 ? 2 * W - 2 : (lu < 1 ? 0 : lu - 1);
+}
+constexpr int mfma_a2_back(int sn, int g, int nt) { return sn - (32 / nt) * g < 0 ? sn - (32 / nt) * g + mfma_slots(nt) : sn - (32 / nt) * g; }
+
+constexpr bool mfma_abandon_apart(int nw, bool gx, int nt, bool p3) { return nw == 12 && mfma_whole_frame(nw, gx, nt, p3); }
 
 }
 
@@ -54,13 +76,17 @@
 #else
 #define RP_MFMA_OCC
 #endif
-template <int W, int NW, bool GX, int NT, bool P3>
-RP_MFMA_OCC __global__ __launch_bounds__(64 * NW, 1) void dtw_mfma_kernel(
-    const float *__restrict__ mfcc, size_t frame_pitch, size_t n_frames_total, size_t total_tiles, unsigned n_chunks, int chunk_base,
-    size_t first_win, size_t n_win, size_t out_win_pitch, const DtwChunk *__restrict__ chunks, const uint4 *__restrict__ aimg, int T,
-    float score_ref, float *__restrict__ scores, float *__restrict__ avg, size_t n_streams, int max_len, const uint32_t *__restrict__ list,
-    const uint32_t *__restrict__ count, uint32_t dense_min, float abandon_nc, uint32_t *__restrict__ sched, unsigned static_rounds,
-    float *__restrict__ agg_out, uint32_t *__restrict__ agg_hot, float agg_threshold, uint32_t *__restrict__ fix) {
+#define RP_MFMA_PARAMS                                                                                                                       \
+    const float *__restrict__ mfcc, size_t frame_pitch, size_t n_frames_total, size_t total_tiles, unsigned n_chunks, int chunk_base,        \
+    size_t first_win, size_t n_win, size_t out_win_pitch, const DtwChunk *__restrict__ chunks, const uint4 *__restrict__ aimg, int T,        \
+    float score_ref, float *__restrict__ scores, float *__restrict__ avg, size_t n_streams, int max_len, const uint32_t *__restrict__ list, \
+    const uint32_t *__restrict__ count, uint32_t dense_min, float abandon_nc, uint32_t *__restrict__ sched, unsigned static_rounds,         \
+    float *__restrict__ agg_out, uint32_t *__restrict__ agg_hot, float agg_threshold, uint32_t *__restrict__ fix
+#define RP_MFMA_ARGS                                                                                                                         \
+    mfcc, frame_pitch, n_frames_total, total_tiles, n_chunks, chunk_base, first_win, n_win, out_win_pitch, chunks, aimg, T, score_ref,      \
+    scores, avg, n_streams, max_len, list, count, dense_min, abandon_nc, sched, static_rounds, agg_out, agg_hot, agg_threshold, fix
+template <int W, int NW, bool GX, int NT, bool P3, bool AB>
+__device__ __forceinline__ void dtw_mfma_body(RP_MFMA_PARAMS) {
     constexpr int K = kMK, B = 2 * W, NS = mfma_slots(NT), NTILE = mfma_tiles(NT), SPT = 32 / NT, NP = NT / 4;
     constexpr int kRowBytes = P3 ? kDtwMfma3RowBytes : kDtwMfmaRowBytes;
 #ifndef RP_MFMA_GX_PD
@@ -71,6 +97,7 @@
     static_assert(NS % PD == 0, "the frame ring's slot must be a compile-time index");
     constexpr bool WF = mfma_whole_frame(NW, GX, NT, P3);
     constexpr int PP = GX ? 2 : 1;
+    constexpr bool A2L = mfma_late_a2(NW, GX, NT, P3);
     static_assert(NS % (2 * PP) == 0, "the pair ring's slot must be a compile-time index");
     static_assert(NT == 8 || NT == 4, "template slots per chunk");
     static_assert(B + 2 <= NS, "the band and its two neighbours must fit the circular row slots");
@@ -89,58 +116,58 @@
     const int L = ch->len;
     const int a_bytes = (max_len + kMSlotsMax) * kRowBytes;
     const int xs_floats = dtw_mfma_stage_floats(max_len);
-    const int tid = threadIdx.x, lane = tid & 63, wave = tid >> 6;
+    const int tid = threadIdx.x, wave = __builtin_amdgcn_readfirstlane(tid >> 6);
     dtw_load_aimg<64 * NW>(smem, aimg, P3 ? ch->aimg3_off : ch->aimg_off, (L + kMSlotsMax) * kRowBytes / 16, tid);
     __syncthreads();
     RP_TRACE(1);
     float *xs = reinterpret_cast<float *>(smem + a_bytes) + wave * xs_floats;
     (void)xs;
-    const int n = lane & 31, h = lane >> 5;
-    const int mrow = lane & 31;
-    const int jj = NT == 8 ? mrow >> 3 : 2 * (mrow >> 3) + ((mrow >> 1) & 1);
-    const int tA = NT == 8 ? ((mrow >> 2) & 1) * 4 + (mrow & 3) : ((mrow >> 2) & 1) * 2 + (mrow & 1);
-    const unsigned a_lane = (unsigned)(h * 128 + tA * 16);
-    unsigned dl[SPT];
-#pragma unroll
-    for (int e = 0; e < SPT; ++e) dl[e] = (unsigned)(((e - jj + NS) % NS) * kRowBytes);
-    const unsigned sel_one = h ? 0x07060100u : 0x03020100u;
-    const unsigned sel_c2 = h ? 0x03020706u : 0x07060302u;
-    const unsigned mask_c2 = h ? 0xffff0000u : 0u;
-    (void)sel_c2; (void)mask_c2;
+    const int hAb = fresh_lane_id() >> 5;
     const float abandon_cost = abandon_nc * (float)(L + L);
     bool slot_real[2 * NP], slot_avg[2 * NP];
 #pragma unroll
     for (int e = 0; e < 2 * NP; ++e) {
-        slot_real[e] = 2 * NP * h + e < ch->count;
-        slot_avg[e] = slot_real[e] && ch->tid[2 * NP * h + e] >= T;
+        slot_real[e] = 2 * NP * hAb + e < ch->count;
+        slot_avg[e] = slot_real[e] && ch->tid[2 * NP * hAb + e] >= T;
     }
 
     uint32_t *next_tile = sched + 2 * (chunk_base + ci);
     unsigned round = 0;
     const size_t chunk_waves = (size_t)n_groups * NW;
     for (;;) {
-        const size_t tile = dtw_next_tile<NW>(next_tile, round, static_rounds, chunk_waves, n_chunks, wave, lane);
-        if (tile >= total_tiles) break;
+        const size_t tile = wave_uniform(dtw_next_tile<NW>(next_tile, round, static_rounds, chunk_waves, n_chunks, wave, fresh_lane_id()));
+        if (tile >= not_hoisted(total_tiles)) break;
+        const int lane_ = fresh_lane_id();
+        const int n = lane_ & 31, h = lane_ >> 5;
         const size_t f0 = tile * kMWin;
-        bool valid;
-        size_t s;
-        int w;
+        const size_t n_win_ = not_hoisted(n_win);
+        const size_t sA = GX ? 0 : f0 / n_win_;
+        const int wA = GX ? 0 : (int)(f0 - sA * n_win_);
+        const int nA = (int)n_win_ - wA < kMWin ? (int)n_win_ - wA : kMWin;
+        const int nB = (nA < kMWin && sA + 1 < n_streams) ? kMWin - nA : 0;
+        const int segA = nA + L + 3;
+        auto locate = [&](int n_, size_t &s_, int &w_) -> bool {
+            if (GX) {
+                size_t f = f0 + n_;
+                const bool valid_ = f < total_entries;
+                if (list) f = list[valid_ ? f : total_entries - 1];
+                s_ = valid_ ? f / n_win_ : 0;
+                w_ = valid_ ? (int)(f - s_ * n_win_) : 0;
+                return valid_;
+            }
+            const bool inA = n_ < nA;
+            s_ = inA ? sA : sA + 1;
+            w_ = inA ? wA + n_ : n_ - nA;
+            return inA || (n_ - nA < nB);
+        };
         const float *xw;
-        if (GX) {
-            size_t f = f0 + n;
-            valid = f < total_entries;
-            if (list) f = list[valid ? f : total_entries - 1];
-            s = valid ? f / n_win : 0;
-            w = valid ? (int)(f - s * n_win) : 0;
-            xw = mfcc + (s * frame_pitch + first_win + (size_t)w) * K;
-        } else {
-            const size_t sA = f0 / n_win;
-            const int wA = (int)(f0 - sA * n_win);
-            const int nA = (int)n_win - wA < kMWin ? (int)n_win - wA : kMWin;
-            const int nB = (nA < kMWin && sA + 1 < n_streams) ? kMWin - nA : 0;
-            const int segA = nA + L + 3;
+        size_t s_gx;
+        int w_gx;
+        const bool valid = locate(n, s_gx, w_gx);
+        if (GX) xw = mfcc + (s_gx * frame_pitch + first_win + (size_t)w_gx) * K;
+        if (!GX) {
             auto stage =[&](const float *src, size_t g0, int n_floats, float *dst) {
-                for (int i0 = lane; i0 < n_floats; i0 += 256) {
+                for (int i0 = lane_; i0 < n_floats; i0 += 256) {
                     float v[4];
 #pragma unroll
                     for (int j = 0; j < 4; ++j) {
@@ -155,11 +182,7 @@
             stage(mfcc + sA * frame_pitch * K, first_win + wA, segA * K, xs);
             if (nB > 0) stage(mfcc + (sA + 1) * frame_pitch * K, first_win, (nB + L + 3) * K, xs + segA * K);
             wave_lds_sync();
-            const bool inA = n < nA;
-            valid = inA || (n - nA < nB);
-            s = inA ? sA : sA + 1;
-            w = inA ? wA + n : n - nA;
-            xw = xs + (inA ? n : (valid ? segA + n - nA : 0)) * K;
+            xw = xs + (n < nA ? n : (valid ? segA + n - nA : 0)) * K;
         }
         const float *xa = xw + (h ? 3 : 0);
         const float *x2 = xw + 2;
@@ -173,7 +196,8 @@
         constexpr int kMeanUnroll = GX ? RP_MFMA_GX_MEAN_UNROLL : RP_MFMA_MEAN_UNROLL;
 #pragma unroll kMeanUnroll
         for (int i = 0; i < L; ++i) { mua += xa[i * K]; mub += xa[i * K + 1]; mu2 += x2[i * K]; }
-        mua = mua / (float)L; mub = mub / (float)L; mu2 = mu2 / (float)L;
+        const float fL = (float)not_hoisted(L);
+        mua = mua / fL; mub = mub / fL; mu2 = mu2 / fL;
         float mu_[K] = {0.f, 0.f, 0.f, 0.f, 0.f};
         (void)mu_;
         if (WF) {
@@ -185,6 +209,22 @@
         }
         const float *xh = xw + h * K;
         (void)xh;
+#define RP_LANE_CONSTS()                                                                                                      \
+        const int laneA_ = fresh_lane_id();                                                                                   \
+        const int hA = laneA_ >> 5;                                                                                           \
+        const bool upper = hA != 0;                                                                                           \
+        const int mrow = laneA_ & 31;                                                                                         \
+        const int jj = NT == 8 ? mrow >> 3 : 2 * (mrow >> 3) + ((mrow >> 1) & 1);                                             \
+        const int tA = NT == 8 ? ((mrow >> 2) & 1) * 4 + (mrow & 3) : ((mrow >> 2) & 1) * 2 + (mrow & 1);                     \
+        const unsigned a_lane = (unsigned)(hA * 128 + tA * 16);                                                               \
+        const unsigned a2_lane = a_lane + 256u + (unsigned)jj * kRowBytes;   \
+        unsigned dl[SPT];                                                                                                     \
+        _Pragma("unroll") for (int e = 0; e < SPT; ++e) dl[e] = (unsigned)(((e - jj + NS) % NS) * kRowBytes);                 \
+        const unsigned sel_one = upper ? 0x07060100u : 0x03020100u;   \
+        const unsigned sel_c2 = upper ? 0x03020706u : 0x07060302u;                                                            \
+        const unsigned mask_c2 = upper ? 0xffff0000u : 0u;                                                                    \
+        (void)a2_lane; (void)dl; (void)sel_one; (void)sel_c2; (void)mask_c2;
+        RP_LANE_CONSTS()
         if (round == 1) RP_TRACE(2);
 
         v2f Q[NP][B + 1];
@@ -236,7 +276,7 @@
 #define RP_P9(cc, par) if (P3) { RP_BSET(par, 0, RP_HI2(r1b_ - x1b_, r1a_ - x1a_)); RP_BSET(par, 1, __builtin_amdgcn_perm(__float_as_uint(r1c_ - tc_), __float_as_uint(u2_), sel_c2)); } \
                        else { const float x0_ = RP_X0F(u2_, pkrtz(u2_, 0.f), 0);  \
                          bop[par].w = __builtin_amdgcn_perm(0x3c000000u, pk_f16_second(x0_, u2_ - x0_), sel_one); }
-#define RP_P10(cc, par) if (P3) { bv[par][4] = bv[par][2]; bv[par][5] = h ? 0x00003f80u : bv[par][1]; }
+#define RP_P10(cc, par) if (P3) { bv[par][4] = bv[par][2]; bv[par][5] = upper ? 0x00003f80u : bv[par][1]; }
 #define RP_PREP_ALL(cc, par) RP_P0(cc, (cc) % PD) RP_P1(cc, (cc) % PD) RP_P2(cc) RP_P3(cc) RP_P4(cc) RP_P5(cc) RP_P6(cc, par) RP_P7(cc, par) RP_P8(cc) RP_P9(cc, par) RP_P10(cc, par)
 #define RP_W_LOAD(cc, rs) g_[rs][0] = xh[((cc) - 1) * K]; g_[rs][1] = xh[((cc) - 1) * K + 1]; g_[rs][2] = xh[((cc) - 1) * K + 2];                 \
                           g_[rs][3] = xh[((cc) - 1) * K + 3]; g_[rs][4] = xh[((cc) - 1) * K + 4];
@@ -265,8 +305,8 @@
             const auto sw_ = __builtin_amdgcn_permlane32_swap(lo_[i], up_[i], false, false);                                  \
             bv[1][i] = sw_[0]; bv[0][i] = sw_[1];                                                                             \
         }                                                                                                                     \
-        bv[1][4] = bv[1][2]; bv[1][5] = h ? 0x00003f80u : bv[1][1];                                                           \
-        bv[0][4] = bv[0][2]; bv[0][5] = h ? 0x00003f80u : bv[0][1];                                                           \
+        bv[1][4] = bv[1][2]; bv[1][5] = upper ? 0x00003f80u : bv[1][1];                                                           \
+        bv[0][4] = bv[0][2]; bv[0][5] = upper ? 0x00003f80u : bv[0][1];                                                           \
     }
 #define RP_W_FIRST(cc, rs) RP_W_NEAR(cc, rs) RP_W_CENTRE(cc, rs) RP_W_NORM() RP_P4(cc) RP_W_SCALE()
 #define RP_W_SECOND(in_window) RP_W_CHK(in_window) RP_W_X0() RP_W_R1() RP_W_X1() RP_W_X2()
@@ -286,10 +326,18 @@
         if (P3) acc[g] = __builtin_amdgcn_mfma_f32_32x32x16_bf16(__builtin_bit_cast(bf16x8, Areg[g]), __builtin_bit_cast(bf16x8, RP_B1(par)), zero16, 0, 0, 0); \
         else acc[g] = __builtin_amdgcn_mfma_f32_32x32x16_f16(__builtin_bit_cast(f16x8, Areg[g]), __builtin_bit_cast(f16x8, bop[par]), zero16, 0, 0, 0); \
     } while (0)
-#define RP_MFMA2(g, par)                                                                                                      \
+#define RP_MFMA2X(g, par, A2)                                                                                                 \
     do {                                                                                                                      \
-        if (P3) acc[g] = __builtin_amdgcn_mfma_f32_32x32x16_bf16(__builtin_bit_cast(bf16x8, Areg2[g]), __builtin_bit_cast(bf16x8, RP_B2(par)), acc[g], 0, 0, 0); \
+        if (P3) acc[g] = __builtin_amdgcn_mfma_f32_32x32x16_bf16(__builtin_bit_cast(bf16x8, A2), __builtin_bit_cast(bf16x8, RP_B2(par)), acc[g], 0, 0, 0); \
     } while (0)
+#define RP_MFMA2(g, par) RP_MFMA2X(g, par, Areg2[g])
+#define RP_A2_LATE(g, GUARD)                                                                                                  \
+    {                                                                                                                         \
+        int off = (c + W - mfma_a2_back((u + 2 + W) % NS, g, NT)) * kRowBytes;                                                \
+        if (GUARD) off = off + (int)(jj * kRowBytes) < 0 ? -(int)(jj * kRowBytes) : off;                                      \
+        a2l[g] = *reinterpret_cast<const u32x4 *>(smem + a2_lane + off);                                                      \
+    }
+#define RP_MFMA2S(g, par) do { if (A2L && g != gn_) RP_MFMA2X(g, par, a2l[g]); else RP_MFMA2(g, par); } while (0)
 
 #ifndef RP_P3_GAP
 #define RP_P3_GAP 1
@@ -298,6 +346,9 @@
     do {                                                                                                                      \
         RP_AREF(c + 1, (u + 1) % NS, GUARD)                                                                                   \
         v2f up[2] = {(v2f){RP_INF, RP_INF}, (v2f){RP_INF, RP_INF}};                                                           \
+        const int gn_ = ((u + 2 + W) % NS) / SPT;                                      \
+        u32x4 a2l[NTILE];                                                                                                     \
+        (void)gn_; (void)a2l;                                                                                                 \
         _Pragma("unroll") for (int q = 0; q < B; ++q) {                                                                       \
             const int sl = (u + q + NS - W + 2) % NS;                                                                         \
             _Pragma("unroll") for (int p = 0; p < NP; ++p) {                 \
@@ -317,8 +368,10 @@
             if (gi == (1 * 2 * B) / 9) { RP_W_CENTRE(c + 3, ((u + 3) / 2) % PP) }                                             \
             if (gi == (2 * 2 * B) / 9) { RP_W_NORM() } if (gi == (3 * 2 * B) / 9) { RP_P4(c + 3) } if (gi == (4 * 2 * B) / 9) { RP_W_SCALE() } \
              \
-            if (gi == (5 * 2 * B) / 9) { RP_W_CHK(!(TAIL) || c + h <= L) RP_W_X0() } if (gi == (6 * 2 * B) / 9) { RP_W_R1() }  \
-            if (gi == (7 * 2 * B) / 9) { RP_W_X1() } if (gi == (8 * 2 * B) / 9) { RP_W_X2() }                                 \
+             \
+            if (gi == (5 * 2 * B) / 9) { RP_W_CHK(!(TAIL) || c + (upper ? 1 : 0) <= L) RP_W_X0() if (NW == 12) { RP_W_R1() } }  \
+            if (NW != 12 && gi == (6 * 2 * B) / 9) { RP_W_R1() }                                                              \
+            if (gi == (7 * 2 * B) / 9) { RP_W_X1() if (NW == 12) { RP_W_X2() } } if (NW != 12 && gi == (8 * 2 * B) / 9) { RP_W_X2() } \
             } else if (!P3) {                                                                                                 \
             if (q == (0 * B) / 10) { RP_P1(c + 2, (u + 3) % PD) RP_P0(c + 2 + PD, (u + 3) % PD) } if (q == (2 * B) / 10) { RP_P2(c + 2) }                       \
             if (q == (3 * B) / 10) { RP_P3(c + 2) } if (q == (4 * B) / 10) { RP_P4(c + 2) } if (q == (5 * B) / 10) { RP_P5(c + 2) } \
@@ -332,14 +385,15 @@
             if (q == (9 * B) / 11) { RP_P10(c + 2, (u + 1) & 1) }                                                             \
             }                                                                                                                 \
             _Pragma("unroll") for (int g = 0; g < NTILE; ++g) {                                                               \
+                if (A2L && g != gn_ && mfma_a2_request<W, NT>(u, g) == q) RP_A2_LATE(g, GUARD)                                \
                 if (mfma_last_use<W, NT>(u, g) == q) RP_MFMA(g, u & 1);                                                       \
-                if (q >= RP_P3_GAP && mfma_last_use<W, NT>(u, g) == q - RP_P3_GAP) RP_MFMA2(g, u & 1);                        \
+                if (q >= RP_P3_GAP && mfma_last_use<W, NT>(u, g) == q - RP_P3_GAP) RP_MFMA2S(g, u & 1);                       \
             }                                                                                                                 \
             __builtin_amdgcn_sched_barrier(0);                                                                                \
         }                                                                                                                     \
         _Pragma("unroll") for (int g = 0; g < NTILE; ++g) {                                                                   \
-            if (mfma_last_use<W, NT>(u, g) < 0) { RP_MFMA(g, u & 1); RP_MFMA2(g, u & 1); }                                    \
-            else if (RP_P3_GAP > 0 && mfma_last_use<W, NT>(u, g) > B - 1 - RP_P3_GAP) RP_MFMA2(g, u & 1);                     \
+            if (mfma_last_use<W, NT>(u, g) < 0) { RP_MFMA(g, u & 1); RP_MFMA2S(g, u & 1); }                                   \
+            else if (RP_P3_GAP > 0 && mfma_last_use<W, NT>(u, g) > B - 1 - RP_P3_GAP) RP_MFMA2S(g, u & 1);                    \
         }                                                                                                                     \
     } while (0)
 
@@ -373,9 +427,9 @@
             for (int u = 0; u < NS; ++u) { const int c = c0 + u; RP_STEP(true, false); }
         }
 #ifdef RP_MFMA_PRICE_NO_ABANDON
-#define RP_ABANDON_ON false
+#define RP_ABANDON_ON (AB && false)
 #else
-#define RP_ABANDON_ON (abandon_nc < RP_INF)
+#define RP_ABANDON_ON (AB && abandon_nc < RP_INF)
 #endif
 #define RP_ABANDON_CHECK()                                                                                                    \
     if (RP_ABANDON_ON) {                                                                                                \
@@ -388,15 +442,19 @@
         }                                                                                                                     \
         if (!__any(alive && valid)) dead = true;                                                                              \
     }
-        for (c0 = 1 + NS; c0 + NS - 1 <= L; c0 += NS) {
-            RP_ABANDON_CHECK()
-            if (dead) break;
-#pragma unroll
-            for (int u = 0; u < NS; ++u) { const int c = c0 + u; RP_STEP(false, false); }
+        {
+            RP_LANE_CONSTS()
+            for (c0 = 1 + NS; c0 + NS - 1 <= L; c0 += NS) {
+                RP_ABANDON_CHECK()
+                if (dead) break;
+#pragma unroll
+                for (int u = 0; u < NS; ++u) { const int c = c0 + u; RP_STEP(false, false); }
+            }
         }
         if (!dead && c0 <= L) {
             RP_ABANDON_CHECK()
             if (!dead) {
+                RP_LANE_CONSTS()
 #pragma unroll
                 for (int u = 0; u < NS - 1; ++u) {
                     const int c = c0 + u;
@@ -405,10 +463,14 @@
             }
         }
 #undef RP_ABANDON_CHECK
+#undef RP_LANE_CONSTS
 #undef RP_ABANDON_ON
 #undef RP_STEP
 #undef RP_MFMA
 #undef RP_MFMA2
+#undef RP_MFMA2X
+#undef RP_MFMA2S
+#undef RP_A2_LATE
 #undef RP_P10
 #undef RP_W_LOAD
 #undef RP_W_NEAR
@@ -443,19 +505,24 @@
 #undef RP_X0F
 
         if (round == 1) RP_TRACE(3);
+        const int lane2_ = fresh_lane_id();
+        const int h2 = lane2_ >> 5;
+        size_t s = s_gx;
+        int w = w_gx;
+        const bool valid2 = GX ? valid : locate(lane2_ & 31, s, w);
         if (WF) {
             const auto sw_ = __builtin_amdgcn_permlane32_swap(__float_as_uint(chk_), __float_as_uint(chk_), false, false);
             chk_ = fmaxf(__uint_as_float(sw_[0]), __uint_as_float(sw_[1]));
         }
         float best = 0.f;
-        if (valid) {
+        if (valid2) {
             const size_t row = s * out_win_pitch + (size_t)w;
-            const float denom = (float)(L + L);
+            const float denom = (float)not_hoisted(L + L);
 #pragma unroll
             for (int p = 0; p < NP; ++p) {
 #pragma unroll
                 for (int e = 0; e < 2; ++e) {
-                    const int slot = 2 * NP * h + 2 * p + e;
+                    const int slot = 2 * NP * h2 + 2 * p + e;
                     if (slot < ch->count) {
                         const float cost = e ? Q[p][W - 2].y : Q[p][W - 2].x;
                         const float nc = cost / denom;
@@ -466,12 +533,12 @@
                     }
                 }
             }
-            if (h == 0 && chk_ > kDtwFixLimit) dtw_fix_append(fix, row, (uint32_t)(chunk_base + (int)ci));
+            if (h2 == 0 && chk_ > kDtwFixLimit) dtw_fix_append(fix, row, (uint32_t)(chunk_base + (int)ci));
         }
         if (agg_out) {
             const auto sw_ = __builtin_amdgcn_permlane32_swap(__float_as_uint(best), __float_as_uint(best), false, false);
             const float m = fmaxf(__uint_as_float(sw_[0]), __uint_as_float(sw_[1]));
-            if (valid && h == 0) {
+            if (valid2 && h2 == 0) {
                 agg_out[s * out_win_pitch + (size_t)w] = m;
                 if (agg_hot && m > agg_threshold) agg_hot[s] = 1u;
             }
@@ -482,7 +549,23 @@
     RP_TRACE(5);
     __syncthreads();
     RP_TRACE(6);
-    dtw_release_tiles(next_tile, n_groups, tid);
+    dtw_release_tiles(next_tile, n_groups, not_hoisted(wave) * 64 + fresh_lane_id());
+}
+
+template <int W, int NW, bool GX, int NT, bool P3>
+RP_MFMA_OCC __global__ __launch_bounds__(64 * NW, 1) void dtw_mfma_kernel(RP_MFMA_PARAMS) {
+    dtw_mfma_body<W, NW, GX, NT, P3, !mfma_abandon_apart(NW, GX, NT, P3)>(RP_MFMA_ARGS);
+}
+template <int W, int NW, bool GX, int NT, bool P3>
+RP_MFMA_OCC __global__ __launch_bounds__(64 * NW, 1) void dtw_mfma_abandon_kernel(RP_MFMA_PARAMS) {
+    dtw_mfma_body<W, NW, GX, NT, P3, true>(RP_MFMA_ARGS);
+}
+#undef RP_MFMA_PARAMS
+#undef RP_MFMA_ARGS
+template <int W, int NW, bool GX, int NT, bool P3>
+constexpr auto mfma_abandon_entry() {
+    if constexpr (mfma_abandon_apart(NW, GX, NT, P3)) return dtw_mfma_abandon_kernel<W, NW, GX, NT, P3>;
+    else return dtw_mfma_kernel<W, NW, GX, NT, P3>;
 }
 
 bool dtw_mfma_supported(const TemplatesDev &t, int band, size_t n_win, bool from_global, int slots, float score_ref) {
@@ -513,8 +596,9 @@
     int nw = dtw_mfma_lds_bytes(t.max_len, 12, row_bytes) <= 160 * 1024 ? 12 : 8;
     if (p3 && slots == 8) {
         static const int env_nw = [] { const char *e = std::getenv("RP_MFMA3_WAVES"); return e ? std::atoi(e) : 0; }();
-        if (env_nw != 12) nw = 8;
-    }
+        if ((from_global || gate.abandon_nc < RP_INF) ? env_nw != 12 : env_nw == 8) nw = 8;
+    }
+    if (nw == 12) dtw_mark(wk, kDtwRanWaves12); else dtw_mark(wk, kDtwRanWaves8);
     const size_t lds = dtw_mfma_lds_bytes(t.max_len, nw, row_bytes);
     const void *image = p3 ? t.aimg3 : t.aimg;
     if (!wk.sched || !wk.fix) return hipErrorInvalidValue;
@@ -522,8 +606,9 @@
     if (hipError_t e = mfma_grid(total_tiles, n_chunks, nw, gate.list != nullptr, blocks, static_rounds); e != hipSuccess) return e;
 #define RP_LAUNCH_MFMA_P(WW, NW, GXV, NT, PP)                                                                                       \
     do {                                                                                                                            \
-        if (hipError_t e = allow_dynamic_lds(reinterpret_cast<const void *>(dtw_mfma_kernel<WW, NW, GXV, NT, PP>), 160 * 1024); e != hipSuccess) return e; \
-        hipLaunchKernelGGL((dtw_mfma_kernel<WW, NW, GXV, NT, PP>), dim3(blocks), dim3(64 * NW), lds, c.st, c.mfcc, c.frame_pitch, c.frame_pitch, \
+        const auto kernel = gate.abandon_nc < RP_INF ? mfma_abandon_entry<WW, NW, GXV, NT, PP>() : dtw_mfma_kernel<WW, NW, GXV, NT, PP>; \
+        if (hipError_t e = allow_dynamic_lds(reinterpret_cast<const void *>(kernel), 160 * 1024); e != hipSuccess) return e;        \
+        hipLaunchKernelGGL(kernel, dim3(blocks), dim3(64 * NW), lds, c.st, c.mfcc, c.frame_pitch, c.frame_pitch,                    \
                            total_tiles, (unsigned)n_chunks, chunk_base, c.first_win, c.n_win, c.out_win_pitch, t.chunks,             \
                            reinterpret_cast<const uint4 *>(image), t.T, c.score_ref, c.scores, c.avg, c.S, t.max_len, gate.list, gate.count, \
                            gate.dense_min, gate.abandon_nc, wk.sched, static_rounds, agg_out, agg_hot, agg_threshold, wk.fix);      \
diff --git a/rustpotter_amd/csrc/rp_kernels.h b/rustpotter_amd/csrc/rp_kernels.h
--- a/rustpotter_amd/csrc/rp_kernels.h
+++ b/rustpotter_amd/csrc/rp_kernels.h
@@ -160,7 +160,8 @@
     size_t rag_streams = 0, rag_rows = 0;
 };
 enum : uint32_t { kDtwRanMfma = 1u, kDtwRanMfmaWide = 2u, kDtwRanRagged = 4u, kDtwRanRegister = 8u, kDtwRanGeneric = 16u, kDtwRanSingle = 32u, kDtwRanRefAll = 64u, kDtwRanMfmaGroup = 128u,
-                  kDtwRanBf16x3 = 256u, kDtwRanF16x2 = 512u };
+                  kDtwRanBf16x3 = 256u, kDtwRanF16x2 = 512u,
+                  kDtwRanWaves8 = 1024u, kDtwRanWaves12 = 2048u };
 inline void dtw_mark(const DtwWork &wk, uint32_t bit) { if (wk.ran) *wk.ran |= bit; }
 __host__ __device__ inline unsigned long long *dtw_fix_stats(uint32_t *fix) { return reinterpret_cast<unsigned long long *>(fix + 2 + 2 * (size_t)kDtwFixCap); }
 
```

Result: faster. 924.7 million scorings/s (median of 6 runs) (+2.5%).
